# Jeremy-Cleland/hmer-img2latex

Measured on AMD Instinct MI355X. Metric: decoded LaTeX tokens/sec at batch 256, 320x64 imgs, seq 150, higher is better.
Workload: dtype f32

## Files before the change

hmer-img2latex_amd/csrc/api.hip:

```cpp
#include "common.h"
#include <new>

extern "C" int i2l_version(void) { return 107; }

extern "C" const char* i2l_error_string(int code) {
    switch (code) {
        case I2L_OK: return "ok";
        case I2L_ERR_ARG: return "invalid argument (null pointer or non-positive dimension)";
        case I2L_ERR_UNSUPPORTED: return "dimension not supported by the gfx950 kernels";
        case I2L_ERR_WORKSPACE: return "workspace missing or too small";
        case I2L_ERR_LAUNCH: return "HIP launch error";
        default: return "unknown error";
    }
}

struct i2l_lanes {
    int n = 0;
    hipStream_t s[I2L_MAX_LANES] = {};
    hipEvent_t fork[I2L_MAX_LANES] = {}, join[I2L_MAX_LANES] = {};
};

extern "C" int i2l_lanes_create(const i2l_stream_t* streams, int n, i2l_lanes** out) {
    if (!streams || !out || n < 1 || n > I2L_MAX_LANES) return I2L_ERR_ARG;
    for (int i = 0; i < n; ++i)
        if (!streams[i]) return I2L_ERR_ARG;
    i2l_lanes* l = new (std::nothrow) i2l_lanes();
    if (!l) return I2L_ERR_WORKSPACE;
    l->n = n;
    bool ok = true;
    for (int i = 0; i < n; ++i) {
        l->s[i] = i2l_s(streams[i]);
        ok = ok && hipEventCreateWithFlags(&l->fork[i], hipEventDisableTiming) == hipSuccess;
        ok = ok && hipEventCreateWithFlags(&l->join[i], hipEventDisableTiming) == hipSuccess;
    }
    if (!ok) { i2l_lanes_destroy(l); return I2L_ERR_LAUNCH; }
    *out = l;
    return I2L_OK;
}

extern "C" int i2l_lanes_destroy(i2l_lanes* l) {
    if (!l) return I2L_OK;
    for (int i = 0; i < I2L_MAX_LANES; ++i) {
        if (l->fork[i]) (void)hipEventDestroy(l->fork[i]);
        if (l->join[i]) (void)hipEventDestroy(l->join[i]);
    }
    delete l;
    return I2L_OK;
}

hipStream_t i2l_side_fork(i2l_lanes* l, hipStream_t main, int lane) {
    if (!l || lane < 0) return nullptr;
    if (lane >= l->n) lane = l->n - 1;
    if (hipEventRecord(l->fork[lane], main) != hipSuccess) return nullptr;
    if (hipStreamWaitEvent(l->s[lane], l->fork[lane], 0) != hipSuccess) return nullptr;
    return l->s[lane];
}

extern "C" int i2l_lanes_join(i2l_lanes* l, i2l_stream_t stream) {
    if (!l) return I2L_ERR_ARG;
    for (int i = 0; i < l->n; ++i) {
        if (hipEventRecord(l->join[i], l->s[i]) != hipSuccess) return I2L_ERR_LAUNCH;
        if (hipStreamWaitEvent(i2l_s(stream), l->join[i], 0) != hipSuccess) return I2L_ERR_LAUNCH;
    }
    return I2L_OK;
}

namespace {
__global__ void wait_value32_kernel(const unsigned* flag, unsigned value, long long ticks) {
    const long long t0 = (long long)wall_clock64();
    for (;;) {
        const unsigned v = __hip_atomic_load(flag, __ATOMIC_ACQUIRE, __HIP_MEMORY_SCOPE_AGENT);
        if ((int)(v - value) >= 0) return;
        if ((long long)wall_clock64() - t0 > ticks) return;
        __builtin_amdgcn_s_sleep(4);
    }
}
}

extern "C" int i2l_stream_wait_value32(const uint32_t* flag, uint32_t value, float timeout_us, i2l_stream_t stream) {
    if (!flag || !(timeout_us >= 0.f) || timeout_us > 100000.f) return I2L_ERR_ARG;
    hipLaunchKernelGGL(wait_value32_kernel, dim3(1), dim3(1), 0, i2l_s(stream), flag, value, (long long)(timeout_us * 100.f));
    return hipGetLastError() == hipSuccess ? I2L_OK : I2L_ERR_LAUNCH;
}
```

hmer-img2latex_amd/csrc/decode.hip:

```cpp
#include <math.h>
#include <stdlib.h>

#include "common.h"

namespace {

#include "lstm_rows.inc.h"

constexpr int MAXL = I2L_MAX_LSTM_LAYERS;
constexpr int NT = 256;
constexpr int VCHUNK = 2 * NT;

constexpr size_t GROUP_STATUS_BYTES = 2048;
inline bool group_shape_ok(int V, int H, int L) { return L == 1 && H == 256 && V <= 512; }

__global__ __launch_bounds__(256) void transpose_perm_kernel(const float* __restrict__ W, int N, int K,
                                                             float* __restrict__ out, int ld_out, int Npad,
                                                             int perm_h) {
    __shared__ float tile[64][65];
    const int c0 = blockIdx.x * 64, k0 = blockIdx.y * 64;
    const int tx = threadIdx.x & 63, ty = threadIdx.x >> 6;
    for (int i = ty; i < 64; i += 4) {
        const int c = c0 + i, k = k0 + tx;
        const int n = perm_h > 0 ? (c & 3) * perm_h + (c >> 2) : c;
// ... 358 lines not shown
                __syncthreads();
                if (p.top_k > 0) {
                    const int kk = min(p.top_k, V);
                    float kth = -1.f;
                    for (int v = tid; v < V; v += NT) {
                        const float pv = pr[v];
                        int gt = 0, ge = 0;
                        for (int u = 0; u < V; ++u) { const float pu = pr[u]; gt += pu > pv; ge += pu >= pv; }
                        if (gt < kk && kk <= ge) kth = pv;
                    }
                    kth = block_max(kth, redv, tid);
                    float s2 = 0.f;
                    for (int v = tid; v < V; v += NT) { const float q = pr[v] < kth ? 0.f : pr[v]; pr[v] = q; s2 += q; }
                    s2 = block_sum(s2, redv, tid);
                    if (s2 > 0.f) for (int v = tid; v < V; v += NT) pr[v] = pr[v] / s2;
                    __syncthreads();
                }
                if (p.top_p > 0.f) {
                    float* nx = lg + (size_t)(R + r) * w.Vp;
                    float s2 = 0.f;
                    for (int v = tid; v < V; v += NT) {
                        const float pv = pr[v];
                        float before = 0.f;
                        for (int u = 0; u < V; ++u) { const float pu = pr[u]; if (pu > pv || (pu == pv && u < v)) before += pu; }
                        const float q = before > p.top_p ? 0.f : pv;
                        nx[v] = q;
                        s2 += q;
                    }
                    __syncthreads();
                    for (int v = tid; v < V; v += NT) pr[v] = nx[v];
                    s2 = block_sum(s2, redv, tid);
                    if (s2 > 0.f) for (int v = tid; v < V; v += NT) pr[v] = pr[v] / s2;
                    __syncthreads();
                }
                if (p.probs && row0 + r < B) {
                    float* po = p.probs + ((size_t)(row0 + r) * T + t) * V;
                    for (int v = tid; v < V; v += NT) po[v] = pr[v];
                }
                const int CH = (V + NT - 1) / NT;
                float part = 0.f;
                for (int v = tid * CH; v < min(V, (tid + 1) * CH); ++v) part += pr[v];
                float* scan = psum;
                scan[tid] = part;
                __syncthreads();
                if (tid == 0) {
                    float run = 0.f;
                    for (int i = 0; i < NT; ++i) { const float x = scan[i]; scan[i] = run; run += x; }
                    scan[NT] = run;
                }
                __syncthreads();
                const float total = scan[NT];
                const float target = uniform01(p.seed, (unsigned)(row0 + r), (unsigned)t) * total;
                int pick = 0x7fffffff;
                float run = scan[tid];
                for (int v = tid * CH; v < min(V, (tid + 1) * CH); ++v) {
                    const float q = pr[v];
                    if (q > 0.f && run + q > target && pick == 0x7fffffff && run <= target) pick = v;
                    run += q;
                }
                float dummy = pick == 0x7fffffff ? -1.f : 1.f;
                int pk = pick;
                float bv[1] = {dummy};
                int bi[1] = {pk};
                block_argmax<1>(bv, bi, redv, redi, tid);
                besti[r] = bi[0] < V ? bi[0] : besti[r];
            }
        }
        if (tid == 0) {
#pragma unroll
            for (int r = 0; r < R; ++r) {
                const int row = row0 + r;
                const int sel = besti[r] < V ? besti[r] : 0;
                const int was_fin = fin_s[r];
                if (p.ids && row < B) p.ids[(size_t)row * T + t] = (p.stop == I2L_STOP_STICKY && was_fin) ? -1 : sel;
                tok_s[r] = sel;
                if (sel == p.end_id || row >= B) fin_s[r] = 1;
            }
        }
        __syncthreads();
        par ^= 1;
        if (p.stop == I2L_STOP_STICKY) {
            bool all = true;
#pragma unroll
            for (int r = 0; r < R; ++r) all = all && (fin_s[r] != 0);
            if (all) { ++t; break; }
        }
    }
    if (p.ids && t < T) {
        for (int idx = tid; idx < R * (T - t); idx += NT) {
            const int r = idx / (T - t), tt = t + (idx - r * (T - t));
            if (row0 + r < B) p.ids[(size_t)(row0 + r) * T + tt] = -1;
        }
    }
    if (p.h_out || p.c_out) {
        for (int idx = tid; idx < L * R * H; idx += NT) {
            const int l = idx / (R * H);
            const int rem = idx - l * (R * H);
            const int r = rem / H, j = rem - r * H;
            if (row0 + r < B) {
                const size_t g = ((size_t)l * B + row0 + r) * H + j;
                if (p.h_out) p.h_out[g] = hs[(size_t)par * L * R * H + idx];
                if (p.c_out) p.c_out[g] = cs[idx];
            }
        }
    }
}

struct BeamParams {
    StepWeights w;
    int images, T, start_id, end_id;
    int32_t* tokhist;
    int32_t* parhist;
    int32_t* seq_out;
    int32_t* len_out;
    double* score_out;
};

template <int K>
__global__ __launch_bounds__(NT) void beam_kernel(BeamParams p) {
    extern __shared__ __attribute__((aligned(16))) float smem[];
    const StepWeights& w = p.w;
    const int H = w.H, L = w.L, T = p.T, V = w.V, Vp = w.Vp;
    const int LKH = L * K * H;
    float* hs = smem;
    float* cs = hs + 2 * LKH;
    float* lg = cs + 2 * LKH;
    float* psum = lg + (size_t)K * Vp;
    double* score = reinterpret_cast<double*>(psum + K * 512);
    double* nscore = score + K;
    float* topv = reinterpret_cast<float*>(nscore + K);
    int* topi = reinterpret_cast<int*>(topv + K * K);
    int* last = topi + K * K;
    int* live = last + K;
    int* npar = live + K;
    int* ntok = npar + K;
    int* ctl = ntok + K;

    const int tid = threadIdx.x, lane = tid & 63, wave = tid >> 6;
    const int img = blockIdx.x;
    int32_t* tokhist = p.tokhist + (size_t)img * T * K;
    int32_t* parhist = p.parhist + (size_t)img * T * K;

    for (int idx = tid; idx < 2 * LKH; idx += NT) { hs[idx] = 0.f; cs[idx] = 0.f; }
    if (tid == 0) {
        for (int q = 0; q < K; ++q) { score[q] = 0.0; last[q] = p.start_id; live[q] = 0; }
        ctl[0] = 1; ctl[1] = 0; ctl[2] = 0;
    }
    bool has_c = false;
    double best_c = 0.0;
    int best_t = -1, best_q = 0;
    int t_last = -1;
    __syncthreads();

    int par = 0, cpar = 0;
    for (int t = 0; t < T; ++t) {
        if (tid == 0) {
            const int nb = ctl[0];
            int nl = 0;
            for (int q = 0; q < K; ++q) {
                int lv = 0;
                if (q < nb) {
                    if (last[q] == p.end_id) {
                        if (!has_c || score[q] > best_c) { has_c = true; best_c = score[q]; best_t = t - 1; best_q = q; }
                    } else { lv = 1; ++nl; }
                }
                live[q] = lv;
            }
            ctl[1] = nl;
        }
        __syncthreads();
        if (ctl[1] == 0) break;

        int tok[K], grow[K];
#pragma unroll
        for (int r = 0; r < K; ++r) { tok[r] = min(max(last[r], 0), V - 1); grow[r] = img; }
        lstm_layers<K>(w, tok, grow, hs, cs + (size_t)cpar * LKH, cs + (size_t)(cpar ^ 1) * LKH, par, tid);
        const float* h_top = hs + ((size_t)(par ^ 1) * L + (L - 1)) * K * H;
        float* lp[K];
#pragma unroll
        for (int r = 0; r < K; ++r) lp[r] = nullptr;
        float best[K];
        int besti[K];
        project<K>(w, h_top, lp, lg, false, 1.f, best, besti, psum, tid);
        __syncthreads();

        for (int r = wave; r < K; r += NT / 64) {
            if (!live[r]) continue;
            const float* x = lg + (size_t)r * Vp;
            float m = -INFINITY;
            for (int v = lane; v < V; v += 64) m = fmaxf(m, x[v]);
            m = wave_max(m);
            float s = 0.f;
            for (int v = lane; v < V; v += 64) s += expf(x[v] - m);
            s = wave_sum(s);
            const float lse = logf(s);
            unsigned taken = 0;
            for (int j = 0; j < K; ++j) {
                float bv = -INFINITY;
                int bi = 0x7fffffff;
                for (int v = lane, i = 0; v < V; v += 64, ++i)
                    if (!((taken >> i) & 1u) && x[v] > bv) { bv = x[v]; bi = v; }
                wave_argmax(bv, bi);
                if (bi < V && (bi & 63) == lane) taken |= 1u << (bi >> 6);
                if (lane == 0) { topv[r * K + j] = (bv - m) - lse; topi[r * K + j] = bi < V ? bi : 0; }
            }
        }
        __syncthreads();

        if (tid == 0) {
            const int nlive = ctl[1];
            const int ncand = nlive * K;
            const int nnew = ncand < K ? ncand : K;
            unsigned long long used = 0ull;
            for (int q = 0; q < nnew; ++q) {
                double bs = 0.0;
                int bc = -1;
                for (int s0 = 0; s0 < K; ++s0) {
                    if (!live[s0]) continue;
                    for (int j = 0; j < K; ++j) {
                        const int c = s0 * K + j;
                        if ((used >> c) & 1ull) continue;
                        const double sc = score[s0] + (double)topv[c];
                        if (bc < 0 || sc > bs) { bs = sc; bc = c; }
                    }
                }
                used |= 1ull << bc;
                npar[q] = bc / K;
                ntok[q] = topi[bc];
                nscore[q] = bs;
                tokhist[(size_t)t * K + q] = topi[bc];
                parhist[(size_t)t * K + q] = bc / K;
            }
            for (int q = nnew; q < K; ++q) { npar[q] = 0; ntok[q] = 0; nscore[q] = 0.0; }
            ctl[0] = nnew;
            t_last = t;
        }
        __syncthreads();

        {
            const float* hsrc = hs + (size_t)(par ^ 1) * LKH;
            float* hdst = hs + (size_t)par * LKH;
            const float* csrc = cs + (size_t)(cpar ^ 1) * LKH;
            float* cdst = cs + (size_t)cpar * LKH;
            for (int idx = tid; idx < LKH; idx += NT) {
                const int l = idx / (K * H);
                const int rem = idx - l * (K * H);
                const int q = rem / H, j = rem - q * H;
                const size_t src = ((size_t)l * K + npar[q]) * H + j;
                hdst[idx] = hsrc[src];
                cdst[idx] = csrc[src];
            }
        }
        __syncthreads();
        if (tid == 0) {
            const int nb = ctl[0];
            bool all_end = true;
            for (int q = 0; q < K; ++q) {
                score[q] = nscore[q];
                last[q] = ntok[q];
                if (q < nb && ntok[q] != p.end_id) all_end = false;
            }
            if (all_end) {
                for (int q = 0; q < nb; ++q)
                    if (!has_c || score[q] > best_c) { has_c = true; best_c = score[q]; best_t = t; best_q = q; }
                ctl[2] = 1;
            }
        }
        __syncthreads();
        if (ctl[2]) break;
    }

    if (tid == 0) {
        int tt = has_c ? best_t : t_last, q = has_c ? best_q : 0;
        const double sc = has_c ? best_c : score[0];
        int32_t* out = p.seq_out + (size_t)img * (T + 1);
        int n = tt + 1;
        for (int pos = tt; pos >= 0; --pos) {
            out[pos] = tokhist[(size_t)pos * K + q];
            q = parhist[(size_t)pos * K + q];
        }
        int len = n;
        for (int i = 0; i < n; ++i)
            if (out[i] == p.end_id) { len = i; break; }
        for (int i = len; i < T + 1; ++i) out[i] = -1;
        p.len_out[img] = len;
        if (p.score_out) p.score_out[img] = sc;
    }
}

struct GroupVariant {
    void (*kernel)(GroupParams);
    int flag;
    int rows, threads;
    size_t lds, xchg_per_group;
};
constexpr int GROUP_VARIANTS = 3;
template <int M>
constexpr GroupVariant grouped_variant(int flag) {
    using S = GroupShape<M>;
    return {decode_group_kernel<M>, flag, M, S::NT, S::LDS, S::XCHG_PER_GROUP};
}
constexpr GroupVariant group_variant(int i) {
    constexpr GroupVariant table[GROUP_VARIANTS] = {
        {decode_group16_kernel, I2L_FLAG_DECODE_GROUP16, G16Q, G16NT, GRP16_LDS, GROUP16_XCHG_PER_GROUP},
        grouped_variant<8>(I2L_FLAG_DECODE_GROUP8),
        grouped_variant<4>(0),
    };
    return table[i];
}

struct Layout {
    size_t P, Genc, WhhT[MAXL], WihT[MAXL], biasP[MAXL], WoutT, boutP, wpack16, gemm_ws, xchg, xchg_bytes, total;
    int Vp;
};

Layout make_layout(int rows, int V, int E, int H, int L) {
    Layout o{};
    size_t off = 0;
    auto take = [&](size_t floats) { size_t r = off; off += i2l_align(floats * sizeof(float)); return r; };
    const size_t G = 4 * (size_t)H;
    o.Vp = i2l_cdiv(V, VCHUNK) * VCHUNK;
    o.P = take((size_t)V * G);
    o.Genc = take((size_t)rows * G);
    for (int l = 0; l < L; ++l) o.WhhT[l] = take((size_t)H * G);
    for (int l = 1; l < L; ++l) o.WihT[l] = take((size_t)H * G);
    for (int l = 1; l < L; ++l) o.biasP[l] = take(G);
    o.WoutT = take((size_t)H * o.Vp);
    o.boutP = take(o.Vp);
    if (group_shape_ok(V, H, L)) o.wpack16 = take((size_t)16 * 4 * 36 * 64 * 4);
    size_t g1 = i2l_gemm_workspace_bytes(V, 4 * H, E), g2 = i2l_gemm_workspace_bytes(rows, 4 * H, E);
    o.gemm_ws = off;
    off += i2l_align(g1 > g2 ? g1 : g2);
    if (group_shape_ok(V, H, L)) {
        o.xchg = off;
        size_t most = 0;
        for (int i = 0; i < GROUP_VARIANTS; ++i) {
            const GroupVariant g = group_variant(i);
            const size_t x = group_xchg_bytes(i2l_cdiv(rows, g.rows), g.xchg_per_group);
            most = x > most ? x : most;
        }
        o.xchg_bytes = GROUP_STATUS_BYTES + most;
        off += i2l_align(o.xchg_bytes);
    }
    o.total = off;
    return o;
}

int check_weights(const i2l_decoder_weights* w) {
    if (!w || !w->embedding || !w->w_ih || !w->w_hh || !w->b_ih || !w->b_hh || !w->w_out || !w->b_out)
        return I2L_ERR_ARG;
    if (w->vocab <= 0 || w->embed <= 0 || w->hidden <= 0 || w->layers <= 0) return I2L_ERR_ARG;
    if (w->layers > MAXL || w->hidden % 64 != 0 || w->hidden > 2048 || w->embed % 4 != 0) return I2L_ERR_UNSUPPORTED;
    for (int l = 0; l < w->layers; ++l)
        if (!w->w_ih[l] || !w->w_hh[l] || !w->b_ih[l] || !w->b_hh[l]) return I2L_ERR_ARG;
    return I2L_OK;
}

StepWeights step_weights(const Layout& lo, const char* base, int V, int H, int L) {
    auto F = [&](size_t off) { return reinterpret_cast<const float*>(base + off); };
    StepWeights w{};
    w.H = H; w.L = L; w.V = V; w.Vp = lo.Vp;
    w.P = F(lo.P); w.Genc = F(lo.Genc);
    for (int l = 0; l < L; ++l) {
        w.WhhT[l] = F(lo.WhhT[l]);
        w.WihT[l] = l > 0 ? F(lo.WihT[l]) : nullptr;
        w.biasP[l] = l > 0 ? F(lo.biasP[l]) : nullptr;
    }
    w.WoutT = F(lo.WoutT); w.boutP = F(lo.boutP);
    w.wpack16 = lo.wpack16 ? base + lo.wpack16 : nullptr;
    return w;
}

constexpr int RES_KR = 76, RES_KL = 36;
constexpr int RES2_KR = 64, RES2_KL = 32;

size_t decode_lds_bytes(int R, int L, int H, int Vp, int select, int KL = 0) {
    size_t floats = (size_t)3 * L * R * H + 4 * R + 4 * R + R + R + 4 + (size_t)R * 512 + (size_t)KL * 4 * H;
    if (select != I2L_SELECT_LOGITS) floats += (size_t)R * Vp;
    if (select == I2L_SELECT_SAMPLE) floats += (size_t)R * Vp;
    return floats * sizeof(float);
}

}

extern "C" size_t i2l_decoder_workspace_bytes(int rows, int vocab, int embed, int hidden, int layers) {
    if (rows <= 0 || vocab <= 0 || embed <= 0 || hidden <= 0 || layers <= 0 || layers > MAXL) return 0;
    return make_layout(rows, vocab, embed, hidden, layers).total;
}

extern "C" int i2l_decoder_prepare(const i2l_decoder_weights* w, const float* enc, int rows, int what,
                                   void* workspace, size_t workspace_bytes, i2l_stream_t stream) {
    int rc = check_weights(w);
    if (rc != I2L_OK) return rc;
    if (rows <= 0 || (what & ~I2L_PREP_ALL) || what == 0) return I2L_ERR_ARG;
    if ((what & I2L_PREP_ROWS) && !enc) return I2L_ERR_ARG;
    const int V = w->vocab, E = w->embed, H = w->hidden, L = w->layers;
    const Layout lo = make_layout(rows, V, E, H, L);
    if (!workspace || workspace_bytes < lo.total) return I2L_ERR_WORKSPACE;
    char* base = static_cast<char*>(workspace);
    hipStream_t s = i2l_s(stream);
    auto F = [&](size_t off) { return reinterpret_cast<float*>(base + off); };
    const int G = 4 * H;

    for (int l = 0; l < L && (what & I2L_PREP_WEIGHTS); ++l) {
        dim3 grid(i2l_cdiv(G, 64), i2l_cdiv(H, 64));
        hipLaunchKernelGGL(transpose_perm_kernel, grid, dim3(256), 0, s, w->w_hh[l], G, H, F(lo.WhhT[l]), G, G, H);
        I2L_CHECK_LAUNCH();
        if (l > 0) {
            hipLaunchKernelGGL(transpose_perm_kernel, grid, dim3(256), 0, s, w->w_ih[l], G, H, F(lo.WihT[l]), G, G, H);
            I2L_CHECK_LAUNCH();
            hipLaunchKernelGGL(bias_perm_kernel, dim3(i2l_cdiv(G, 256)), dim3(256), 0, s, w->b_ih[l], w->b_hh[l],
                               F(lo.biasP[l]), H);
            I2L_CHECK_LAUNCH();
        }
    }
    if (what & I2L_PREP_WEIGHTS) {
        dim3 grid(i2l_cdiv(lo.Vp, 64), i2l_cdiv(H, 64));
        hipLaunchKernelGGL(transpose_perm_kernel, grid, dim3(256), 0, s, w->w_out, V, H, F(lo.WoutT), lo.Vp, lo.Vp, 0);
        I2L_CHECK_LAUNCH();
        hipLaunchKernelGGL(bout_pad_kernel, dim3(i2l_cdiv(lo.Vp, 256)), dim3(256), 0, s, w->b_out, F(lo.boutP), V, lo.Vp);
        I2L_CHECK_LAUNCH();
        if (lo.wpack16) {
            hipLaunchKernelGGL(pack16_kernel, dim3(16 * 4), dim3(64), 0, s, F(lo.WhhT[0]), F(lo.WoutT),
                               reinterpret_cast<u32x4_t*>(base + lo.wpack16));
            I2L_CHECK_LAUNCH();
        }
    }
    const size_t gws = lo.total - lo.gemm_ws;
    if (what & I2L_PREP_WEIGHTS) {
        GemmArgs g = gemm_args();
        g.A = w->embedding; g.lda = E;
        g.W = w->w_ih[0]; g.ldw = 2 * E;
        g.C = F(lo.P); g.ldc = G;
        g.M = V; g.N = G; g.K = E; g.perm_h = H;
        rc = i2l_gemm(g, base + lo.gemm_ws, gws, s);
        if (rc != I2L_OK) return rc;
    }
    if (what & I2L_PREP_ROWS) {
        GemmArgs g = gemm_args();
        g.A = enc; g.lda = E;
        g.W = w->w_ih[0] + E; g.ldw = 2 * E;
        g.bias = w->b_ih[0]; g.bias2 = w->b_hh[0];
        g.C = F(lo.Genc); g.ldc = G;
        g.M = rows; g.N = G; g.K = E; g.perm_h = H;
        rc = i2l_gemm(g, base + lo.gemm_ws, gws, s);
        if (rc != I2L_OK) return rc;
    }
    return I2L_OK;
}

namespace {
int launch_decode(const i2l_decoder_weights* w, const void* workspace, int rows, int steps, const int32_t* tok0,
                  const int32_t* forced, const float* h0, const float* c0, float temperature, int select, int stop,
                  int end_id, int top_k, float top_p, unsigned long long seed, int32_t* ids_out, float* logits_out,
                  float* probs_out, float* h_out, float* c_out, i2l_stream_t stream, int rows_per_wg = 0, int flags = 0,
                  uint32_t* resident_flag = nullptr, uint32_t resident_value = 0);
}

extern "C" int i2l_greedy_decode_ex(const i2l_decoder_weights* w, const void* workspace, int rows, int steps,
                                    const int32_t* tok0, const int32_t* forced, const float* h0, const float* c0,
                                    float temperature, int select, int stop, int end_id, int rows_per_workgroup,
                                    int32_t* ids_out, float* logits_out, float* h_out, float* c_out, int flags,
                                    uint32_t* resident_flag, uint32_t resident_value, i2l_stream_t stream) {
    if (select != I2L_SELECT_LOGITS && select != I2L_SELECT_SOFTMAX) return I2L_ERR_ARG;
    if (rows_per_workgroup != 0 && rows_per_workgroup != 1 && rows_per_workgroup != 2 && rows_per_workgroup != 4)
        return I2L_ERR_ARG;
    return launch_decode(w, workspace, rows, steps, tok0, forced, h0, c0, temperature, select, stop, end_id, 0, 0.f, 0ull,
                         ids_out, logits_out, nullptr, h_out, c_out, stream, rows_per_workgroup, flags, resident_flag,
                         resident_value);
}

extern "C" int i2l_greedy_decode(const i2l_decoder_weights* w, const void* workspace, int rows, int steps,
                                 const int32_t* tok0, const int32_t* forced, const float* h0, const float* c0,
                                 float temperature, int select, int stop, int end_id, int32_t* ids_out,
                                 float* logits_out, float* h_out, float* c_out, i2l_stream_t stream) {
    if (select != I2L_SELECT_LOGITS && select != I2L_SELECT_SOFTMAX) return I2L_ERR_ARG;
    return launch_decode(w, workspace, rows, steps, tok0, forced, h0, c0, temperature, select, stop, end_id, 0, 0.f, 0ull,
                         ids_out, logits_out, nullptr, h_out, c_out, stream);
}

extern "C" int i2l_sample_decode(const i2l_decoder_weights* w, const void* workspace, int rows, int steps,
                                 const int32_t* tok0, const float* h0, const float* c0, float temperature, int top_k,
                                 float top_p, uint64_t seed, int stop, int end_id, int32_t* ids_out, float* probs_out,
                                 float* h_out, float* c_out, i2l_stream_t stream) {
    if (!(temperature > 0.f) || top_k < 0 || top_p < 0.f || (top_k == 0 && top_p == 0.f)) return I2L_ERR_ARG;
    if (w && w->vocab > 8 * 256) return I2L_ERR_UNSUPPORTED;
    return launch_decode(w, workspace, rows, steps, tok0, nullptr, h0, c0, temperature, I2L_SELECT_SAMPLE, stop, end_id,
                         top_k, top_p, (unsigned long long)seed, ids_out, nullptr, probs_out, h_out, c_out, stream);
}

namespace {
__global__ void publish_value32_kernel(unsigned* flag, unsigned value) { publish_max32(flag, value); }

int launch_decode(const i2l_decoder_weights* w, const void* workspace, int rows, int steps, const int32_t* tok0,
                  const int32_t* forced, const float* h0, const float* c0, float temperature, int select, int stop,
                  int end_id, int top_k, float top_p, unsigned long long seed, int32_t* ids_out, float* logits_out,
                  float* probs_out, float* h_out, float* c_out, i2l_stream_t stream, int rows_per_wg, int flags,
                  uint32_t* resident_flag, uint32_t resident_value) {
    int rc = check_weights(w);
    if (rc != I2L_OK) return rc;
    if (!workspace || !tok0 || rows <= 0 || steps <= 0) return I2L_ERR_ARG;
    if ((h0 == nullptr) != (c0 == nullptr)) return I2L_ERR_ARG;
    if (stop != I2L_STOP_NONE && stop != I2L_STOP_STICKY) return I2L_ERR_ARG;
    const int V = w->vocab, E = w->embed, H = w->hidden, L = w->layers;
    const Layout lo = make_layout(rows, V, E, H, L);
    const char* base = static_cast<const char*>(workspace);

    DecodeParams p{};
    p.w = step_weights(lo, base, V, H, L);
    p.B = rows; p.T = steps;
    p.tok0 = tok0; p.forced = forced; p.h0 = h0; p.c0 = c0;
    p.h_out = h_out; p.c_out = c_out; p.ids = ids_out; p.logits = logits_out;
    p.temperature = temperature; p.use_temp = (temperature != 1.0f) ? 1 : 0;
    p.select = select; p.stop = stop; p.end_id = end_id;
    p.top_k = top_k; p.top_p = top_p; p.seed = seed; p.probs = probs_out;

    if (rows_per_wg == 0 && lo.xchg_bytes && (select == I2L_SELECT_LOGITS || select == I2L_SELECT_SOFTMAX) && !h0 &&
        !h_out && !c_out &&
        steps >= 8 && steps <= 65000) {
        GroupParams gp{};
        gp.w = p.w; gp.B = rows; gp.T = steps;
        gp.tok0 = tok0; gp.forced = forced; gp.ids = ids_out; gp.logits = logits_out;
        gp.temperature = temperature; gp.use_temp = p.use_temp; gp.stop = stop; gp.end_id = end_id;
        char* xb = const_cast<char*>(base) + lo.xchg;
        gp.status = reinterpret_cast<unsigned*>(xb);
        gp.xchg = reinterpret_cast<u64_t*>(xb + GROUP_STATUS_BYTES);
        gp.opts = group_opts(steps, flags);
        gp.resident_flag = resident_flag; gp.resident_value = resident_value;
        hipStream_t gs = i2l_s(stream);
        const bool ids_only = ids_out && !logits_out && !forced;
        static std::atomic<unsigned> attr[GROUP_VARIANTS]{};
        for (int i = 0; i < GROUP_VARIANTS; ++i) {
            const GroupVariant g = group_variant(i);
            if (g.flag && !((flags & g.flag) && ids_only)) continue;
            if (!i2l_lds_attr(reinterpret_cast<const void*>(g.kernel), g.lds, attr[i])) continue;
            if (!(flags & I2L_FLAG_DECODE_REGION_CLEARED) && hipMemsetAsync(xb, 0, lo.xchg_bytes, gs) != hipSuccess) return I2L_ERR_LAUNCH;
            gp.n_groups = i2l_cdiv(rows, g.rows);
            hipLaunchKernelGGL(g.kernel, dim3(group_grid(gp.n_groups, g.rows)), dim3(g.threads), g.lds, gs, gp);
            I2L_CHECK_LAUNCH();
            return I2L_OK;
        }
    }
    if (resident_flag) {
        hipLaunchKernelGGL(publish_value32_kernel, dim3(1), dim3(1), 0, i2l_s(stream), resident_flag, resident_value);
        I2L_CHECK_LAUNCH();
    }
    int R = rows <= 256 ? 1 : (rows <= 512 ? 2 : 4);
    if (rows_per_wg > 0) R = rows_per_wg;
    while (R > 1 && decode_lds_bytes(R, L, H, lo.Vp, select) > 64 * 1024) R >>= 1;
    const size_t lds = decode_lds_bytes(R, L, H, lo.Vp, select);
    if (lds > 64 * 1024) return I2L_ERR_UNSUPPORTED;
    const dim3 grid(i2l_cdiv(rows, R));
    hipStream_t s = i2l_s(stream);
    if (select == I2L_SELECT_SAMPLE) {
        if (R == 1) hipLaunchKernelGGL((decode_kernel<1, 0, 0, true>), grid, dim3(NT), lds, s, p);
        else if (R == 2) hipLaunchKernelGGL((decode_kernel<2, 0, 0, true>), grid, dim3(NT), lds, s, p);
        else hipLaunchKernelGGL((decode_kernel<4, 0, 0, true>), grid, dim3(NT), lds, s, p);
        I2L_CHECK_LAUNCH();
        return I2L_OK;
    }
    const bool resident = (R == 1 || R == 2) && L == 1 && H == 256 && steps >= 8;
    if (resident) {
        const size_t lds_r = decode_lds_bytes(R, 1, H, lo.Vp, select, R == 1 ? RES_KL : RES2_KL);
        auto kern = R == 1 ? decode_kernel<1, RES_KR, RES_KL> : decode_kernel<2, RES2_KR, RES2_KL>;
        if (lds_r <= 160 * 1024 &&
            hipFuncSetAttribute(reinterpret_cast<const void*>(kern), hipFuncAttributeMaxDynamicSharedMemorySize,
                                (int)lds_r) == hipSuccess) {
            hipLaunchKernelGGL(kern, grid, dim3(NT), lds_r, s, p);
            I2L_CHECK_LAUNCH();
            return I2L_OK;
        }
    }
    if (R == 1) hipLaunchKernelGGL((decode_kernel<1, 0, 0>), grid, dim3(NT), lds, s, p);
    else if (R == 2) hipLaunchKernelGGL((decode_kernel<2, 0, 0>), grid, dim3(NT), lds, s, p);
    else hipLaunchKernelGGL((decode_kernel<4, 0, 0>), grid, dim3(NT), lds, s, p);
    I2L_CHECK_LAUNCH();
    return I2L_OK;
}
}

extern "C" size_t i2l_decode_batched_scratch_bytes(int rows, int vocab, int hidden, int layers) {
    if (!batched_dims_ok(rows, vocab, hidden, layers)) return 0;
    return batched_layout(rows, i2l_cdiv(vocab, VCHUNK) * VCHUNK, hidden, layers).total;
}

namespace {
template <int TB>
void launch_batched_lstm(const BatchedParams& p, int layer, int t, hipStream_t s) {
    hipLaunchKernelGGL(lstm_step_mfma_kernel<TB>, dim3(p.w.H / 16, i2l_cdiv(p.B, TB)), dim3(DB_NT), 0, s, p, layer, t);
}
template <int TB>
void launch_batched_logits(const BatchedParams& p, int t, hipStream_t s) {
    hipLaunchKernelGGL(logits_mfma_kernel<TB>, dim3(p.w.Vp / DB_COLS, i2l_cdiv(p.B, TB)), dim3(DB_NT), 0, s, p, t);
}
}

extern "C" int i2l_greedy_decode_batched(const i2l_decoder_weights* w, const void* workspace, int rows, int steps,
                                         const int32_t* tok0, const int32_t* forced, const float* h0, const float* c0,
                                         float temperature, int select, int stop, int end_id, int32_t* ids_out,
                                         float* logits_out, float* h_out, float* c_out, void* scratch,
                                         size_t scratch_bytes, int flags, uint32_t* resident_flag,
                                         uint32_t resident_value, i2l_stream_t stream) {
    (void)flags;
    int rc = check_weights(w);
    if (rc != I2L_OK) return rc;
    if (select != I2L_SELECT_LOGITS && select != I2L_SELECT_SOFTMAX) return I2L_ERR_ARG;
    if (!workspace || !tok0 || rows <= 0 || steps <= 0) return I2L_ERR_ARG;
    if ((h0 == nullptr) != (c0 == nullptr)) return I2L_ERR_ARG;
    if (stop != I2L_STOP_NONE && stop != I2L_STOP_STICKY) return I2L_ERR_ARG;
    const int V = w->vocab, E = w->embed, H = w->hidden, L = w->layers;
    const Layout lo = make_layout(rows, V, E, H, L);
    const BatchedLayout bl = batched_layout(rows, lo.Vp, H, L);
    if (!scratch || scratch_bytes < bl.total) return I2L_ERR_WORKSPACE;

    char* sb = static_cast<char*>(scratch);
    BatchedParams p{};
    p.w = step_weights(lo, static_cast<const char*>(workspace), V, H, L);
    p.B = rows; p.T = steps; p.genc_div = 1; p.forced = forced;
    p.h = reinterpret_cast<float*>(sb + bl.h); p.c = reinterpret_cast<float*>(sb + bl.c);
    p.lg = reinterpret_cast<float*>(sb + bl.lg);
    p.tok = reinterpret_cast<int*>(sb + bl.tok); p.fin = reinterpret_cast<int*>(sb + bl.fin);
    p.live = reinterpret_cast<unsigned*>(sb + bl.live);
    p.ids = ids_out; p.logits_out = logits_out;
    p.temperature = temperature; p.use_temp = (temperature != 1.0f) ? 1 : 0;
    p.select = select; p.stop = stop; p.end_id = end_id;

    hipStream_t s = i2l_s(stream);
    if (resident_flag) {
        hipLaunchKernelGGL(publish_value32_kernel, dim3(1), dim3(1), 0, s, resident_flag, resident_value);
        I2L_CHECK_LAUNCH();
    }
    const size_t most = (size_t)L * rows * H > (size_t)rows * steps ? (size_t)L * rows * H : (size_t)rows * steps;
    const size_t copy_blocks = (most + DB_NT - 1) / DB_NT;
    const int copy_grid = (int)(copy_blocks < 1024 ? copy_blocks : 1024);
    hipLaunchKernelGGL(init_batched_kernel, dim3(copy_grid), dim3(DB_NT), 0, s, p, tok0, h0, c0);
    I2L_CHECK_LAUNCH();
    const int tb_lstm = batched_tile_rows(H / 16, rows), tb_logits = batched_tile_rows(lo.Vp / DB_COLS, rows);
    const int sel_grid = i2l_cdiv(rows, DB_NT / 64);
    for (int t = 0; t < steps; ++t) {
        for (int l = 0; l < L; ++l) {
            if (tb_lstm == 16) launch_batched_lstm<16>(p, l, t, s);
            else if (tb_lstm == 32) launch_batched_lstm<32>(p, l, t, s);
            else launch_batched_lstm<64>(p, l, t, s);
        }
        if (tb_logits == 16) launch_batched_logits<16>(p, t, s);
        else if (tb_logits == 32) launch_batched_logits<32>(p, t, s);
        else launch_batched_logits<64>(p, t, s);
        hipLaunchKernelGGL(select_batched_kernel, dim3(sel_grid), dim3(DB_NT), 0, s, p, t);
        I2L_CHECK_LAUNCH();
    }
    if (h_out || c_out) {
        hipLaunchKernelGGL(state_out_batched_kernel, dim3(copy_grid), dim3(DB_NT), 0, s, p, h_out, c_out);
        I2L_CHECK_LAUNCH();
    }
    return I2L_OK;
}

namespace {

size_t beam_lds_bytes(int K, int L, int H, int Vp) {
    size_t b = (size_t)4 * L * K * H * sizeof(float) + (size_t)K * Vp * sizeof(float) + (size_t)K * 512 * sizeof(float);
    b = (b + 7) / 8 * 8;
    b += 2 * (size_t)K * sizeof(double) + (size_t)2 * K * K * 4 + (size_t)4 * K * 4 + 4 * 4;
    return b;
}

template <int K>
int launch_beam(const BeamParams& p, size_t lds, hipStream_t s) {
    if (lds > 64 * 1024) {
        if (hipFuncSetAttribute(reinterpret_cast<const void*>(&beam_kernel<K>),
                                hipFuncAttributeMaxDynamicSharedMemorySize, (int)lds) != hipSuccess)
            return I2L_ERR_UNSUPPORTED;
    }
    hipLaunchKernelGGL(beam_kernel<K>, dim3(p.images), dim3(NT), lds, s, p);
    I2L_CHECK_LAUNCH();
    return I2L_OK;
}

}

namespace {
inline bool beam_group_ok(int beam, int H, int L) { return L == 1 && H == 256 && beam >= 2 && beam <= 6; }
inline int beam_groups(int images, int beam) { return i2l_cdiv(images, BG_S / beam); }
inline size_t beam_hist_bytes(int images, int beam, int steps) {
    return i2l_align((size_t)2 * images * steps * beam * sizeof(int32_t));
}
template <int K>
int launch_beam_group(const BeamGroupParams& p, hipStream_t s) {
    constexpr size_t lds = bg_lds_bytes();
    static_assert(lds <= 160 * 1024, "beam_group_kernel LDS");
    static std::atomic<unsigned> attr{0};
    if (!i2l_lds_attr(reinterpret_cast<const void*>(&beam_group_kernel<K>), lds, attr)) return I2L_ERR_UNSUPPORTED;
    hipLaunchKernelGGL(beam_group_kernel<K>, dim3(group_grid(p.n_groups, GQ)), dim3(GNT), lds, s, p);
    I2L_CHECK_LAUNCH();
    return I2L_OK;
}
}

extern "C" size_t i2l_beam_workspace_bytes(int images, int beam, int hidden, int layers, int steps) {
    if (images <= 0 || beam <= 0 || beam > I2L_MAX_BEAM || steps <= 0) return 0;
    size_t b = beam_hist_bytes(images, beam, steps);
    if (beam_group_ok(beam, hidden, layers))
        b += GROUP_STATUS_BYTES + group_xchg_bytes(beam_groups(images, beam), BEAM_XCHG_PER_GROUP);
    return b;
}

extern "C" int i2l_beam_decode(const i2l_decoder_weights* w, const void* workspace, int images, int beam, int steps,
                               int start_id, int end_id, void* beam_workspace, size_t beam_workspace_bytes,
                               int32_t* seq_out, int32_t* len_out, double* score_out, int flags, i2l_stream_t stream) {
    int rc = check_weights(w);
    if (rc != I2L_OK) return rc;
    if (!workspace || !beam_workspace || !seq_out || !len_out || images <= 0 || steps <= 0 || beam <= 0)
        return I2L_ERR_ARG;
    if (beam > I2L_MAX_BEAM || beam > w->vocab) return I2L_ERR_UNSUPPORTED;
    const size_t need = (size_t)2 * images * steps * beam * sizeof(int32_t);
    if (beam_workspace_bytes < need) return I2L_ERR_WORKSPACE;
    const int V = w->vocab, E = w->embed, H = w->hidden, L = w->layers;
    const Layout lo = make_layout(images, V, E, H, L);
    if (lo.Vp > 64 * 32) return I2L_ERR_UNSUPPORTED;
    hipStream_t s = i2l_s(stream);
    const bool group_on = !(flags & I2L_FLAG_NO_GROUP);
    if (group_on && beam_group_ok(beam, H, L) && V <= 512 && steps <= 65000 &&
        beam_workspace_bytes >= i2l_beam_workspace_bytes(images, beam, H, L, steps)) {
        BeamGroupParams gp{};
        gp.w = step_weights(lo, static_cast<const char*>(workspace), V, H, L);
        gp.images = images; gp.T = steps; gp.n_groups = beam_groups(images, beam);
        gp.start_id = start_id; gp.end_id = end_id;
        gp.tokhist = static_cast<int32_t*>(beam_workspace);
        gp.parhist = gp.tokhist + (size_t)images * steps * beam;
        gp.seq_out = seq_out; gp.len_out = len_out; gp.score_out = score_out;
        char* xb = static_cast<char*>(beam_workspace) + beam_hist_bytes(images, beam, steps);
        const size_t xbytes = GROUP_STATUS_BYTES + group_xchg_bytes(gp.n_groups, BEAM_XCHG_PER_GROUP);
        gp.status = reinterpret_cast<unsigned*>(xb);
        gp.xchg = reinterpret_cast<u64_t*>(xb + GROUP_STATUS_BYTES);
        gp.opts = group_opts(steps, flags);
        if (hipMemsetAsync(xb, 0, xbytes, s) != hipSuccess) return I2L_ERR_LAUNCH;
        switch (beam) {
            case 2: return launch_beam_group<2>(gp, s);
            case 3: return launch_beam_group<3>(gp, s);
            case 4: return launch_beam_group<4>(gp, s);
            case 5: return launch_beam_group<5>(gp, s);
            case 6: return launch_beam_group<6>(gp, s);
            default: break;
        }
    }
    BeamParams p{};
    p.w = step_weights(lo, static_cast<const char*>(workspace), V, H, L);
    p.images = images; p.T = steps; p.start_id = start_id; p.end_id = end_id;
    p.tokhist = static_cast<int32_t*>(beam_workspace);
    p.parhist = p.tokhist + (size_t)images * steps * beam;
    p.seq_out = seq_out; p.len_out = len_out; p.score_out = score_out;
    const size_t lds = beam_lds_bytes(beam, L, H, lo.Vp);
    if (lds > 160 * 1024) return I2L_ERR_UNSUPPORTED;
    switch (beam) {
        case 1: return launch_beam<1>(p, lds, s);
        case 2: return launch_beam<2>(p, lds, s);
        case 3: return launch_beam<3>(p, lds, s);
        case 4: return launch_beam<4>(p, lds, s);
        case 5: return launch_beam<5>(p, lds, s);
        case 6: return launch_beam<6>(p, lds, s);
        case 7: return launch_beam<7>(p, lds, s);
        case 8: return launch_beam<8>(p, lds, s);
        default: return I2L_ERR_UNSUPPORTED;
    }
}

extern "C" size_t i2l_beam_batched_scratch_bytes(int images, int beam, int vocab, int hidden, int layers, int steps) {
    if (!beam_batched_dims_ok(images, beam, vocab, hidden, layers, steps)) return 0;
    return beam_batched_layout(images, beam, i2l_cdiv(vocab, VCHUNK) * VCHUNK, hidden, layers, steps).total;
}

namespace {
template <int K>
void launch_beam_step_batched(const BeamBatchedParams& p, float* c_cur, float* c_next, int t, hipStream_t s) {
    hipLaunchKernelGGL(beam_step_batched_kernel<K>, dim3(p.images), dim3(DB_NT), 0, s, p, c_cur, c_next, t);
}
}

extern "C" int i2l_beam_decode_batched(const i2l_decoder_weights* w, const void* workspace, int images, int beam,
                                       int steps, int start_id, int end_id, void* scratch, size_t scratch_bytes,
                                       int32_t* seq_out, int32_t* len_out, double* score_out, int flags,
                                       i2l_stream_t stream) {
    (void)flags;
    int rc = check_weights(w);
    if (rc != I2L_OK) return rc;
    if (!workspace || !scratch || !seq_out || !len_out || images <= 0 || steps <= 0 || beam <= 0) return I2L_ERR_ARG;
    const int V = w->vocab, E = w->embed, H = w->hidden, L = w->layers;
    if (!beam_batched_dims_ok(images, beam, V, H, L, steps)) return I2L_ERR_UNSUPPORTED;
    const Layout lo = make_layout(images, V, E, H, L);
    const BeamBatchedLayout bl = beam_batched_layout(images, beam, lo.Vp, H, L, steps);
    if (scratch_bytes < bl.total) return I2L_ERR_WORKSPACE;

    char* sb = static_cast<char*>(scratch);
    const int R = images * beam;
    const size_t LRH = (size_t)L * R * H;
    BeamBatchedParams bp{};
    bp.images = images; bp.T = steps; bp.V = V; bp.Vp = lo.Vp; bp.H = H; bp.L = L;
    bp.start_id = start_id; bp.end_id = end_id;
    bp.tokhist = reinterpret_cast<int32_t*>(sb + bl.hist);
    bp.parhist = bp.tokhist + (size_t)images * steps * beam;
    bp.h = reinterpret_cast<float*>(sb + bl.h); bp.c = reinterpret_cast<float*>(sb + bl.c);
    bp.lg = reinterpret_cast<float*>(sb + bl.lg);
    bp.score = reinterpret_cast<double*>(sb + bl.score);
    bp.last = reinterpret_cast<int*>(sb + bl.last); bp.slot_live = reinterpret_cast<int*>(sb + bl.slot_live);
    bp.img = reinterpret_cast<BeamImage*>(sb + bl.img);
    bp.live = reinterpret_cast<unsigned*>(sb + bl.live);
    bp.seq_out = seq_out; bp.len_out = len_out; bp.score_out = score_out;

    BatchedParams p{};
    p.w = step_weights(lo, static_cast<const char*>(workspace), V, H, L);
    p.B = R; p.T = steps; p.genc_div = beam; p.forced = nullptr;
    p.h = bp.h; p.lg = reinterpret_cast<float*>(sb + bl.lg);
    p.tok = bp.last; p.live = bp.live;
    p.temperature = 1.0f; p.select = I2L_SELECT_LOGITS; p.stop = I2L_STOP_NONE; p.end_id = end_id;

    hipStream_t s = i2l_s(stream);
    const size_t init_blocks = (2 * LRH + DB_NT - 1) / DB_NT;
    hipLaunchKernelGGL(beam_init_batched_kernel, dim3((unsigned)(init_blocks < 1024 ? init_blocks : 1024)), dim3(DB_NT), 0,
                       s, bp, beam);
    I2L_CHECK_LAUNCH();
    const int tb_lstm = batched_tile_rows(H / 16, R), tb_logits = batched_tile_rows(lo.Vp / DB_COLS, R);
    for (int t = 0; t < steps; ++t) {
        float* c_cur = bp.c + (size_t)(t & 1) * LRH;
        float* c_next = bp.c + (size_t)((t + 1) & 1) * LRH;
        p.c = c_cur;
        for (int l = 0; l < L; ++l) {
            if (tb_lstm == 16) launch_batched_lstm<16>(p, l, 0, s);
            else if (tb_lstm == 32) launch_batched_lstm<32>(p, l, 0, s);
            else launch_batched_lstm<64>(p, l, 0, s);
        }
        if (tb_logits == 16) launch_batched_logits<16>(p, 0, s);
        else if (tb_logits == 32) launch_batched_logits<32>(p, 0, s);
        else launch_batched_logits<64>(p, 0, s);
        switch (beam) {
            case 1: launch_beam_step_batched<1>(bp, c_cur, c_next, t, s); break;
            case 2: launch_beam_step_batched<2>(bp, c_cur, c_next, t, s); break;
            case 3: launch_beam_step_batched<3>(bp, c_cur, c_next, t, s); break;
            case 4: launch_beam_step_batched<4>(bp, c_cur, c_next, t, s); break;
            case 5: launch_beam_step_batched<5>(bp, c_cur, c_next, t, s); break;
            case 6: launch_beam_step_batched<6>(bp, c_cur, c_next, t, s); break;
            case 7: launch_beam_step_batched<7>(bp, c_cur, c_next, t, s); break;
            default: launch_beam_step_batched<8>(bp, c_cur, c_next, t, s); break;
        }
        I2L_CHECK_LAUNCH();
    }
    hipLaunchKernelGGL(beam_final_batched_kernel, dim3(i2l_cdiv(images, DB_NT)), dim3(DB_NT), 0, s, bp, beam);
    I2L_CHECK_LAUNCH();
    return I2L_OK;
}

extern "C" size_t i2l_decoder_group_status_offset(int rows, int vocab, int embed, int hidden, int layers) {
    const Layout lo = make_layout(rows, vocab, embed, hidden, layers);
    return lo.xchg_bytes ? lo.xchg : 0;
}

extern "C" size_t i2l_decoder_group_region_bytes(int rows, int vocab, int embed, int hidden, int layers) {
    return make_layout(rows, vocab, embed, hidden, layers).xchg_bytes;
}

#ifdef I2L_GROUP_STAMPS
extern "C" size_t i2l_debug_group_status_offset(int rows, int vocab, int embed, int hidden, int layers) {
    return make_layout(rows, vocab, embed, hidden, layers).xchg;
}
#endif
```

hmer-img2latex_amd/csrc/decode_group.inc.h:

```cpp
#include "group_common.inc.h"

constexpr int GQ = 4;
constexpr int GNT = 512;
constexpr int GRAN_H = 256;
constexpr int GRAN_C = GRAN_H;
constexpr int GRAN_X = GRAN_H + 16;
constexpr int GRAN = GRAN_H + 32;

template <int M>
struct GroupShape {
    static_assert(M == 4 || M == 8, "members per group");
    static constexpr int NT = 2048 / M;
    static constexpr int UPM = 256 / M;
    static constexpr int CPM = 512 / M;
    static constexpr size_t LDS = (size_t)(256 * CPM + 2 * 256 * M + (M == 4 ? 4 * NT : 0)) * sizeof(float) +
                                  (size_t)2 * M * 8 + 8 * sizeof(int);
    static constexpr size_t XCHG_PER_GROUP = (size_t)2 * M * GRAN * 8;
};

struct GroupParams {
    StepWeights w;
    int B, T, n_groups;
    const int32_t* tok0;
    const int32_t* forced;
    int32_t* ids;
    float* logits;
    float temperature;
    int use_temp, stop, end_id;
    u64_t* xchg;
    unsigned* status;
    GroupOpts opts;
    unsigned* resident_flag;
    unsigned resident_value;
};

constexpr int DPP_SHL12 = 0x10C;

template <int NT>
__device__ __forceinline__ void load_weight_image(f32x2 (&wreg)[32][2], float4* wout_s4, const StepWeights& w, int unit,
                                                  int ke, int col, int ks, int tid) {
#pragma unroll
    for (int j = 0; j < 32; ++j) {
        const float4 t4 = *reinterpret_cast<const float4*>(w.WhhT[0] + (size_t)(8 * j + ke) * 1024 + 4 * unit);
        wreg[j][0] = f32x2{t4.x, t4.y};
        wreg[j][1] = f32x2{t4.z, t4.w};
    }
#pragma unroll
    for (int j = 0; j < 16; ++j)
        wout_s4[j * NT + tid] = *reinterpret_cast<const float4*>(w.WoutT + (size_t)(16 * j + ks) * 512 + col);
}

template <class Hook>
__device__ __forceinline__ void rec_product4(f32x2 (&acc)[4][2], const f32x2 (&wreg)[32][2], const float4* hq4,
                                             Hook&& hook) {
    float4 hb[2][4];
#pragma unroll
    for (int i = 0; i < 4; ++i) hb[0][i] = hq4[8 * i];
#pragma unroll
    for (int b = 0; b < 8; ++b) {
        if (b + 1 < 8) {
#pragma unroll
            for (int i = 0; i < 4; ++i) hb[(b + 1) & 1][i] = hq4[8 * ((b + 1) * 4 + i)];
        }
        hook(b);
        __builtin_amdgcn_sched_barrier(0);
#pragma unroll
        for (int i = 0; i < 4; ++i) fma_4x4(acc, wreg[b * 4 + i][0], wreg[b * 4 + i][1], hb[b & 1][i]);
    }
}
__device__ __forceinline__ void fold_gates4(const f32x2 (&acc)[4][2], int ke, float (&z)[2]) {
    const bool b0 = ke & 1, b1 = ke & 2, b2 = ke & 4;
#pragma unroll
    for (int e = 0; e < 2; ++e) {
        float wv[2];
#pragma unroll
        for (int rp = 0; rp < 2; ++rp) {
            const float ux = rs_level<DPP_HMIRROR>(acc[e][rp].x, acc[2 + e][rp].x, b2);
            const float uy = rs_level<DPP_HMIRROR>(acc[e][rp].y, acc[2 + e][rp].y, b2);
            wv[rp] = rs_level<DPP_XOR1>(ux, uy, b0);
        }
        z[e] = rs_level<DPP_XOR2>(wv[0], wv[1], b1);
    }
}
template <int NT>
__device__ __forceinline__ void logits_product4(f32x2 (&pa)[4][2], const float4* wout_s4, const float4* hq4, int tid) {
#pragma unroll
    for (int c = 0; c < 4; ++c) { pa[c][0] = splat2(0.f); pa[c][1] = splat2(0.f); }
    float4 wb[2][2], hb[2][2];
    auto fetch = [&](int set, int b) {
#pragma unroll
        for (int i = 0; i < 2; ++i) {
            wb[set][i] = wout_s4[(b * 2 + i) * NT + tid];
            hb[set][i] = hq4[16 * (b * 2 + i)];
        }
    };
    fetch(0, 0);
#pragma unroll
    for (int b = 0; b < 8; ++b) {
        if (b + 1 < 8) fetch((b + 1) & 1, b + 1);
        __builtin_amdgcn_sched_barrier(0);
#pragma unroll
        for (int i = 0; i < 2; ++i) {
            const float4 w4 = wb[b & 1][i];
            fma_4x4(pa, f32x2{w4.x, w4.y}, f32x2{w4.z, w4.w}, hb[b & 1][i]);
        }
    }
}
__device__ __forceinline__ float fold_logits4(const f32x2 (&pa)[4][2], int ks) {
    const bool b0 = ks & 1, b1 = ks & 2, b2 = ks & 4, b3 = ks & 8;
    float z[2];
#pragma unroll
    for (int e = 0; e < 2; ++e) {
        float wv[2];
#pragma unroll
        for (int rp = 0; rp < 2; ++rp) {
            const float ux = rs_level<DPP_HMIRROR>(pa[e][rp].x, pa[2 + e][rp].x, b2);
            const float uy = rs_level<DPP_HMIRROR>(pa[e][rp].y, pa[2 + e][rp].y, b2);
            wv[rp] = rs_level<DPP_XOR1>(ux, uy, b0);
        }
        z[e] = rs_level<DPP_XOR2>(wv[0], wv[1], b1);
    }
    return rs_level<DPP_ROR8>(z[0], z[1], b3);
}

template <class Hook>
__device__ __forceinline__ void rec_product8(f32x2 (&acc)[2][4][2], const f32x2 (&wreg)[32][2], const float4* hq4,
                                             Hook&& hook) {
    float4 hb[2][2][2];
#pragma unroll
    for (int i = 0; i < 2; ++i) { hb[0][i][0] = hq4[16 * i]; hb[0][i][1] = hq4[16 * i + 1]; }
#pragma unroll
    for (int b = 0; b < 16; ++b) {
        if (b + 1 < 16) {
#pragma unroll
            for (int i = 0; i < 2; ++i) {
                hb[(b + 1) & 1][i][0] = hq4[16 * ((b + 1) * 2 + i)];
                hb[(b + 1) & 1][i][1] = hq4[16 * ((b + 1) * 2 + i) + 1];
            }
        }
        hook(b);
        __builtin_amdgcn_sched_barrier(0);
#pragma unroll
        for (int i = 0; i < 2; ++i) {
            fma_4x4(acc[0], wreg[b * 2 + i][0], wreg[b * 2 + i][1], hb[b & 1][i][0]);
            fma_4x4(acc[1], wreg[b * 2 + i][0], wreg[b * 2 + i][1], hb[b & 1][i][1]);
        }
    }
}
__device__ __forceinline__ void fold_gates8(const f32x2 (&acc)[2][4][2], int ke, float (&z)[4]) {
    const bool b0 = ke & 1, b1 = ke & 2, b2 = ke & 4;
#pragma unroll
    for (int g = 0; g < 4; ++g) {
        const float u0x = rs_level<DPP_HMIRROR>(acc[0][g][0].x, acc[1][g][0].x, b2);
        const float u0y = rs_level<DPP_HMIRROR>(acc[0][g][0].y, acc[1][g][0].y, b2);
        const float u1x = rs_level<DPP_HMIRROR>(acc[0][g][1].x, acc[1][g][1].x, b2);
        const float u1y = rs_level<DPP_HMIRROR>(acc[0][g][1].y, acc[1][g][1].y, b2);
        const float vx = rs_level<DPP_XOR2>(u0x, u1x, b1);
        const float vy = rs_level<DPP_XOR2>(u0y, u1y, b1);
        z[g] = rs_level<DPP_XOR1>(vx, vy, b0);
    }
}
template <int NT>
__device__ __forceinline__ void logits_product8(f32x2 (&pa)[2][4][2], const float4* wout_s4, const float4* hq4, int tid) {
#pragma unroll
    for (int hf = 0; hf < 2; ++hf)
#pragma unroll
        for (int c = 0; c < 4; ++c) { pa[hf][c][0] = splat2(0.f); pa[hf][c][1] = splat2(0.f); }
    float4 wb[2], hb[2][2];
    wb[0] = wout_s4[tid];
    hb[0][0] = hq4[0]; hb[0][1] = hq4[1];
#pragma unroll
    for (int j = 0; j < 16; ++j) {
        if (j + 1 < 16) {
            wb[(j + 1) & 1] = wout_s4[(j + 1) * NT + tid];
            hb[(j + 1) & 1][0] = hq4[32 * (j + 1)];
            hb[(j + 1) & 1][1] = hq4[32 * (j + 1) + 1];
        }
        __builtin_amdgcn_sched_barrier(0);
        const float4 w4 = wb[j & 1];
        fma_4x4(pa[0], f32x2{w4.x, w4.y}, f32x2{w4.z, w4.w}, hb[j & 1][0]);
        fma_4x4(pa[1], f32x2{w4.x, w4.y}, f32x2{w4.z, w4.w}, hb[j & 1][1]);
    }
}
__device__ __forceinline__ void fold_logits8(const f32x2 (&pa)[2][4][2], int ks, float (&lv)[2]) {
    const bool b0 = ks & 1, b1 = ks & 2, b2 = ks & 4, b3 = ks & 8;
    float v[4];
#pragma unroll
    for (int c = 0; c < 4; ++c) {
        const float u0x = rs_level<DPP_ROR8>(pa[0][c][0].x, pa[1][c][0].x, b3);
        const float u0y = rs_level<DPP_ROR8>(pa[0][c][0].y, pa[1][c][0].y, b3);
        const float u1x = rs_level<DPP_ROR8>(pa[0][c][1].x, pa[1][c][1].x, b3);
        const float u1y = rs_level<DPP_ROR8>(pa[0][c][1].y, pa[1][c][1].y, b3);
        const float wx = rs_level<DPP_HMIRROR>(u0x, u1x, b2);
        const float wy = rs_level<DPP_HMIRROR>(u0y, u1y, b2);
        v[c] = rs_level<DPP_XOR2>(wx, wy, b1);
    }
    lv[0] = rs_level<DPP_XOR1>(v[0], v[2], b0);
    lv[1] = rs_level<DPP_XOR1>(v[1], v[3], b0);
}

template <int M>
__global__ __launch_bounds__(GroupShape<M>::NT) void decode_group_kernel(GroupParams p) {
    using S = GroupShape<M>;
    constexpr int NT = S::NT, UPM = S::UPM, CPM = S::CPM;
    constexpr bool FULL = M == 4;
    extern __shared__ __attribute__((aligned(16))) float smem[];
    float4* wout_s4 = reinterpret_cast<float4*>(smem);
    float* h_s = smem + 256 * CPM;
    float4* genc_s = reinterpret_cast<float4*>(h_s + 2 * 256 * M);
    u64_t* redk = reinterpret_cast<u64_t*>(genc_s + (M == 4 ? NT : 0));
    int* cnt_s = reinterpret_cast<int*>(redk + 2 * M);

    const StepWeights& w = p.w;
    const int tid = threadIdx.x, lane = tid & 63, wave = tid >> 6;
    const GroupSeat seat = group_seat<M>();
    const int group = seat.group, m = seat.m;
    if (group >= p.n_groups) return;
    const int B = p.B, T = p.T, V = w.V;
    const int row0 = group * M;
    const int ul = tid >> 3, ke = tid & 7;
    const int unit = UPM * m + ul;
    const int cq = tid >> 4, ks = tid & 15;
    const int l_row = M == 4 ? ks & 3 : ks >> 1;
    const int l_v = CPM * m + 4 * cq + (M == 4 ? ((ks >> 2) & 1) * 2 + (ks >> 3) : 2 * (ks & 1));
    const int my_r = ke & (M - 1);
    constexpr int G = 1024;

    f32x2 wreg[32][2];
    load_weight_image<NT>(wreg, wout_s4, w, unit, ke, CPM * m + 4 * cq, ks, tid);
    for (int idx = tid; idx < 2 * 256 * M; idx += NT) h_s[idx] = 0.f;
    if (tid < 2 * M) redk[tid] = 0;
    if (tid < 4) cnt_s[tid] = 0;
    float4 genc;
    {
        const float4 g4 = *reinterpret_cast<const float4*>(w.Genc + (size_t)min(row0 + my_r, B - 1) * G + 4 * unit);
        if constexpr (M == 4) genc_s[tid] = g4; else genc = g4;
    }
    float l_bias[M / 4];
#pragma unroll
    for (int i = 0; i < M / 4; ++i) l_bias[i] = w.boutP[l_v + i];
    float c_own = 0.f, h_own = 0.f;
    unsigned fin = 0;
#pragma unroll
    for (int r = 0; r < M; ++r)
        if (row0 + r >= B) fin |= 1u << r;
    u64_t* xg = p.xchg + (size_t)group * 2 * M * GRAN;
    const bool own_row = row0 + m < B;
    int32_t* ids_row = (p.ids && own_row) ? p.ids + (size_t)(row0 + m) * T : nullptr;
    float* lrow = (FULL && p.logits && row0 + l_row < B && l_v < V) ? p.logits + (size_t)(row0 + l_row) * T * V + l_v
                                                                    : nullptr;
    __syncthreads();
    if (wave == 0) {
        const Placement pl = group_placement<M>(xg, GRAN, GRAN_X, m, p.opts);
        if (lane == 0) {
            cnt_s[3] = (pl.one_xcd && !pl.timed_out) ? 1 : 0;
            if (pl.timed_out) cnt_s[2] = 1;
            if (m == 0 && !pl.timed_out)
                report_group(p.status, p.n_groups, p.resident_flag, p.resident_value, pl.one_xcd && !p.opts.agent_scope);
        }
    }
    __syncthreads();
    const bool local = cnt_s[3] != 0 && !p.opts.agent_scope;

    int mytok = min(max(p.tok0[min(row0 + my_r, B - 1)], 0), V - 1);
    if (FULL && p.forced) mytok = min(max(p.forced[(size_t)min(row0 + my_r, B - 1) * T], 0), V - 1);
    float4 pvec = *reinterpret_cast<const float4*>(w.P + (size_t)mytok * G + 4 * unit);

    int t = 0;
    bool failed = cnt_s[2] != 0;
    I2L_STAMPS_BEGIN;
    for (; !failed; ++t) {
        f32x2 acc[M / 4][4][2];
#pragma unroll
        for (int hf = 0; hf < M / 4; ++hf)
#pragma unroll
            for (int g = 0; g < 4; ++g) { acc[hf][g][0] = splat2(0.f); acc[hf][g][1] = splat2(0.f); }
        const float* hprev = h_s + ((t - 1) & 1) * 256 * M;
        const u64_t* cand_src = xg + (size_t)((t - 1) & 1) * M * GRAN + (size_t)((lane / M) & (M - 1)) * GRAN + GRAN_C +
                                (lane & (M - 1));
        const unsigned c_epoch = (unsigned)t;
        bool have = t == 0;
        int tk[M] = {};
        u64_t gv = 0;
        auto issue = [&]() {
            if (lane < M * M) gv = load_granule(cand_src);
        };
        auto check = [&]() {
            if (!__all(lane >= M * M || (unsigned)(gv >> 48) == c_epoch)) return;
            u64_t best;
            if constexpr (M == 4) {
                const int g_lo = (int)(unsigned)gv, g_hi = (int)(unsigned)(gv >> 32);
                best = am_key(__int_as_float(g_lo), g_hi & 0xFFFF);
                best = umax64(best, am_key(__int_as_float(__builtin_amdgcn_mov_dpp(g_lo, DPP_SHL4, 0xF, 0xF, true)),
                                           __builtin_amdgcn_mov_dpp(g_hi, DPP_SHL4, 0xF, 0xF, true) & 0xFFFF));
                best = umax64(best, am_key(__int_as_float(__builtin_amdgcn_mov_dpp(g_lo, DPP_SHL8, 0xF, 0xF, true)),
                                           __builtin_amdgcn_mov_dpp(g_hi, DPP_SHL8, 0xF, 0xF, true) & 0xFFFF));
                best = umax64(best, am_key(__int_as_float(__builtin_amdgcn_mov_dpp(g_lo, DPP_SHL12, 0xF, 0xF, true)),
                                           __builtin_amdgcn_mov_dpp(g_hi, DPP_SHL12, 0xF, 0xF, true) & 0xFFFF));
            } else {
                best = am_key(__uint_as_float((unsigned)gv), (int)((unsigned)(gv >> 32) & 0xFFFFu));
                best = umax64(best, dpp_u64<DPP_SHL8>(best));
                best = umax64(best, (u64_t)__shfl_xor((unsigned long long)best, 16));
                best = umax64(best, (u64_t)__shfl_xor((unsigned long long)best, 32));
            }
            const int bi = am_idx(best);
#pragma unroll
            for (int r = 0; r < M; ++r) {
                tk[r] = __builtin_amdgcn_readlane(bi, r);
                tk[r] = tk[r] < V ? tk[r] : 0;
            }
            have = true;
            if (t < T) {
                mytok = tk[0];
#pragma unroll
                for (int r = 1; r < M; ++r) mytok = my_r == r ? tk[r] : mytok;
                if (FULL && p.forced) mytok = min(max(p.forced[(size_t)min(row0 + my_r, B - 1) * T + t], 0), V - 1);
                pvec = *reinterpret_cast<const float4*>(w.P + (size_t)mytok * G + 4 * unit);
            }
        };
        if (t > 0 && t < T) {
            constexpr int NB = 2 * M;
            auto poll = [&](int b) {
                if (b == NB / 8) issue();
                if (b == NB / 2) { check(); if (!have) issue(); }
                if (b == NB - NB / 8 && !have) check();
            };
            if constexpr (M == 4) rec_product4(acc[0], wreg, reinterpret_cast<const float4*>(hprev) + ke, poll);
            else rec_product8(acc, wreg, reinterpret_cast<const float4*>(hprev) + 2 * ke, poll);
        }
        I2L_STAMP(0);
        bool bail = false;
        if (!have) {
            PollClock clk;
            for (;;) {
                issue();
                check();
// ... 137 lines not shown
```

hmer-img2latex_amd/csrc/decode_group16.inc.h:

```cpp
#include "mfma_slab.inc.h"

constexpr int G16Q = 16;
constexpr int G16NT = 256;
constexpr int G16GRAN_H = 256;
constexpr int G16GRAN_C = G16GRAN_H;
constexpr int G16GRAN_X = G16GRAN_H + 16;
constexpr int G16GRAN = G16GRAN_H + 32;
constexpr int G16_HP_PIECE = 32 * 16 * 8;
constexpr size_t GRP16_LDS = (size_t)2 * 3 * G16_HP_PIECE * 2 + (size_t)2 * 64 * 16 + (size_t)2 * 16 * 8 + 8 * sizeof(int);
constexpr size_t GROUP16_XCHG_PER_GROUP = (size_t)2 * G16Q * G16GRAN * 8;

__device__ __forceinline__ void load_run64(const u64_t* src, u32x4_t (&g)[4]) {
    asm volatile(
        "global_load_dwordx4 %0, %4, off sc1\n\t"
        "global_load_dwordx4 %1, %4, off offset:16 sc1\n\t"
        "global_load_dwordx4 %2, %4, off offset:32 sc1\n\t"
        "global_load_dwordx4 %3, %4, off offset:48 sc1\n\t"
        "s_waitcnt vmcnt(0)"
        : "=&v"(g[0]), "=&v"(g[1]), "=&v"(g[2]), "=&v"(g[3])
        : "v"(src)
        : "memory");
}

__global__ __launch_bounds__(64) void pack16_kernel(const float* __restrict__ WhhT, const float* __restrict__ WoutT,
                                                    u32x4_t* __restrict__ pack) {
    const int m = blockIdx.x >> 2, wave = blockIdx.x & 3, lane = threadIdx.x;
    const int lhi = lane >> 4, lcol = lane & 15, ltile = wave & 1, lhalf = wave >> 1;
    u32x4_t* dst = pack + (size_t)blockIdx.x * 36 * 64 + lane;
    const float* src = WhhT + 64 * m + 16 * wave + lcol;
    for (int ks = 0; ks < 8; ++ks) {
        Frag16 f0, f1, f2;
#pragma unroll
        for (int j = 0; j < 8; ++j) split3(src[(size_t)(32 * ks + 8 * lhi + j) * 1024], f0.s[j], f1.s[j], f2.s[j]);
        dst[(ks * 3 + 0) * 64] = f0.q; dst[(ks * 3 + 1) * 64] = f1.q; dst[(ks * 3 + 2) * 64] = f2.q;
    }
    const float* srl = WoutT + 32 * m + 16 * ltile + lcol;
    for (int ks = 0; ks < 4; ++ks) {
        Frag16 f0, f1, f2;
#pragma unroll
        for (int j = 0; j < 8; ++j) split3(srl[(size_t)(32 * (4 * lhalf + ks) + 8 * lhi + j) * 512], f0.s[j], f1.s[j], f2.s[j]);
        dst[(24 + ks * 3 + 0) * 64] = f0.q; dst[(24 + ks * 3 + 1) * 64] = f1.q; dst[(24 + ks * 3 + 2) * 64] = f2.q;
    }
}

__device__ __forceinline__ void load_run64x2(const u64_t* s0, const u64_t* s1, u32x4_t (&g)[8]) {
    asm volatile(
        "global_load_dwordx4 %0, %8, off sc1\n\t"
        "global_load_dwordx4 %1, %8, off offset:16 sc1\n\t"
        "global_load_dwordx4 %2, %8, off offset:32 sc1\n\t"
        "global_load_dwordx4 %3, %8, off offset:48 sc1\n\t"
        "global_load_dwordx4 %4, %9, off sc1\n\t"
        "global_load_dwordx4 %5, %9, off offset:16 sc1\n\t"
        "global_load_dwordx4 %6, %9, off offset:32 sc1\n\t"
        "global_load_dwordx4 %7, %9, off offset:48 sc1\n\t"
        "s_waitcnt vmcnt(0)"
        : "=&v"(g[0]), "=&v"(g[1]), "=&v"(g[2]), "=&v"(g[3]), "=&v"(g[4]), "=&v"(g[5]), "=&v"(g[6]), "=&v"(g[7])
        : "v"(s0), "v"(s1)
        : "memory");
}
__device__ __forceinline__ void unpack_run(const u32x4_t* g, u32x4_t* dst) {
    u32x4_t o0, o1, o2;
    o0.x = (g[0].y & 0xFFFFu) | (g[0].w << 16); o0.y = (g[1].y & 0xFFFFu) | (g[1].w << 16);
    o0.z = (g[2].y & 0xFFFFu) | (g[2].w << 16); o0.w = (g[3].y & 0xFFFFu) | (g[3].w << 16);
    o1.x = (g[0].x >> 16) | (g[0].z & 0xFFFF0000u); o1.y = (g[1].x >> 16) | (g[1].z & 0xFFFF0000u);
    o1.z = (g[2].x >> 16) | (g[2].z & 0xFFFF0000u); o1.w = (g[3].x >> 16) | (g[3].z & 0xFFFF0000u);
    o2.x = (g[0].x & 0xFFFFu) | (g[0].z << 16); o2.y = (g[1].x & 0xFFFFu) | (g[1].z << 16);
    o2.z = (g[2].x & 0xFFFFu) | (g[2].z << 16); o2.w = (g[3].x & 0xFFFFu) | (g[3].z << 16);
    dst[0] = o0;
    dst[G16_HP_PIECE / 8] = o1;
    dst[2 * (G16_HP_PIECE / 8)] = o2;
}

__global__ __launch_bounds__(G16NT, 2) void decode_group16_kernel(GroupParams p) {
    extern __shared__ __attribute__((aligned(16))) unsigned char smem16[];
    unsigned short* hp = reinterpret_cast<unsigned short*>(smem16);
    f32x4_t* lpart = reinterpret_cast<f32x4_t*>(smem16 + (size_t)2 * 3 * G16_HP_PIECE * 2);
    u64_t* redk = reinterpret_cast<u64_t*>(lpart + 2 * 64);
    int* cnt_s = reinterpret_cast<int*>(redk + 2 * 16);
    const StepWeights& w = p.w;
    const int tid = threadIdx.x, lane = tid & 63, wave = tid >> 6;
    const int within = blockIdx.x & 127;
    const int group = (blockIdx.x >> 7) * 8 + (within & 7), m = within >> 3;
    if (group >= p.n_groups) return;
    const int B = p.B, T = p.T, V = w.V;
    const int row0 = group * G16Q;
    constexpr int G = 1024;
    const int lq = lane & 3, uq = (lane >> 2) & 3, lhi = lane >> 4, lcol = lane & 15;
    const int cell_row = 4 * lhi + lq;
    const int unit = 16 * m + 4 * wave + uq;
    const int ltile = wave & 1, lhalf = wave >> 1;

    u64_t* xg = p.xchg + (size_t)group * 2 * G16Q * G16GRAN;
    if (tid < 8) cnt_s[tid] = 0;
    if (wave == 0) {
        unsigned xcc;
        asm volatile("s_getreg_b32 %0, hwreg(HW_REG_XCC_ID)" : "=s"(xcc));
        xcc &= 0xFu;
        if (lane == 0 && !(p.opts.drop_member && m == 3))
            store_granule(xg + (size_t)m * G16GRAN + G16GRAN_X, granule(0xC0DEu, __uint_as_float(xcc)), false);
        const int pq = (lane & 15) + ((lane & 15) >= m ? 1 : 0);
        u64_t pv = 0;
        bool bad = false;
        long long t_start = 0;
        unsigned spins = 0;
        for (;;) {
            bool ok = true;
            if (lane < 15) { pv = load_granule(xg + (size_t)pq * G16GRAN + G16GRAN_X); ok = (unsigned)(pv >> 32) == 0xC0DEu; }
            if (__all(ok)) break;
            __builtin_amdgcn_s_sleep(1);
            if ((++spins & 255u) == 0) {
                const long long now = (long long)wall_clock64();
                if (t_start == 0) t_start = now;
                else if (now - t_start > p.opts.limit_first) { bad = true; break; }
            }
        }
        const bool all_same = __all(lane >= 15 || (unsigned)pv == xcc);
        if (lane == 0) {
            cnt_s[3] = (all_same && !bad) ? 1 : 0;
            if (bad) cnt_s[2] = 1;
            if (m == 0 && !bad) {
                count_resident_group(p.status, p.n_groups, p.resident_flag, p.resident_value);
                if (all_same && !p.opts.agent_scope) atomicAdd(p.status + GRP_STAT_LOCAL, 1u);
            }
        }
    }
    bf16x8_t wg[24], wl[12];
    {
        const u32x4_t* pk = static_cast<const u32x4_t*>(w.wpack16) + (size_t)(m * 4 + wave) * 36 * 64 + lane;
#pragma unroll
        for (int i = 0; i < 24; ++i) { Frag16 f; f.q = pk[i * 64]; wg[i] = f.v; }
#pragma unroll
        for (int i = 0; i < 12; ++i) { Frag16 f; f.q = pk[(24 + i) * 64]; wl[i] = f.v; }
    }
    for (int idx = tid; idx < 2 * 3 * G16_HP_PIECE / 2; idx += G16NT) reinterpret_cast<unsigned*>(hp)[idx] = 0u;
    if (tid < 32) redk[tid] = 0;
    const float4 genc = *reinterpret_cast<const float4*>(w.Genc + (size_t)min(row0 + cell_row, B - 1) * G + 4 * unit);
    const float l_bias = w.boutP[32 * m + 16 * ltile + lcol];
    float c_own = 0.f, h_own = 0.f;
    unsigned fin = 0;
#pragma unroll
    for (int r = 0; r < G16Q; ++r)
        if (row0 + r >= B) fin |= 1u << r;
    const bool own_row = row0 + m < B;
    int32_t* ids_row = (p.ids && own_row) ? p.ids + (size_t)(row0 + m) * T : nullptr;

    __syncthreads();
    const bool local = cnt_s[3] != 0 && !p.opts.agent_scope;

    int mytok = min(max(p.tok0[min(row0 + cell_row, B - 1)], 0), V - 1);
    float4 pvec = *reinterpret_cast<const float4*>(w.P + (size_t)mytok * G + 4 * unit);

    int t = 0;
    bool failed = cnt_s[2] != 0;
#ifdef I2L_GROUP_STAMPS
    long long st_acc[8] = {0, 0, 0, 0, 0, 0, 0, 0};
    long long st_last = (long long)wall_clock64();
#define I2L_STAMP16(i) do { const long long n_ = (long long)wall_clock64(); st_acc[i] += n_ - st_last; st_last = n_; } while (0)
#else
#define I2L_STAMP16(i) do { } while (0)
#endif
    for (; !failed; ++t) {
        f32x4_t acc[3];
#pragma unroll
        for (int c = 0; c < 3; ++c) acc[c] = f32x4_t{0.f, 0.f, 0.f, 0.f};
        const u64_t* cand_src = xg + (size_t)((t - 1) & 1) * G16Q * G16GRAN + (size_t)(4 * lhi) * G16GRAN + G16GRAN_C + lcol;
        const unsigned c_epoch = (unsigned)t & 0xFFFFu;
        bool have = t == 0;
        int tk[16];
#pragma unroll
        for (int r = 0; r < 16; ++r) tk[r] = 0;
        u64_t gv[4] = {0, 0, 0, 0};
        auto issue = [&]() {
#pragma unroll
            for (int i = 0; i < 4; ++i) gv[i] = load_granule(cand_src + (size_t)i * G16GRAN);
        };
        auto check = [&]() {
            bool ok = true;
#pragma unroll
            for (int i = 0; i < 4; ++i) ok = ok && (unsigned)(gv[i] >> 48) == c_epoch;
            if (!__all(ok)) return;
            u64_t best = 0;
#pragma unroll
            for (int i = 0; i < 4; ++i)
                best = umax64(best, am_key(__uint_as_float((unsigned)gv[i]), (int)((unsigned)(gv[i] >> 32) & 0xFFFFu)));
            best = umax64(best, (u64_t)__shfl_xor((unsigned long long)best, 16));
            best = umax64(best, (u64_t)__shfl_xor((unsigned long long)best, 32));
            const int bi = am_idx(best);
#pragma unroll
            for (int r = 0; r < 16; ++r) {
                tk[r] = __builtin_amdgcn_readlane(bi, r);
                tk[r] = tk[r] < V ? tk[r] : 0;
            }
            have = true;
            if (t < T) {
                mytok = __shfl(bi, cell_row);
                mytok = mytok < V ? mytok : 0;
                pvec = *reinterpret_cast<const float4*>(w.P + (size_t)mytok * G + 4 * unit);
            }
        };
        if (t > 0 && t < T) {
            const u32x4_t* hq = reinterpret_cast<const u32x4_t*>(hp + (size_t)((t - 1) & 1) * 3 * G16_HP_PIECE) + lhi * 16 + lcol;
            issue();
            Frag16 fa[2][3];
#pragma unroll
            for (int c = 0; c < 3; ++c) fa[0][c].q = hq[(c * 32) * 16];
#pragma unroll
            for (int ks = 0; ks < 8; ++ks) {
                if (ks + 1 < 8) {
#pragma unroll
                    for (int c = 0; c < 3; ++c) fa[(ks + 1) & 1][c].q = hq[(c * 32 + 4 * (ks + 1)) * 16];
                }
                if (ks == 6) { check(); if (!have) issue(); }
                __builtin_amdgcn_sched_barrier(0);
                const bf16x8_t a0 = fa[ks & 1][0].v, a1 = fa[ks & 1][1].v, a2 = fa[ks & 1][2].v;
                acc[0] = __builtin_amdgcn_mfma_f32_16x16x32_bf16(a0, wg[ks * 3 + 0], acc[0], 0, 0, 0);
                acc[1] = __builtin_amdgcn_mfma_f32_16x16x32_bf16(a0, wg[ks * 3 + 1], acc[1], 0, 0, 0);
                acc[1] = __builtin_amdgcn_mfma_f32_16x16x32_bf16(a1, wg[ks * 3 + 0], acc[1], 0, 0, 0);
                acc[2] = __builtin_amdgcn_mfma_f32_16x16x32_bf16(a0, wg[ks * 3 + 2], acc[2], 0, 0, 0);
                acc[2] = __builtin_amdgcn_mfma_f32_16x16x32_bf16(a1, wg[ks * 3 + 1], acc[2], 0, 0, 0);
                acc[2] = __builtin_amdgcn_mfma_f32_16x16x32_bf16(a2, wg[ks * 3 + 0], acc[2], 0, 0, 0);
            }
            if (!have) check();
        }
        I2L_STAMP16(0);
        bool bail = false;
        if (!have) {
            long long t_start = 0;
            unsigned spins = 0;
            for (;;) {
                issue();
                check();
                if (have) break;
                __builtin_amdgcn_s_sleep(1);
                if ((++spins & 255u) == 0) {
                    const long long now = (long long)wall_clock64();
                    if (t_start == 0) t_start = now;
                    else if (now - t_start > p.opts.limit_step) { bail = true; break; }
                }
            }
            if (bail) cnt_s[2] = 1;
        }
        if (t > 0 && !bail) {
            bool all_fin = true;
#pragma unroll
            for (int r = 0; r < G16Q; ++r) {
                const bool was_fin = (fin >> r) & 1u;
                if (r == m && tid == 0 && ids_row) ids_row[t - 1] = (p.stop == I2L_STOP_STICKY && was_fin) ? -1 : tk[r];
                if (tk[r] == p.end_id) fin |= 1u << r;
                all_fin = all_fin && ((fin >> r) & 1u);
            }
            if (t == T || (p.stop == I2L_STOP_STICKY && all_fin)) break;
        }
        I2L_STAMP16(1);
        const unsigned epoch = ((unsigned)t + 1u) & 0xFFFFu;
        const int par = t & 1;
        u64_t* slot = xg + (size_t)par * G16Q * G16GRAN;
        unsigned short* hcur = hp + (size_t)par * 3 * G16_HP_PIECE;
        if (!bail) {
            const bool b0 = lq & 1, b1 = lq & 2;
            float z[4];
#pragma unroll
            for (int i = 0; i < 4; ++i) z[i] = (acc[2][i] + acc[1][i]) + acc[0][i];
            const float r0 = dpp_f<DPP_XOR1>(b0 ? z[0] : z[1]), r1 = dpp_f<DPP_XOR1>(b0 ? z[2] : z[3]);
            const float e0 = b0 ? r0 : z[0], e1 = b0 ? z[1] : r0, e2 = b0 ? r1 : z[2], e3 = b0 ? z[3] : r1;
            const float s0 = dpp_f<DPP_XOR2>(b1 ? e0 : e2), s1 = dpp_f<DPP_XOR2>(b1 ? e1 : e3);
            const float gi = b1 ? s0 : e0, gf = b1 ? s1 : e1, gc = b1 ? e2 : s0, go = b1 ? e3 : s1;
            const float xi = (gi + genc.x) + pvec.x, xf = (gf + genc.y) + pvec.y;
            const float xc = (gc + genc.z) + pvec.z, xo = (go + genc.w) + pvec.w;
            const float ig = sigmoidf_(xi), fg = sigmoidf_(xf), gg = tanhf_(xc), og = sigmoidf_(xo);
            c_own = fg * c_own + ig * gg;
            h_own = og * tanhf_(c_own);
            unsigned short q0, q1, q2;
            split3(h_own, q0, q1, q2);
            const int ul = 4 * wave + uq;
            const u64_t gran = ((u64_t)epoch << 48) | ((u64_t)q0 << 32) | ((u64_t)q1 << 16) | (u64_t)q2;
            store_granule(slot + (size_t)m * G16GRAN + ((ul >> 3) * 16 + cell_row) * 8 + (ul & 7), gran, local);
            const int o = ((2 * m + (ul >> 3)) * 16 + cell_row) * 8 + (ul & 7);
            hcur[o] = q0;
            hcur[G16_HP_PIECE + o] = q1;
            hcur[2 * G16_HP_PIECE + o] = q2;
        }
        I2L_STAMP16(2);
        if (!bail) {
            const int ta = tid, tb = tid + G16NT < 15 * 32 ? tid + G16NT : tid;
            const int qa_ = ta >> 5, qa = qa_ + (qa_ >= m ? 1 : 0), qb_ = tb >> 5, qb = qb_ + (qb_ >= m ? 1 : 0);
            const u64_t* sa = slot + (size_t)qa * G16GRAN + (((ta >> 4) & 1) * 16 + (ta & 15)) * 8;
            const u64_t* sb = slot + (size_t)qb * G16GRAN + (((tb >> 4) & 1) * 16 + (tb & 15)) * 8;
            u32x4_t g[8];
            long long t_start = 0;
            unsigned spins = 0;
            for (;;) {
                load_run64x2(sa, sb, g);
                bool ok = true;
#pragma unroll
                for (int i = 0; i < 8; ++i) ok = ok && (g[i].y >> 16) == epoch && (g[i].w >> 16) == epoch;
                if (ok) break;
                __builtin_amdgcn_s_sleep(1);
                if ((++spins & 255u) == 0) {
                    const long long now = (long long)wall_clock64();
                    if (t_start == 0) t_start = now;
                    else if (now - t_start > p.opts.limit_step) { cnt_s[2] = 1; break; }
                }
            }
            unpack_run(g, reinterpret_cast<u32x4_t*>(hcur) + (2 * qa + ((ta >> 4) & 1)) * 16 + (ta & 15));
            unpack_run(g + 4, reinterpret_cast<u32x4_t*>(hcur) + (2 * qb + ((tb >> 4) & 1)) * 16 + (tb & 15));
        }
        I2L_STAMP16(3);
        __syncthreads();
        if (cnt_s[2] != 0) { failed = true; break; }
        I2L_STAMP16(4);

        {
            f32x4_t la[3] = {f32x4_t{0.f, 0.f, 0.f, 0.f}, f32x4_t{0.f, 0.f, 0.f, 0.f}, f32x4_t{0.f, 0.f, 0.f, 0.f}};
            const u32x4_t* hq = reinterpret_cast<const u32x4_t*>(hcur) + lhi * 16 + lcol;
            Frag16 fa[4][3];
#pragma unroll
            for (int ks = 0; ks < 4; ++ks)
#pragma unroll
                for (int c = 0; c < 3; ++c) fa[ks][c].q = hq[(c * 32 + 4 * (4 * lhalf + ks)) * 16];
#pragma unroll
            for (int ks = 0; ks < 4; ++ks) {
                const bf16x8_t a0 = fa[ks][0].v, a1 = fa[ks][1].v, a2 = fa[ks][2].v;
                la[0] = __builtin_amdgcn_mfma_f32_16x16x32_bf16(a0, wl[ks * 3 + 0], la[0], 0, 0, 0);
                la[1] = __builtin_amdgcn_mfma_f32_16x16x32_bf16(a0, wl[ks * 3 + 1], la[1], 0, 0, 0);
                la[1] = __builtin_amdgcn_mfma_f32_16x16x32_bf16(a1, wl[ks * 3 + 0], la[1], 0, 0, 0);
                la[2] = __builtin_amdgcn_mfma_f32_16x16x32_bf16(a0, wl[ks * 3 + 2], la[2], 0, 0, 0);
                la[2] = __builtin_amdgcn_mfma_f32_16x16x32_bf16(a1, wl[ks * 3 + 1], la[2], 0, 0, 0);
                la[2] = __builtin_amdgcn_mfma_f32_16x16x32_bf16(a2, wl[ks * 3 + 0], la[2], 0, 0, 0);
            }
            f32x4_t part;
#pragma unroll
            for (int i = 0; i < 4; ++i) part[i] = (la[2][i] + la[1][i]) + la[0][i];
            if (lhalf == 1) {
                lpart[ltile * 64 + lane] = part;
                if (lane == 0) __hip_atomic_store(cnt_s + 4 + ltile, (int)epoch, __ATOMIC_RELEASE, __HIP_MEMORY_SCOPE_WORKGROUP);
                I2L_STAMP16(5);
            } else {
                while (__hip_atomic_load(cnt_s + 4 + ltile, __ATOMIC_ACQUIRE, __HIP_MEMORY_SCOPE_WORKGROUP) != (int)epoch)
                    __builtin_amdgcn_s_sleep(0);
                const f32x4_t other = lpart[ltile * 64 + lane];
                I2L_STAMP16(5);
                const int l_v = 32 * m + 16 * ltile + lcol;
#pragma unroll
                for (int i = 0; i < 4; ++i) {
                    float lv = (part[i] + other[i]) + l_bias;
                    if (p.use_temp) lv = lv / p.temperature;
                    unsigned vk = __float_as_uint(lv + 0.0f);
                    vk ^= (vk >> 31) ? 0xFFFFFFFFu : 0x80000000u;
                    unsigned mx = vk;
                    mx = max(mx, (unsigned)__builtin_amdgcn_mov_dpp((int)mx, DPP_ROR8, 0xF, 0xF, true));
                    mx = max(mx, (unsigned)__builtin_amdgcn_mov_dpp((int)mx, DPP_ROR4, 0xF, 0xF, true));
                    mx = max(mx, (unsigned)__builtin_amdgcn_mov_dpp((int)mx, DPP_XOR2, 0xF, 0xF, true));
                    mx = max(mx, (unsigned)__builtin_amdgcn_mov_dpp((int)mx, DPP_XOR1, 0xF, 0xF, true));
                    const unsigned long long hit = __ballot(vk == mx);
                    const int first = __ffs((unsigned)(hit >> (16 * lhi)) & 0xFFFFu) - 1;
                    const u64_t key = ((u64_t)mx << 32) | (u64_t)(0xFFFFFFFFu - (unsigned)(l_v - lcol + first));
                    if (lcol == 0) atomicMax(reinterpret_cast<unsigned long long*>(redk + par * 16 + 4 * lhi + i), (unsigned long long)key);
                }
                int arrived = 0;
                if (lane == 0) arrived = atomicAdd(cnt_s + par, 1);
                arrived = __builtin_amdgcn_readfirstlane(arrived);
                if (arrived == 1) {
                    if (lane < 16) {
                        const u64_t best = redk[par * 16 + lane];
                        store_granule(slot + (size_t)m * G16GRAN + G16GRAN_C + lane,
                                      granule((epoch << 16) | (unsigned)(am_idx(best) & 0xFFFF), am_val(best)), local);
                        redk[(par ^ 1) * 16 + lane] = 0;
                    }
                    if (lane == 0) cnt_s[par ^ 1] = 0;
                }
                I2L_STAMP16(6);
            }
        }
    }
#ifdef I2L_GROUP_STAMPS
    if (lane == 0 && (wave & 1) == 0 && blockIdx.x < 16)
// ... 11 lines not shown
```

hmer-img2latex_amd/img2latex_amd/_lib.py:

```python
from __future__ import annotations

import ctypes
import os
from ctypes import POINTER, c_char_p, c_double, c_float, c_int, c_int32, c_size_t, c_uint64, c_void_p
from typing import Optional, Sequence

import torch

_HERE = os.path.dirname(os.path.abspath(__file__))
LIB_PATH = os.path.join(_HERE, "libimg2latex_hip.so")

OK = 0
ERR_ARG, ERR_UNSUPPORTED, ERR_WORKSPACE, ERR_LAUNCH = -1, -2, -3, -4
STOP_NONE, STOP_STICKY = 0, 1
SELECT_LOGITS, SELECT_SOFTMAX, SELECT_SAMPLE = 0, 1, 2
PREP_WEIGHTS, PREP_ROWS, PREP_ALL = 1, 2, 3
MAX_LSTM_LAYERS, MAX_BEAM = 4, 8
FLAG_EXACT_FP32, FLAG_NO_GROUP, FLAG_RESNET_NO_RING, FLAG_RESNET_IM2COL_STEM = 0x1, 0x2, 0x4, 0x8
FLAG_WEIGHTS_PACKED = 0x10
FLAG_AGENT_SCOPE_EXCHANGE = 0x20
FLAG_CONV_NO_SPARSE_WGRAD = 0x4000
FLAG_CONV_COL_READY = 0x10000
FLAG_DECODE_REGION_CLEARED = 0x2000000
FLAG_RESNET_WIDE_TILES = 0x40000
FLAG_RESNET_NO_PATCH = 0x20000
FLAG_DECODE_GROUP16 = 0x8000
FLAG_DECODE_GROUP8 = 0x1000
FLAG_DECODE_BATCHED = 0x2000
FLAG_BEAM_BATCHED = 0x80000
FLAG_TRAIN_BATCHED = 0x100000
FLAG_TEST_SHORT_TIMEOUT, FLAG_TEST_DROP_MEMBER = 0x40, 0x80


def flag_resnet_ring_depth(n: int) -> int:
    return (int(n) & 0xF) << 8


def flag_resnet_patch_shape(n: int) -> int:
    return (int(n) & 0xF) << 20


class DecoderWeights(ctypes.Structure):
    _fields_ = [("embedding", c_void_p), ("w_ih", POINTER(c_void_p)), ("w_hh", POINTER(c_void_p)),
                ("b_ih", POINTER(c_void_p)), ("b_hh", POINTER(c_void_p)), ("w_out", c_void_p),
                ("b_out", c_void_p), ("vocab", c_int), ("embed", c_int), ("hidden", c_int), ("layers", c_int)]


class DecoderGrads(ctypes.Structure):
    _fields_ = [("embedding", c_void_p), ("w_ih", POINTER(c_void_p)), ("w_hh", POINTER(c_void_p)),
                ("b_ih", POINTER(c_void_p)), ("b_hh", POINTER(c_void_p)), ("w_out", c_void_p), ("b_out", c_void_p)]


_SIGNATURES = {
    "i2l_version": (c_int, []),
    "i2l_error_string": (c_char_p, [c_int]),
    "i2l_lanes_create": (c_int, [POINTER(c_void_p), c_int, POINTER(c_void_p)]),
    "i2l_lanes_destroy": (c_int, [c_void_p]),
    "i2l_lanes_join": (c_int, [c_void_p, c_void_p]),
    "i2l_stream_wait_value32": (c_int, [c_void_p, ctypes.c_uint32, ctypes.c_float, c_void_p]),
    "i2l_conv_workspace_bytes": (c_size_t, [c_int, c_int]),
    "i2l_conv3x3_relu_pool2_fwd": (c_int, [c_void_p, c_void_p, c_void_p, c_void_p, c_void_p, c_int, c_int, c_int,
                                           c_int, c_int, c_void_p, c_size_t, c_int, c_void_p]),
    "i2l_conv_bwd_workspace_bytes": (c_size_t, [c_int, c_int, c_int, c_int, c_int]),
    "i2l_conv3x3_relu_pool2_bwd": (c_int, [c_void_p, c_void_p, c_void_p, c_void_p, c_void_p, c_void_p, c_void_p,
                                           c_void_p, c_int, c_int, c_int, c_int, c_int, c_void_p, c_size_t, c_int,
                                           c_void_p, c_void_p]),
    "i2l_linear_bwd_workspace_bytes": (c_size_t, [c_int, c_int, c_int]),
    "i2l_linear_bias_act_bwd": (c_int, [c_void_p, c_void_p, c_void_p, c_void_p, c_void_p, c_void_p, c_void_p, c_int,
                                        c_int, c_int, c_int, c_void_p, c_size_t, c_int, c_void_p, c_void_p]),
    "i2l_linear_workspace_bytes": (c_size_t, [c_int, c_int, c_int]),
    "i2l_linear_bias_act_fwd": (c_int, [c_void_p, c_void_p, c_void_p, c_void_p, c_int, c_int, c_int, c_int,
                                        c_void_p, c_size_t, c_int, c_void_p]),
    "i2l_conv_bf16_packed_bytes": (c_size_t, [c_int] * 4),
    "i2l_conv_bn_bf16_pack": (c_int, [c_void_p, c_void_p, c_void_p, c_void_p, c_void_p, c_float, c_void_p, c_size_t,
                                      c_int, c_int, c_int, c_int, c_void_p]),
    "i2l_conv_bf16_workspace_bytes": (c_size_t, [c_int] * 10),
    "i2l_conv_bn_act_bf16_fwd": (c_int, [c_void_p, c_int, c_void_p, c_void_p, c_void_p] + [c_int] * 10 +
                                 [c_void_p, c_size_t, c_int, c_void_p]),
    "i2l_bottleneck_join_bf16_fwd": (c_int, [c_void_p, c_void_p, c_void_p, c_void_p, c_void_p, c_void_p, ctypes.c_long,
                                             c_int, c_int, c_int, c_void_p]),
    "i2l_maxpool3x3s2_bf16_fwd": (c_int, [c_void_p, c_void_p, c_int, c_int, c_int, c_int, c_void_p]),
    "i2l_global_avgpool_bf16_fwd": (c_int, [c_void_p, c_void_p, c_int, c_int, c_int, c_int, c_void_p]),
    "i2l_decoder_workspace_bytes": (c_size_t, [c_int, c_int, c_int, c_int, c_int]),
    "i2l_decoder_prepare": (c_int, [POINTER(DecoderWeights), c_void_p, c_int, c_int, c_void_p, c_size_t, c_void_p]),
    "i2l_greedy_decode": (c_int, [POINTER(DecoderWeights), c_void_p, c_int, c_int, c_void_p, c_void_p, c_void_p,
                                  c_void_p, c_float, c_int, c_int, c_int, c_void_p, c_void_p, c_void_p, c_void_p,
                                  c_void_p]),
    "i2l_greedy_decode_ex": (c_int, [POINTER(DecoderWeights), c_void_p, c_int, c_int, c_void_p, c_void_p, c_void_p,
                                     c_void_p, c_float, c_int, c_int, c_int, c_int, c_void_p, c_void_p, c_void_p,
                                     c_void_p, c_int, c_void_p, ctypes.c_uint32, c_void_p]),
    "i2l_decode_batched_scratch_bytes": (c_size_t, [c_int, c_int, c_int, c_int]),
    "i2l_greedy_decode_batched": (c_int, [POINTER(DecoderWeights), c_void_p, c_int, c_int, c_void_p, c_void_p, c_void_p,
                                          c_void_p, c_float, c_int, c_int, c_int, c_void_p, c_void_p, c_void_p, c_void_p,
                                          c_void_p, c_size_t, c_int, c_void_p, ctypes.c_uint32, c_void_p]),
    "i2l_sample_decode": (c_int, [POINTER(DecoderWeights), c_void_p, c_int, c_int, c_void_p, c_void_p, c_void_p, c_float,
                                  c_int, c_float, c_uint64, c_int, c_int, c_void_p, c_void_p, c_void_p, c_void_p,
                                  c_void_p]),
    "i2l_beam_workspace_bytes": (c_size_t, [c_int, c_int, c_int, c_int, c_int]),
    "i2l_beam_decode": (c_int, [POINTER(DecoderWeights), c_void_p, c_int, c_int, c_int, c_int, c_int, c_void_p,
                                c_size_t, c_void_p, c_void_p, c_void_p, c_int, c_void_p]),
    "i2l_beam_batched_scratch_bytes": (c_size_t, [c_int] * 6),
    "i2l_beam_decode_batched": (c_int, [POINTER(DecoderWeights), c_void_p, c_int, c_int, c_int, c_int, c_int, c_void_p,
                                        c_size_t, c_void_p, c_void_p, c_void_p, c_int, c_void_p]),
    "i2l_attention_context_fwd": (c_int, [c_void_p, c_void_p, c_void_p, c_void_p, c_void_p, c_void_p, c_int, c_int,
                                          c_int, c_int, c_void_p]),
    "i2l_decoder_train_workspace_bytes": (c_size_t, [c_int, c_int, c_int, c_int, c_int, c_int]),
    "i2l_decoder_train_batched_ok": (c_int, [c_int, c_int, c_int, c_int]),
    "i2l_decoder_train_fwd": (c_int, [POINTER(DecoderWeights), c_void_p, c_void_p, c_int, c_int, c_float, c_uint64,
                                      c_int, c_void_p, c_size_t, c_void_p, c_int, c_void_p]),
    "i2l_decoder_train_bwd": (c_int, [POINTER(DecoderWeights), c_void_p, c_int, c_int, c_float, c_uint64, c_int,
                                      c_void_p, c_size_t, c_void_p, POINTER(DecoderGrads), c_void_p, c_int, c_void_p,
                                      c_void_p]),
    "i2l_optimizer_workspace_bytes": (c_size_t, []),
    "i2l_grad_clip_adam_step": (c_int, [c_void_p, c_void_p, c_void_p, c_void_p, c_size_t, c_void_p, c_float, c_float,
                                        c_float, c_float, c_float, c_float, c_int, c_void_p, c_size_t, c_void_p,
                                        c_void_p]),
    "i2l_ce_workspace_bytes": (c_size_t, [c_int]),
    "i2l_ce_label_smooth_fwd_bwd": (c_int, [c_void_p, c_void_p, c_int, c_int, c_int, c_float, c_void_p, c_size_t,
                                            c_void_p, c_void_p, c_void_p]),
}

_SIGNATURES.update({
    "i2l_sequence_metrics": (c_int, [c_void_p, c_void_p, c_int, c_void_p, c_void_p, c_int, c_int, c_int, c_int, c_int,
                                     c_void_p, c_void_p, c_void_p, c_void_p]),
    "i2l_compact_ids": (c_int, [c_void_p, c_int, c_int, c_int, c_int, c_void_p, c_int, c_void_p, c_int, c_void_p, c_void_p]),
    "i2l_detokenize_workspace_bytes": (c_size_t, [c_int]),
    "i2l_detokenize": (c_int, [c_void_p, c_int, c_int, c_int, c_int, c_void_p, c_int, c_void_p, c_void_p, c_int, c_int,
                               c_void_p, ctypes.c_int64, c_void_p, c_void_p, c_void_p, c_size_t, c_void_p]),
    "i2l_tokenize_table_bytes": (c_size_t, [c_int, ctypes.c_int64]),
    "i2l_tokenize_table_build": (c_int, [c_void_p, c_void_p, c_void_p, c_int, c_void_p, c_size_t]),
    "i2l_tokenize": (c_int, [c_void_p, ctypes.c_int64, c_void_p, c_int, c_void_p, c_size_t] + [c_int] * 6 +
                     [c_void_p, c_int, c_void_p, c_void_p, c_void_p, c_void_p]),
    "i2l_tokenize_packed_workspace_bytes": (c_size_t, [c_int]),
    "i2l_tokenize_packed": (c_int, [c_void_p, ctypes.c_int64, c_void_p, c_int, c_void_p, c_size_t] + [c_int] * 4 +
                            [c_void_p, ctypes.c_int64, c_void_p, c_void_p, c_void_p, c_size_t, c_void_p]),
    "i2l_collate_ids": (c_int, [c_void_p, ctypes.c_int64, c_void_p, ctypes.c_int64, c_void_p, c_int, c_int, c_int,
                                c_void_p, c_int, c_void_p, c_void_p]),
    "i2l_gather_ragged_u8": (c_int, [c_void_p, ctypes.c_int64, c_void_p, c_void_p, c_int, ctypes.c_int64, c_void_p,
                                     ctypes.c_int64, c_void_p, c_void_p, c_void_p]),
    "i2l_png_decode_workspace_bytes": (c_size_t, [c_int, ctypes.c_int64]),
    "i2l_png_decode": (c_int, [c_void_p, ctypes.c_int64, c_void_p, c_int, c_void_p, ctypes.c_int64, c_void_p, c_void_p,
                               c_size_t, c_void_p]),
    "i2l_vocab_fit_workspace_bytes": (c_size_t, [c_int, ctypes.c_int64]),
    "i2l_vocab_fit": (c_int, [c_void_p, ctypes.c_int64, c_void_p, c_int, c_void_p, c_void_p, c_int, ctypes.c_int64, c_int,
                      c_void_p, ctypes.c_int64, c_void_p, c_void_p, c_void_p, c_int, c_void_p, c_void_p, c_size_t,
                      c_void_p]),
    "i2l_masked_accuracy": (c_int, [c_void_p, c_void_p, ctypes.c_int64, c_int, ctypes.c_int64, c_void_p, c_void_p]),
    "i2l_lanczos_ksize": (c_int, [c_int, c_int]),
    "i2l_lanczos_coeffs": (c_int, [c_int, c_int, c_void_p, c_void_p]),
    "i2l_preprocess_images": (c_int, [c_void_p, c_void_p, c_void_p, c_int, c_int, c_int, c_int, c_int, c_int, c_void_p,
                                      c_void_p, c_void_p]),
    "i2l_bn_train_workspace_bytes": (c_size_t, [ctypes.c_int64, c_int]),
    "i2l_bn_train_fwd_f32": (c_int, [c_void_p, c_void_p, c_void_p, c_void_p, c_void_p, c_void_p, c_float, c_float, c_int,
                                     c_void_p, c_void_p, c_void_p, ctypes.c_int64, c_int, c_void_p, c_size_t, c_void_p]),
    "i2l_bn_train_bwd_f32": (c_int, [c_void_p, c_void_p, c_void_p, c_void_p, c_void_p, c_void_p, c_void_p, c_void_p,
                                     c_void_p, c_void_p, c_int, ctypes.c_int64, c_int, c_void_p, c_size_t, c_void_p]),
    "i2l_conv_f32_workspace_bytes": (c_size_t, [c_int] * 11),
    "i2l_conv_f32_fwd": (c_int, [c_void_p, c_int, c_void_p, c_void_p] + [c_int] * 9 + [c_void_p, c_size_t, c_int, c_void_p]),
    "i2l_conv_f32_bwd": (c_int, [c_void_p, c_int, c_void_p, c_void_p, c_void_p, c_void_p] + [c_int] * 9 +
                         [c_void_p, c_size_t, c_int, c_void_p]),
    "i2l_bn_eval_fold_f32": (c_int, [c_void_p, c_void_p, c_void_p, c_void_p, c_float, c_void_p, c_void_p, c_int, c_void_p]),
    "i2l_conv_bn_act_f32_fwd": (c_int, [c_void_p, c_int, c_void_p, c_void_p, c_void_p, c_void_p, c_void_p] + [c_int] * 10 +
                                [c_void_p, c_size_t, c_int, c_void_p]),
    "i2l_im2col_f32": (c_int, [c_void_p, c_int, c_int, c_int, c_int, c_int, c_int, c_int, c_int, c_int, c_void_p, c_void_p]),
    "i2l_col2im_f32": (c_int, [c_void_p, c_int, c_int, c_int, c_int, c_int, c_int, c_int, c_int, c_void_p, c_int, c_void_p]),
    "i2l_maxpool3x3s2_f32_fwd": (c_int, [c_void_p, c_void_p, c_int, c_int, c_int, c_int, c_void_p]),
    "i2l_maxpool3x3s2_f32_bwd": (c_int, [c_void_p, c_void_p, c_void_p, c_int, c_int, c_int, c_int, c_void_p]),
    "i2l_global_avgpool_f32_fwd": (c_int, [c_void_p, c_void_p, c_int, c_int, c_int, c_int, c_void_p]),
    "i2l_global_avgpool_bwd_f32": (c_int, [c_void_p, c_void_p, c_int, c_int, c_int, c_int, c_void_p]),
    "i2l_decoder_group_status_offset": (c_size_t, [c_int, c_int, c_int, c_int, c_int]),
    "i2l_decoder_group_region_bytes": (c_size_t, [c_int] * 5),
    "i2l_resample_ksize": (c_int, [c_int, c_int, c_int]),
    "i2l_resample_coeffs": (c_int, [c_int, c_int, c_int, c_void_p, c_void_p]),
    "i2l_resample_coeffs_batch": (c_int, [c_int, c_int, c_void_p, c_void_p, c_void_p, c_void_p, c_int]),
    "i2l_scores_from_statistics": (c_int, [c_void_p, c_int, c_int, c_int, POINTER(c_double), POINTER(c_double)]),
    "i2l_resample_coeffs_device": (c_int, [c_int, c_int, c_void_p, c_void_p, c_void_p, c_void_p, c_int, c_void_p]),
    "i2l_pack_host": (c_int, [c_void_p, c_void_p, c_void_p, c_int, c_void_p, c_int]),
    "i2l_resize_bilinear_f32": (c_int, [c_void_p, c_void_p, ctypes.c_int64, c_int, c_int, c_int, c_int, c_void_p]),
    "i2l_teacher_forced_eval_workspace_bytes": (c_size_t, [c_int, c_int]),
    "i2l_teacher_forced_eval": (c_int, [c_void_p, c_void_p, c_int, c_int, c_int, c_int, c_float, c_void_p, c_size_t,
                                        c_void_p, c_void_p, c_void_p, c_void_p, c_void_p, c_void_p]),
    "i2l_affine_nearest_u8": (c_int, [c_void_p, c_void_p, c_void_p, c_void_p, c_int, c_int, ctypes.c_int64, c_void_p]),
    "i2l_affine_nearest_f32": (c_int, [c_void_p, c_void_p, c_void_p, c_void_p, c_int, c_int, c_int, c_int, c_void_p]),
})
FILTER_LANCZOS, FILTER_BICUBIC = 1, 3
EXPORTED_SYMBOLS = tuple(_SIGNATURES)
_LIB: Optional[ctypes.CDLL] = None


def lib() -> ctypes.CDLL:
    global _LIB
    if _LIB is None:
        if not os.path.exists(LIB_PATH):
            raise RuntimeError(
                f"img2latex_amd: HIP extension {LIB_PATH} is missing -- build it with "
                "`make -C hmer-img2latex_amd/csrc` (or __graft_entry__.build()); there is no CPU fallback")
        handle = ctypes.CDLL(LIB_PATH)
        for name, (res, args) in _SIGNATURES.items():
            fn = getattr(handle, name)
            fn.restype = res
            fn.argtypes = args
        _LIB = handle
    return _LIB


def check(rc: int, what: str) -> None:
    if rc != OK:
        raise RuntimeError(f"img2latex_amd: {what} failed: {lib().i2l_error_string(rc).decode()} (code {rc})")


def ids_timed_out(ids_host: torch.Tensor) -> bool:
    first = ids_host[:, 0] if ids_host.dim() == 2 else ids_host
    return bool(first.numel()) and bool((first == -3).any())


def check_ids(ids_host: torch.Tensor) -> torch.Tensor:
    if ids_timed_out(ids_host):
        raise RuntimeError("img2latex_amd: grouped decode timed out waiting for a peer workgroup "
                           "(GPU oversubscribed?); pass rows_per_workgroup=1 to use the row-per-workgroup kernel")
    return ids_host


def stream_ptr() -> int:
    return torch.cuda.current_stream().cuda_stream


def require_gpu(t: torch.Tensor, name: str, dtype=torch.float32) -> torch.Tensor:
    if not isinstance(t, torch.Tensor):
        raise TypeError(f"{name} must be a torch.Tensor")
    if not t.is_cuda:
        raise RuntimeError(f"img2latex_amd: {name} is on {t.device}; the HIP path needs a ROCm device "
                           "tensor and there is no CPU fallback")
    if t.dtype != dtype:
        raise TypeError(f"{name} must be {dtype}, got {t.dtype}")
    return t if t.is_contiguous() else t.contiguous()


def ptr(t: Optional[torch.Tensor]) -> Optional[int]:
    return None if t is None else t.data_ptr()


class Lanes:

    def __init__(self, device, n: int = 2):
        self.streams = [torch.cuda.Stream(device=device) for _ in range(n)]
        arr = (c_void_p * n)(*[s.cuda_stream for s in self.streams])
        out = c_void_p()
        with torch.cuda.device(device):
            check(lib().i2l_lanes_create(arr, n, ctypes.byref(out)), "lanes_create")
        self.handle = out.value

    def join(self) -> None:
        check(lib().i2l_lanes_join(self.handle, stream_ptr()), "lanes_join")

    def close(self) -> None:
        if getattr(self, "handle", None):
            lib().i2l_lanes_destroy(self.handle)
            self.handle = None

    def __del__(self):
        try:
            self.close()
        except Exception:
            pass


def pointer_array(tensors: Sequence[torch.Tensor]):
    arr = (c_void_p * len(tensors))()
    for i, t in enumerate(tensors):
        arr[i] = t.data_ptr()
    return arr


_STAGE_HOOK = None


def set_stage_hook(fn):
    global _STAGE_HOOK
    old, _STAGE_HOOK = _STAGE_HOOK, fn
    return old


def mark(name: str) -> None:
    if _STAGE_HOOK is not None:
        _STAGE_HOOK(name)
```

hmer-img2latex_amd/img2latex_amd/model/lstm_decoder.py:

```python
from __future__ import annotations

import ctypes
from typing import Optional, Tuple

import torch
import torch.nn as nn

from .. import _lib

Hidden = Tuple[torch.Tensor, torch.Tensor]


class Attention(nn.Module):

    def __init__(self, hidden_dim: int, encoder_dim: int):
        super().__init__()
        self.hidden_dim, self.encoder_dim = hidden_dim, encoder_dim
        self.attn = nn.Linear(hidden_dim + encoder_dim, hidden_dim)
        self.v = nn.Linear(hidden_dim, 1, bias=False)

    def forward(self, hidden: torch.Tensor, encoder_outputs: torch.Tensor) -> torch.Tensor:
        hidden = _lib.require_gpu(hidden, "hidden")
        enc = _lib.require_gpu(encoder_outputs, "encoder_outputs")
        B, S, E = enc.shape
        if hidden.shape != (B, 1, self.hidden_dim) or E != self.encoder_dim:
            raise RuntimeError(f"Attention: bad shapes hidden {tuple(hidden.shape)} enc {tuple(enc.shape)}")
        ctx = torch.empty((B, 1, E), dtype=torch.float32, device=enc.device)
        _lib.check(_lib.lib().i2l_attention_context_fwd(
            hidden.data_ptr(), enc.data_ptr(), self.attn.weight.detach().contiguous().data_ptr(),
            self.attn.bias.detach().data_ptr(), self.v.weight.detach().contiguous().data_ptr(), ctx.data_ptr(),
            B, S, self.hidden_dim, E, _lib.stream_ptr()), "attention_context_fwd")
        return ctx


class LSTMDecoder(nn.Module):

    def __init__(self, vocab_size: int, embedding_dim: int = None, hidden_dim: int = None,
                 max_seq_length: int = None, lstm_layers: int = None, dropout: float = None,
                 attention: bool = True):
        super().__init__()
        embedding_dim = 256 if embedding_dim is None else embedding_dim
        hidden_dim = 256 if hidden_dim is None else hidden_dim
        max_seq_length = 141 if max_seq_length is None else max_seq_length
        lstm_layers = 1 if lstm_layers is None else lstm_layers
        dropout = 0.1 if dropout is None else dropout
        self.vocab_size, self.embedding_dim, self.hidden_dim = vocab_size, embedding_dim, hidden_dim
        self.max_seq_length, self.lstm_layers, self.dropout = max_seq_length, lstm_layers, dropout
        self.use_attention = attention
        self.embedding = nn.Embedding(vocab_size, embedding_dim)
        self.lstm = nn.LSTM(input_size=2 * embedding_dim, hidden_size=hidden_dim, num_layers=lstm_layers,
                            batch_first=True, dropout=dropout if lstm_layers > 1 else 0)
        if attention:
            self.attention = Attention(hidden_dim, embedding_dim)
        self.output_layer = nn.Linear(hidden_dim, vocab_size)
        self.dropout_layer = nn.Dropout(dropout)
        self._ws: Optional[torch.Tensor] = None
        self._ws_key = None
        self._ws_by_stream = {}
        self.kernel_flags = 0

    def _weights_struct(self):
        L = self.lstm_layers
        names = ("weight_ih", "weight_hh", "bias_ih", "bias_hh")
        tens = {n: [_lib.require_gpu(getattr(self.lstm, f"{n}_l{l}").detach(), f"lstm.{n}_l{l}") for l in range(L)]
                for n in names}
        emb = _lib.require_gpu(self.embedding.weight.detach(), "embedding.weight")
        wout = _lib.require_gpu(self.output_layer.weight.detach(), "output_layer.weight")
        bout = _lib.require_gpu(self.output_layer.bias.detach(), "output_layer.bias")
        arrs = {n: _lib.pointer_array(tens[n]) for n in names}
        w = _lib.DecoderWeights()
        w.embedding = emb.data_ptr()
        w.w_ih, w.w_hh = arrs["weight_ih"], arrs["weight_hh"]
        w.b_ih, w.b_hh = arrs["bias_ih"], arrs["bias_hh"]
        w.w_out, w.b_out = wout.data_ptr(), bout.data_ptr()
        w.vocab, w.embed, w.hidden, w.layers = self.vocab_size, self.embedding_dim, self.hidden_dim, L
        return w, (tens, emb, wout, bout, arrs)

    def _weights_version(self):
        return tuple((p.data_ptr(), p._version) for p in self.parameters())

    def prepare(self, encoder_output: torch.Tensor, reuse_weight_images: bool = True, slot=None):
        enc = _lib.require_gpu(encoder_output, "encoder_output")
        if enc.dim() != 2 or enc.shape[1] != self.embedding_dim:
            raise RuntimeError(f"encoder_output must be (B,{self.embedding_dim}), got {tuple(enc.shape)}")
        rows = enc.shape[0]
        L = _lib.lib()
        w, keep = self._weights_struct()
        nbytes = L.i2l_decoder_workspace_bytes(rows, self.vocab_size, self.embedding_dim, self.hidden_dim,
                                               self.lstm_layers)
        if nbytes == 0:
            raise RuntimeError("img2latex_amd: decoder dimensions not supported by the HIP kernels")
        key = (rows, enc.device, self._weights_version())
        what = _lib.PREP_ALL
        sid = _lib.stream_ptr() if slot is None else ("slot", slot)
        self._ws, self._ws_key = self._ws_by_stream.get(sid, (None, None))
        if self._ws is None or self._ws.numel() < nbytes or self._ws.device != enc.device:
            self._ws = torch.empty(nbytes, dtype=torch.uint8, device=enc.device)
            self._ws_key = None
        if reuse_weight_images and self._ws_key == key:
            what = _lib.PREP_ROWS
        _lib.check(L.i2l_decoder_prepare(ctypes.byref(w), enc.data_ptr(), rows, what, self._ws.data_ptr(),
                                         self._ws.numel(), _lib.stream_ptr()), "decoder_prepare")
        self._ws_key = key
        self._ws_by_stream[sid] = (self._ws, key)
        _lib.mark("prepare")
        return w, keep, enc

    def release_slots(self, owner) -> None:
        for sid in [k for k in self._ws_by_stream
                    if isinstance(k, tuple) and k[0] == "slot" and isinstance(k[1], tuple) and len(k[1]) > 1 and k[1][1] == owner]:
            ws, _ = self._ws_by_stream.pop(sid)
            if self._ws is ws:
                self._ws, self._ws_key = None, None

    def group_status(self):
        if self._ws is None or self._ws_key is None:
            return None
        off = _lib.lib().i2l_decoder_group_status_offset(self._ws_key[0], self.vocab_size, self.embedding_dim,
                                                         self.hidden_dim, self.lstm_layers)
        if off == 0:
            return None
        st = self._ws[off:off + 16].view(torch.int32).cpu().tolist()
        return {"timed_out": bool(st[0]), "groups": st[1], "groups_on_one_xcd": st[2]}

    def run_steps(self, encoder_output: torch.Tensor, steps: int, tok0: torch.Tensor,
                  forced: Optional[torch.Tensor] = None, hidden: Optional[Hidden] = None,
                  temperature: float = 1.0, select: int = _lib.SELECT_LOGITS, stop: int = _lib.STOP_NONE,
                  end_id: int = -1, want_ids: bool = True, want_logits: bool = False,
                  want_state: bool = False, reuse_weight_images: bool = True, rows_per_workgroup: int = 0,
                  flags: int = 0, prepared=None, resident=None):
        if prepared is None:
            w, keep, enc = self.prepare(encoder_output, reuse_weight_images)
            ws = self._ws
        else:
            w, keep, enc, ws = prepared
        rows, dev = enc.shape[0], enc.device
        tok0 = _lib.require_gpu(tok0, "tok0", torch.int32)
        if forced is not None:
            forced = _lib.require_gpu(forced, "forced", torch.int32)
            if forced.shape != (rows, steps):
                raise RuntimeError(f"forced tokens must be ({rows},{steps}), got {tuple(forced.shape)}")
        h0 = c0 = None
        if hidden is not None:
            h0 = _lib.require_gpu(hidden[0], "h0")
            c0 = _lib.require_gpu(hidden[1], "c0")
            shp = (self.lstm_layers, rows, self.hidden_dim)
            if tuple(h0.shape) != shp or tuple(c0.shape) != shp:
                raise RuntimeError(f"hidden state must be {shp}, got {tuple(h0.shape)} / {tuple(c0.shape)}")
        ids = torch.empty((rows, steps), dtype=torch.int32, device=dev) if want_ids else None
        logits = torch.empty((rows, steps, self.vocab_size), dtype=torch.float32, device=dev) if want_logits else None
        h = c = None
        if want_state:
            h = torch.empty((self.lstm_layers, rows, self.hidden_dim), dtype=torch.float32, device=dev)
            c = torch.empty_like(h)
        all_flags = int(flags) | int(self.kernel_flags)
        res_ptr = None if resident is None else resident[0].data_ptr()
        res_val = 0 if resident is None else int(resident[1]) & 0xFFFFFFFF
        if all_flags & _lib.FLAG_DECODE_BATCHED:
            nbytes = _lib.lib().i2l_decode_batched_scratch_bytes(rows, self.vocab_size, self.hidden_dim, self.lstm_layers)
            if nbytes == 0:
                raise RuntimeError("img2latex_amd: decoder dimensions not supported by the step-batched decode")
            scratch = torch.empty(nbytes, dtype=torch.uint8, device=dev)
            _lib.check(_lib.lib().i2l_greedy_decode_batched(
                ctypes.byref(w), ws.data_ptr(), rows, steps, tok0.data_ptr(), _lib.ptr(forced), _lib.ptr(h0),
                _lib.ptr(c0), float(temperature), select, stop, int(end_id), _lib.ptr(ids), _lib.ptr(logits),
                _lib.ptr(h), _lib.ptr(c), scratch.data_ptr(), nbytes, all_flags, res_ptr, res_val, _lib.stream_ptr()),
                "greedy_decode_batched")
            _lib.mark("decode")
            del keep, scratch
            return ids, logits, ((h, c) if want_state else None)
        _lib.check(_lib.lib().i2l_greedy_decode_ex(
            ctypes.byref(w), ws.data_ptr(), rows, steps, tok0.data_ptr(), _lib.ptr(forced), _lib.ptr(h0),
            _lib.ptr(c0), float(temperature), select, stop, int(end_id), int(rows_per_workgroup), _lib.ptr(ids),
            _lib.ptr(logits), _lib.ptr(h), _lib.ptr(c), int(flags) | int(self.kernel_flags),
            None if resident is None else resident[0].data_ptr(), 0 if resident is None else int(resident[1]) & 0xFFFFFFFF,
            _lib.stream_ptr()), "greedy_decode")
        _lib.mark("decode")
        del keep
        return ids, logits, ((h, c) if want_state else None)

    def sample_steps(self, encoder_output: torch.Tensor, steps: int, tok0: torch.Tensor, temperature: float,
                     top_k: int, top_p: float, seed: int, stop: int = _lib.STOP_STICKY, end_id: int = -1,
                     hidden: Optional[Hidden] = None, want_probs: bool = False):
        w, keep, enc = self.prepare(encoder_output)
        rows, dev = enc.shape[0], enc.device
        tok0 = _lib.require_gpu(tok0, "tok0", torch.int32)
        h0 = c0 = None
        if hidden is not None:
            h0, c0 = _lib.require_gpu(hidden[0], "h0"), _lib.require_gpu(hidden[1], "c0")
        ids = torch.empty((rows, steps), dtype=torch.int32, device=dev)
        probs = torch.empty((rows, steps, self.vocab_size), dtype=torch.float32, device=dev) if want_probs else None
        _lib.check(_lib.lib().i2l_sample_decode(
            ctypes.byref(w), self._ws.data_ptr(), rows, steps, tok0.data_ptr(), _lib.ptr(h0), _lib.ptr(c0),
            float(temperature), int(top_k), float(top_p), int(seed) & 0xFFFFFFFFFFFFFFFF, stop, int(end_id),
            ids.data_ptr(), _lib.ptr(probs), None, None, _lib.stream_ptr()), "sample_decode")
        del keep
        return ids, probs

    def forward(self, encoder_output: torch.Tensor, target_sequence: torch.Tensor, hidden=None) -> torch.Tensor:
        tgt = target_sequence
        if not tgt.is_cuda:
            raise RuntimeError("img2latex_amd: target_sequence must be on the ROCm device (no CPU fallback)")
        B, T = tgt.shape
        forced = tgt.to(torch.int32).contiguous()
        needs_grad = torch.is_grad_enabled() and (encoder_output.requires_grad
                                                  or any(p.requires_grad for p in self.parameters()))
        if needs_grad or (self.training and self.dropout > 0):
            if hidden is not None:
                raise NotImplementedError("img2latex_amd: training forward starts from a zero state (as the Trainer does)")
            from ._train_fn import DecoderTeacherForcedFn
            seed = int(torch.randint(0, 2 ** 62, (1,)).item())
            return DecoderTeacherForcedFn.apply(self, encoder_output, forced, seed, *self.parameters())
        _, logits, _ = self.run_steps(encoder_output, T, forced[:, 0].contiguous(), forced=forced, hidden=hidden,
                                      want_ids=False, want_logits=True)
        return logits

    def decode_step(self, encoder_output: torch.Tensor, input_token: torch.Tensor, hidden=None
                    ) -> Tuple[torch.Tensor, Hidden]:
        if input_token.dim() != 2 or input_token.shape[1] != 1:
            raise RuntimeError(f"Shape mismatch: input_token must be (B,1), got {tuple(input_token.shape)}")
        if not input_token.is_cuda:
            raise RuntimeError("img2latex_amd: input_token must be on the ROCm device (no CPU fallback)")
        tok0 = input_token.reshape(-1).to(torch.int32).contiguous()
        _, logits, state = self.run_steps(encoder_output, 1, tok0, hidden=hidden, want_ids=False,
                                          want_logits=True, want_state=True, reuse_weight_images=True)
        return logits, state
```

hmer-img2latex_amd/img2latex_amd/pipeline.py:

```python
from __future__ import annotations

from collections import deque
from typing import Deque, List, Optional, Tuple

import torch

from . import _lib


class GreedyPipeline:

    def __init__(self, model, start_token_id: int, end_token_id: int, max_length: int = 150,
                 temperature: float = 1.0, depth: int = 3, rows_per_workgroup: int = 2, decode_streams: int = 1,
                 decode_flags: int = 0, encoder_flags: int = 0, decode_priority: int = 0, encoder_streams: int = 1,
                 encoder_priority: int = 0, hold_encoder: Optional[bool] = None, wait_timeout_us: float = 20000.0,
                 clear_early: bool = True,
                 stop: int = _lib.STOP_NONE, select: int = _lib.SELECT_LOGITS, detokenize=None):
        self.model = model
        self.start, self.end, self.max_length, self.temperature = start_token_id, end_token_id, max_length, temperature
        dev = next(model.parameters()).device
        if dev.type != "cuda":
            raise RuntimeError("img2latex_amd: GreedyPipeline needs the model on a ROCm device (no CPU fallback)")
        self.device = dev
        self.enc_streams = [torch.cuda.Stream(device=dev, priority=int(encoder_priority)) for _ in range(max(1, encoder_streams))]
        self._next_enc = 0
        self.dec_streams = [torch.cuda.Stream(device=dev, priority=int(decode_priority)) for _ in range(max(1, decode_streams))]
        self._next_dec = 0
        self.depth = max(depth, len(self.dec_streams) + len(self.enc_streams))
        self.rows_per_workgroup = rows_per_workgroup
        self.decode_flags = int(decode_flags)
        self.stop, self.select = int(stop), int(select)
        self.encoder_flags = int(encoder_flags)
        if len(self.enc_streams) >= 2:
            self.encoder_flags |= getattr(model.encoder, "MULTI_STREAM_FLAGS", 0)
        if hold_encoder is None:
            hold_encoder = bool(self.decode_flags & (_lib.FLAG_DECODE_GROUP8 | _lib.FLAG_DECODE_GROUP16))
        self.hold_encoder = bool(hold_encoder)
        self.clear_early = bool(clear_early)
        self.wait_timeout_us = float(wait_timeout_us)
        self._resident = torch.zeros(1, dtype=torch.int32, device=dev)
        self.trace: Optional[list] = None
        self.trace_every = 1
        self._inflight: Deque[Tuple[torch.cuda.Event, torch.Tensor, torch.Tensor]] = deque()
        self.copy_stream = torch.cuda.Stream(device=dev)
        self._batch_no = 0
        self._slots = self.depth + 1
        self._free: List[torch.Tensor] = []
        self._lent: Optional[torch.Tensor] = None
        self.detok = detokenize
        self._text_dev: dict = {}
        self._text_free: List[Tuple[torch.Tensor, torch.Tensor]] = []

    def submit(self, images: torch.Tensor) -> None:
        if len(self._inflight) >= self.depth:
            raise RuntimeError(f"GreedyPipeline: {self.depth} batches already in flight; collect() first")
        cur = torch.cuda.current_stream(self.device)
        enc_stream = self.enc_streams[self._next_enc]
        self._next_enc = (self._next_enc + 1) % len(self.enc_streams)
        enc_stream.wait_stream(cur)
        with torch.no_grad():
            with torch.cuda.stream(enc_stream):
                if self.hold_encoder and self._batch_no >= len(self.enc_streams):
                    _lib.check(_lib.lib().i2l_stream_wait_value32(
                        self._resident.data_ptr(), self._batch_no - len(self.enc_streams) + 1, self.wait_timeout_us,
                        _lib.stream_ptr()), "stream_wait_value32")
                rec = None
                if self.trace is not None and self._batch_no % self.trace_every < 2:
                    rec = {k: torch.cuda.Event(enable_timing=True) for k in ("enc_start", "enc_end", "dec_start", "dec_end")}
                    rec["batch"] = self._batch_no
                    rec["enc_start"].record(enc_stream)
                    self.trace.append(rec)
                saved = self.model.encoder.kernel_flags
                self.model.encoder.kernel_flags = saved | self.encoder_flags
                try:
                    enc = self.model.encoder(images)
                finally:
                    self.model.encoder.kernel_flags = saved
                slot = self._batch_no % self._slots
                seq = self._batch_no + 1
                self._batch_no += 1
                dec = self.model.decoder
                w, keep, enc_c = dec.prepare(enc, slot=("pipe", id(self), slot))
                prepared = (w, keep, enc_c, dec._ws)
                dflags = self.decode_flags
                if self.clear_early and dflags & (_lib.FLAG_DECODE_GROUP8 | _lib.FLAG_DECODE_GROUP16):
                    dims = (enc.shape[0], dec.vocab_size, dec.embedding_dim, dec.hidden_dim, dec.lstm_layers)
                    off = _lib.lib().i2l_decoder_group_status_offset(*dims)
                    nb = _lib.lib().i2l_decoder_group_region_bytes(*dims)
                    if off and nb:
                        dec._ws[off:off + nb].zero_()
                        dflags |= _lib.FLAG_DECODE_REGION_CLEARED
                enc_done = torch.cuda.Event() if rec is None else rec["enc_end"]
                enc_done.record(enc_stream)
            images.record_stream(enc_stream)
            dec_stream = self.dec_streams[self._next_dec]
            self._next_dec = (self._next_dec + 1) % len(self.dec_streams)
            with torch.cuda.stream(dec_stream):
                dec_stream.wait_event(enc_done)
                enc.record_stream(dec_stream)
                if rec is not None:
                    rec["dec_start"].record(dec_stream)
                ids, _ = self.model.greedy_ids(enc, self.start, self.end, self.max_length, self.temperature,
                                               stop=self.stop, select=self.select,
                                               rows_per_workgroup=self.rows_per_workgroup, flags=dflags,
                                               prepared=prepared,
                                               resident=(self._resident, seq) if self.hold_encoder else None)
                if rec is not None:
                    rec["dec_end"].record(dec_stream)
                host = self._host_buffer(ids.shape)
                text = dev_text = None
                if self.detok is not None:
                    key = (slot, tuple(ids.shape))
                    if key not in self._text_dev:
                        self._text_dev = {k: v for k, v in self._text_dev.items() if k[0] != slot}
                        self._text_dev[key] = self.detok.buffers(*ids.shape)
                    dev_text = self.detok.launch(ids, self.end, self._text_dev[key])
                    text = self._text_buffer(dev_text)
                if self.copy_stream is None:
                    host.copy_(ids, non_blocking=True)
                    if text is not None:
                        text[0].copy_(dev_text[0], non_blocking=True)
                        text[1].copy_(dev_text[1], non_blocking=True)
                    done = torch.cuda.Event()
                    done.record(dec_stream)
                else:
                    decoded = torch.cuda.Event()
                    decoded.record(dec_stream)
                    self.copy_stream.wait_event(decoded)
                    with torch.cuda.stream(self.copy_stream):
                        host.copy_(ids, non_blocking=True)
                        if text is not None:
                            text[0].copy_(dev_text[0], non_blocking=True)
                            text[1].copy_(dev_text[1], non_blocking=True)
                        done = torch.cuda.Event()
                        done.record(self.copy_stream)
                    ids.record_stream(self.copy_stream)
        self._inflight.append((done, host, enc, text))

    def close(self) -> None:
        inflight = getattr(self, "_inflight", None)
        if inflight:
            inflight.clear()
            for s in self.enc_streams + self.dec_streams + [self.copy_stream]:
                if s is not None:
                    s.synchronize()
        self._text_dev = {}
        dec = getattr(getattr(self, "model", None), "decoder", None)
        if dec is not None and hasattr(dec, "release_slots"):
            dec.release_slots(id(self))

    def __del__(self):
        try:
            self.close()
        except Exception:
            pass

    def _host_buffer(self, shape) -> torch.Tensor:
        for i, t in enumerate(self._free):
            if t.shape == shape:
                return self._free.pop(i)
        return torch.empty(shape, dtype=torch.int32).pin_memory()

    def _text_buffer(self, dev_text) -> Tuple[torch.Tensor, torch.Tensor]:
        shapes = (dev_text[0].shape, dev_text[1].shape)
        for i, t in enumerate(self._text_free):
            if (t[0].shape, t[1].shape) == shapes:
                return self._text_free.pop(i)
        return (torch.empty(shapes[0], dtype=torch.uint8).pin_memory(), torch.empty(shapes[1], dtype=torch.int32).pin_memory())

    def pending(self) -> int:
        return len(self._inflight)

    def collect(self) -> Optional[torch.Tensor]:
        entry = self._collect()
        if entry is None:
            return None
        if entry[1] is not None:
            self._text_free.append(entry[1])
        return entry[0]

    def collect_strings(self) -> Optional[List[str]]:
        if self.detok is None:
            raise RuntimeError("GreedyPipeline: collect_strings() needs detokenize=<DetokenizeTable>")
        entry = self._collect()
        if entry is None:
            return None
        text = entry[1]
        try:
            return self.detok.strings(*text)
        finally:
            self._text_free.append(text)

    def _collect(self):
        if not self._inflight:
            return None
        done, host, enc, text = self._inflight.popleft()
        done.synchronize()
        if _lib.ids_timed_out(host):
            import warnings
            warnings.warn("img2latex_amd: grouped decode timed out inside the pipeline; re-running the batch on the "
                          "row-per-workgroup kernel", RuntimeWarning)
            with torch.no_grad():
                ids, _ = self.model.greedy_ids(enc, self.start, self.end, self.max_length, self.temperature,
                                               stop=self.stop, select=self.select, rows_per_workgroup=1)
            host.copy_(ids)
            if text is not None:
                dev_text = self.detok.launch(ids, self.end)
                text[0].copy_(dev_text[0])
                text[1].copy_(dev_text[1])
        if self._lent is not None:
            self._free.append(self._lent)
        self._lent = host
        return _lib.check_ids(host), text

    def drain(self) -> List[torch.Tensor]:
        out = []
        while self._inflight:
            out.append(self.collect().clone())
        return out

    def to_sequences(self, ids_host: torch.Tensor):
        all_end = (ids_host == self.end).all(dim=0)
        steps = int(all_end.nonzero()[0]) + 1 if bool(all_end.any()) else ids_host.shape[1]
        return [[self.start] + r for r in ids_host[:, :steps].tolist()]
```

include/img2latex_hip.h:

```cpp
#ifndef IMG2LATEX_HIP_H
#define IMG2LATEX_HIP_H

#include <stddef.h>
#include <stdint.h>

#ifdef __cplusplus
extern "C" {
#endif

#define I2L_OK 0
#define I2L_ERR_ARG (-1)
#define I2L_ERR_UNSUPPORTED (-2)
#define I2L_ERR_WORKSPACE (-3)
#define I2L_ERR_LAUNCH (-4)

#define I2L_MAX_LSTM_LAYERS 4
#define I2L_MAX_BEAM 8

typedef void* i2l_stream_t;

#define I2L_FLAG_EXACT_FP32 0x1
#define I2L_FLAG_NO_GROUP 0x2
#define I2L_FLAG_RESNET_NO_RING 0x4
#define I2L_FLAG_RESNET_IM2COL_STEM 0x8
#define I2L_FLAG_WEIGHTS_PACKED 0x10
#define I2L_FLAG_AGENT_SCOPE_EXCHANGE 0x20
#define I2L_FLAG_TEST_SHORT_TIMEOUT 0x40
#define I2L_FLAG_TEST_DROP_MEMBER 0x80
#define I2L_FLAG_DECODE_GROUP8 0x1000
#define I2L_FLAG_DECODE_BATCHED 0x2000
#define I2L_FLAG_BEAM_BATCHED 0x80000
#define I2L_FLAG_TRAIN_BATCHED 0x100000
#define I2L_FLAG_DECODE_GROUP16 0x8000
#define I2L_FLAG_CONV_COL_READY 0x10000
#define I2L_FLAG_RESNET_WIDE_TILES 0x40000
#define I2L_FLAG_RESNET_NO_PATCH 0x20000
#define I2L_FLAG_DECODE_REGION_CLEARED 0x2000000
#define I2L_FLAG_CONV_NO_SPARSE_WGRAD 0x4000
#define I2L_FLAG_RESNET_RING_DEPTH(n) (((n) & 0xF) << 8)
#define I2L_FLAG_RESNET_PATCH_SHAPE(n) (((n) & 0xF) << 20)

int i2l_version(void);
const char* i2l_error_string(int code);
#define I2L_MAX_LANES 4
typedef struct i2l_lanes i2l_lanes;
int i2l_lanes_create(const i2l_stream_t* streams, int n, i2l_lanes** out);
int i2l_lanes_destroy(i2l_lanes* lanes);
int i2l_lanes_join(i2l_lanes* lanes, i2l_stream_t stream);
int i2l_stream_wait_value32(const uint32_t* flag, uint32_t value, float timeout_us, i2l_stream_t stream);


size_t i2l_conv_workspace_bytes(int Cin, int Cout);
int i2l_conv3x3_relu_pool2_fwd(const float* x, const float* w, const float* bias, float* y,
                               uint8_t* argmax_out, int B, int Cin, int H, int W, int Cout, void* workspace,
                               size_t workspace_bytes, int flags, i2l_stream_t stream);

size_t i2l_conv_bwd_workspace_bytes(int B, int Cin, int H, int W, int Cout);
int i2l_conv3x3_relu_pool2_bwd(const float* x, const float* w, const float* y, const uint8_t* argmax,
                               const float* dy, float* dx, float* dw, float* db, int B, int Cin, int H,
                               int W, int Cout, void* workspace, size_t workspace_bytes, int flags,
                               i2l_lanes* lanes, i2l_stream_t stream);

size_t i2l_linear_workspace_bytes(int M, int K, int N);
int i2l_linear_bias_act_fwd(const float* x, const float* w, const float* bias, float* y,
                            int M, int K, int N, int relu, void* workspace, size_t workspace_bytes,
                            int flags, i2l_stream_t stream);
size_t i2l_linear_bwd_workspace_bytes(int M, int K, int N);
int i2l_linear_bias_act_bwd(const float* x, const float* w, const float* y, const float* dy, float* dx,
                            float* dw, float* db, int M, int K, int N, int relu, void* workspace,
                            size_t workspace_bytes, int flags, i2l_lanes* lanes, i2l_stream_t stream);

size_t i2l_conv_bf16_packed_bytes(int Cout, int Cin, int kh, int kw);
int i2l_conv_bn_bf16_pack(const float* w, const float* bn_weight, const float* bn_bias, const float* bn_mean,
                          const float* bn_var, float bn_eps, void* packed, size_t packed_bytes, int Cout,
                          int Cin, int kh, int kw, i2l_stream_t stream);
size_t i2l_conv_bf16_workspace_bytes(int B, int H, int W, int Cin, int Cout, int kh, int kw, int stride, int pad,
                                     int flags);
int i2l_conv_bn_act_bf16_fwd(const void* x, int x_is_nchw_f32, const void* packed, const void* residual,
                             void* y, int B, int H, int W, int Cin, int Cout, int kh, int kw, int stride,
                             int pad, int relu, void* workspace, size_t workspace_bytes, int flags,
                             i2l_stream_t stream);
int i2l_bottleneck_join_bf16_fwd(const void* o2, const void* packed3, const void* identity, void* y, const void* packed1_next,
                                 void* z, long positions, int c_mid, int c_out, int n2, i2l_stream_t stream);
int i2l_maxpool3x3s2_bf16_fwd(const void* x, void* y, int B, int H, int W, int C, i2l_stream_t stream);
int i2l_global_avgpool_bf16_fwd(const void* x, float* y, int B, int H, int W, int C, i2l_stream_t stream);

size_t i2l_conv_f32_workspace_bytes(int x_kind, int B, int H, int W, int Cin, int Cout, int kh, int kw, int stride,
                                    int pad, int backward_dx);
int i2l_conv_f32_fwd(const float* x, int x_kind, const float* w, float* z, int B, int H, int W, int Cin, int Cout,
                     int kh, int kw, int stride, int pad, void* workspace, size_t workspace_bytes, int flags,
                     i2l_stream_t stream);
int i2l_conv_f32_bwd(const float* x, int x_kind, const float* w, const float* dz, float* dx, float* dw, int B, int H,
                     int W, int Cin, int Cout, int kh, int kw, int stride, int pad, void* workspace,
                     size_t workspace_bytes, int flags, i2l_stream_t stream);
size_t i2l_bn_train_workspace_bytes(int64_t M, int C);
int i2l_bn_train_fwd_f32(const float* z, const float* residual, const float* gamma, const float* beta,
                         float* running_mean, float* running_var, float momentum, float eps, int relu, float* y,
                         float* save_mean, float* save_invstd, int64_t M, int C, void* workspace,
                         size_t workspace_bytes, i2l_stream_t stream);
int i2l_bn_train_bwd_f32(const float* dy, const float* y_relu, const float* z, const float* gamma, const float* save_mean,
                         const float* save_invstd, float* dz, float* dgamma, float* dbeta, float* dres,
                         int dres_accumulate, int64_t M, int C, void* workspace, size_t workspace_bytes,
                         i2l_stream_t stream);
int i2l_bn_eval_fold_f32(const float* gamma, const float* beta, const float* running_mean, const float* running_var,
                         float eps, float* scale_out, float* shift_out, int C, i2l_stream_t stream);
int i2l_conv_bn_act_f32_fwd(const float* x, int x_kind, const float* w, const float* scale, const float* shift,
                            const float* residual, float* y, int B, int H, int W, int Cin, int Cout, int kh, int kw,
                            int stride, int pad, int relu, void* workspace, size_t workspace_bytes, int flags,
                            i2l_stream_t stream);
int i2l_im2col_f32(const void* x, int x_kind, int B, int H, int W, int C, int kh, int kw, int stride, int pad,
                   float* col, i2l_stream_t stream);
int i2l_col2im_f32(const float* dcol, int B, int H, int W, int C, int kh, int kw, int stride, int pad, float* dx,
                   int accumulate, i2l_stream_t stream);
int i2l_maxpool3x3s2_f32_fwd(const float* x, float* y, int B, int H, int W, int C, i2l_stream_t stream);
int i2l_maxpool3x3s2_f32_bwd(const float* x, const float* dy, float* dx, int B, int H, int W, int C, i2l_stream_t stream);
int i2l_global_avgpool_f32_fwd(const float* x, float* y, int B, int H, int W, int C, i2l_stream_t stream);
int i2l_global_avgpool_bwd_f32(const float* dfeat, float* dx, int B, int H, int W, int C, i2l_stream_t stream);


typedef struct i2l_decoder_weights {
    const float* embedding;
    const float* const* w_ih;
    const float* const* w_hh;
    const float* const* b_ih;
    const float* const* b_hh;
    const float* w_out;
    const float* b_out;
    int vocab, embed, hidden, layers;
} i2l_decoder_weights;

size_t i2l_decoder_workspace_bytes(int rows, int vocab, int embed, int hidden, int layers);

#define I2L_PREP_WEIGHTS 1
#define I2L_PREP_ROWS 2
#define I2L_PREP_ALL 3
int i2l_decoder_prepare(const i2l_decoder_weights* w, const float* enc, int rows, int what,
                        void* workspace, size_t workspace_bytes, i2l_stream_t stream);

#define I2L_STOP_NONE 0
#define I2L_STOP_STICKY 1

#define I2L_SELECT_LOGITS 0
#define I2L_SELECT_SOFTMAX 1
#define I2L_SELECT_SAMPLE 2

int i2l_greedy_decode(const i2l_decoder_weights* w, const void* workspace, int rows, int steps,
                      const int32_t* tok0, const int32_t* forced, const float* h0, const float* c0,
                      float temperature, int select, int stop, int end_id,
                      int32_t* ids_out, float* logits_out, float* h_out, float* c_out,
                      i2l_stream_t stream);

int i2l_greedy_decode_ex(const i2l_decoder_weights* w, const void* workspace, int rows, int steps,
                         const int32_t* tok0, const int32_t* forced, const float* h0, const float* c0,
                         float temperature, int select, int stop, int end_id, int rows_per_workgroup,
                         int32_t* ids_out, float* logits_out, float* h_out, float* c_out, int flags,
                         uint32_t* resident_flag, uint32_t resident_value, i2l_stream_t stream);

size_t i2l_decode_batched_scratch_bytes(int rows, int vocab, int hidden, int layers);
int i2l_greedy_decode_batched(const i2l_decoder_weights* w, const void* workspace, int rows, int steps,
                              const int32_t* tok0, const int32_t* forced, const float* h0, const float* c0,
                              float temperature, int select, int stop, int end_id, int32_t* ids_out,
                              float* logits_out, float* h_out, float* c_out, void* scratch, size_t scratch_bytes,
                              int flags, uint32_t* resident_flag, uint32_t resident_value, i2l_stream_t stream);

int i2l_sample_decode(const i2l_decoder_weights* w, const void* workspace, int rows, int steps,
                      const int32_t* tok0, const float* h0, const float* c0, float temperature, int top_k,
                      float top_p, uint64_t seed, int stop, int end_id, int32_t* ids_out, float* probs_out,
                      float* h_out, float* c_out, i2l_stream_t stream);

size_t i2l_beam_workspace_bytes(int images, int beam, int hidden, int layers, int steps);
int i2l_beam_decode(const i2l_decoder_weights* w, const void* workspace, int images, int beam,
                    int steps, int start_id, int end_id, void* beam_workspace,
                    size_t beam_workspace_bytes, int32_t* seq_out, int32_t* len_out,
                    double* score_out, int flags, i2l_stream_t stream);

size_t i2l_beam_batched_scratch_bytes(int images, int beam, int vocab, int hidden, int layers, int steps);
int i2l_beam_decode_batched(const i2l_decoder_weights* w, const void* workspace, int images, int beam, int steps,
                            int start_id, int end_id, void* scratch, size_t scratch_bytes, int32_t* seq_out,
                            int32_t* len_out, double* score_out, int flags, i2l_stream_t stream);

int i2l_attention_context_fwd(const float* hidden, const float* enc, const float* w_attn,
                              const float* b_attn, const float* v, float* context,
                              int B, int S, int H, int E, i2l_stream_t stream);


typedef struct i2l_decoder_grads {
    float* embedding;
    float* const* w_ih;
    float* const* w_hh;
    float* const* b_ih;
    float* const* b_hh;
    float* w_out;
    float* b_out;
} i2l_decoder_grads;

size_t i2l_decoder_train_workspace_bytes(int B, int T, int vocab, int embed, int hidden, int layers);
int i2l_decoder_train_batched_ok(int vocab, int embed, int hidden, int layers);
int i2l_decoder_train_fwd(const i2l_decoder_weights* w, const float* enc, const int32_t* tokens, int B, int T,
                          float dropout_p, uint64_t seed, int attention_path, void* workspace,
                          size_t workspace_bytes, float* logits_out, int flags, i2l_stream_t stream);
int i2l_decoder_train_bwd(const i2l_decoder_weights* w, const int32_t* tokens, int B, int T, float dropout_p,
                          uint64_t seed, int attention_path, void* workspace, size_t workspace_bytes,
                          const float* dlogits, const i2l_decoder_grads* grads, float* denc_out,
                          int flags, i2l_lanes* lanes, i2l_stream_t stream);

size_t i2l_ce_workspace_bytes(int rows);
int i2l_ce_label_smooth_fwd_bwd(const float* logits, const int32_t* targets, int rows, int vocab, int pad_id,
                                float label_smoothing, void* workspace, size_t workspace_bytes,
                                float* dlogits_out, float* loss_sum_and_count_out, i2l_stream_t stream);

size_t i2l_optimizer_workspace_bytes(void);
int i2l_grad_clip_adam_step(float* params, const float* grads, float* exp_avg, float* exp_avg_sq, size_t n,
                            const float* count_ptr, float max_norm, float lr, float beta1, float beta2,
                            float eps, float weight_decay, int step, void* workspace, size_t workspace_bytes,
                            float* stats_out, i2l_stream_t stream);


int i2l_sequence_metrics(const int32_t* pred, const int32_t* pred_len, int pred_stride, const int32_t* target,
                         const int32_t* target_len, int target_stride, int pairs, int max_len, int max_n,
                         int pad_id, int32_t* lev_out, int32_t* match_out, int32_t* tla_out, i2l_stream_t stream);

int i2l_scores_from_statistics(const int32_t* stats, int pairs, int stride, int n, double* bleu_mean_out,
                               double* lev_mean_out);

int i2l_compact_ids(const int32_t* ids, int rows, int width, int stride, int end_id, const int32_t* drop_ids,
                    int n_drop, int32_t* out_ids, int out_stride, int32_t* out_len, i2l_stream_t stream);

size_t i2l_detokenize_workspace_bytes(int rows);
int i2l_detokenize(const int32_t* ids, int rows, int width, int stride, int end_id, const int32_t* drop_ids, int n_drop,
                   const uint8_t* tok_bytes, const int32_t* tok_off, int vocab, int unk_id, uint8_t* out_bytes,
                   int64_t out_capacity, int32_t* out_off, int32_t* status, void* workspace, size_t workspace_bytes,
                   i2l_stream_t stream);

size_t i2l_tokenize_table_bytes(int n, int64_t key_bytes);
int i2l_tokenize_table_build(const uint8_t* tok_bytes, const int32_t* tok_off, const int32_t* tok_id, int n, void* image,
                             size_t image_bytes);
int i2l_tokenize(const uint8_t* text, int64_t text_bytes, const int32_t* row_off, int rows, const void* table,
                 size_t table_bytes, int unk_id, int pad_id, int start_id, int end_id, int add_special, int width,
                 int32_t* out_ids, int out_stride, int32_t* out_len, int32_t* out_count, int32_t* status,
                 i2l_stream_t stream);

#define I2L_TOKENIZE_PACKED_OVERFLOW 1
size_t i2l_tokenize_packed_workspace_bytes(int rows);
int i2l_tokenize_packed(const uint8_t* text, int64_t text_bytes, const int32_t* row_off, int rows, const void* table,
                        size_t table_bytes, int unk_id, int start_id, int end_id, int add_special, int32_t* out_ids,
                        int64_t out_capacity, int64_t* out_off, int32_t* status, void* workspace, size_t workspace_bytes,
                        i2l_stream_t stream);

#define I2L_COLLATE_ROW_TOO_LONG 1
#define I2L_COLLATE_BAD_INDEX 2
int i2l_collate_ids(const int32_t* ids, int64_t n_ids, const int64_t* off, int64_t rows, const int64_t* index, int B, int width,
                    int pad_id, int32_t* out, int out_stride, int32_t* status, i2l_stream_t stream);

int i2l_gather_ragged_u8(const uint8_t* src, int64_t src_bytes, const int64_t* src_off, const int64_t* size, int n,
                         int64_t max_size, uint8_t* dst, int64_t dst_bytes, const int64_t* dst_off, int32_t* status,
                         i2l_stream_t stream);

typedef struct i2l_png_image {
    int64_t z_off, z_len;
    int64_t pal_off;
    int64_t out_off;
    int32_t width, height, colour_type;
    int32_t pal_n;
    int32_t channels;
    int32_t reserved;
} i2l_png_image;
#define I2L_PNG_E_HEADER 1
#define I2L_PNG_E_TRUNCATED 2
#define I2L_PNG_E_BLOCK_TYPE 3
#define I2L_PNG_E_STORED_LEN 4
#define I2L_PNG_E_CODE_LENGTHS 5
#define I2L_PNG_E_SYMBOL 6
#define I2L_PNG_E_DISTANCE 7
#define I2L_PNG_E_TOO_MANY 8
#define I2L_PNG_E_TOO_FEW 9
#define I2L_PNG_E_TRAILING 10
#define I2L_PNG_E_ADLER 11
#define I2L_PNG_E_FILTER 12
#define I2L_PNG_E_PALETTE 13
size_t i2l_png_decode_workspace_bytes(int n, int64_t filtered_bytes_total);
int i2l_png_decode(const uint8_t* z, int64_t z_bytes, const i2l_png_image* images, int n, uint8_t* pixels,
                   int64_t pixels_bytes, int32_t* status, void* workspace, size_t workspace_bytes, i2l_stream_t stream);

#define I2L_VOCAB_FIT_META_WORDS 16
#define I2L_VOCAB_FIT_FULL 1
#define I2L_VOCAB_FIT_BAD_OFFSETS 2
#define I2L_VOCAB_FIT_OUT_TOO_SMALL 4
#define I2L_VOCAB_FIT_NO_AGGREGATE 1
size_t i2l_vocab_fit_workspace_bytes(int rows, int64_t slots);
int i2l_vocab_fit(const uint8_t* text, int64_t text_bytes, const int32_t* row_off, int rows, const uint8_t* skip_bytes,
                  const int32_t* skip_off, int n_skip, int64_t slots, int flags, uint8_t* out_bytes,
                  int64_t out_byte_capacity, int32_t* out_off, int32_t* out_count, int32_t* out_first, int out_capacity,
                  int32_t* meta, void* workspace, size_t workspace_bytes, i2l_stream_t stream);

int i2l_masked_accuracy(const float* logits, const int64_t* targets, int64_t rows, int vocab, int64_t pad_id,
                        uint64_t* correct_total_out, i2l_stream_t stream);

size_t i2l_teacher_forced_eval_workspace_bytes(int batch, int steps);
int i2l_teacher_forced_eval(const float* logits, const int32_t* targets, int batch, int steps, int vocab, int pad_id,
                            float label_smoothing, void* workspace, size_t workspace_bytes, int32_t* argmax_out,
                            int32_t* pred_len_out, int32_t* target_len_out, float* loss_sum_count_out,
                            int64_t* correct_total_out, i2l_stream_t stream);

size_t i2l_decoder_group_status_offset(int rows, int vocab, int embed, int hidden, int layers);
size_t i2l_decoder_group_region_bytes(int rows, int vocab, int embed, int hidden, int layers);


int i2l_lanczos_ksize(int in_size, int out_size);
int i2l_lanczos_coeffs(int in_size, int out_size, int32_t* bounds_out, int32_t* kk_out);
#define I2L_FILTER_LANCZOS 1
#define I2L_FILTER_BICUBIC 3
int i2l_resample_ksize(int filter, int in_size, int out_size);
int i2l_resample_coeffs(int filter, int in_size, int out_size, int32_t* bounds_out, int32_t* kk_out);
int i2l_resample_coeffs_batch(int filter, int n, const int32_t* in_sizes, const int32_t* out_sizes,
                              const int64_t* offsets, int32_t* out, int threads);

int i2l_resample_coeffs_device(int filter, int n, const int32_t* in_sizes, const int32_t* out_sizes, const int64_t* offsets,
                               int32_t* tables, int max_out_size, i2l_stream_t stream);
int i2l_pack_host(const void* const* srcs, const int64_t* sizes, const int64_t* offsets, int n, void* dst, int threads);

typedef struct i2l_resize_plan {
    int64_t src_offset;
    int64_t tmp_offset;
    int64_t bh_offset, kh_offset;
    int64_t bv_offset, kv_offset;
    int32_t src_h, src_w, src_c;
    int32_t new_w;
    int32_t ybox_first, tmp_rows;
    int32_t need_h, need_v;
    int32_t kh_ksize, kv_ksize;
} i2l_resize_plan;

int i2l_preprocess_images(const uint8_t* pixels, const i2l_resize_plan* plans, const int32_t* tables, int n,
                          int max_tmp_px, int out_c, int out_h, int out_w, int normalize, void* workspace,
                          float* out, i2l_stream_t stream);

int i2l_resize_bilinear_f32(const float* in, float* out, int64_t planes, int in_h, int in_w, int out_h, int out_w,
                            i2l_stream_t stream);


typedef struct i2l_affine_params {
    int32_t a0, a1, a2, a3, a4, a5;
    int32_t tx, ty;
} i2l_affine_params;

int i2l_affine_nearest_u8(const uint8_t* pixels, uint8_t* out, const i2l_resize_plan* plans,
                          const i2l_affine_params* params, int n, int max_side, int64_t max_page_bytes,
                          i2l_stream_t stream);

int i2l_affine_nearest_f32(const float* x, float* out, const i2l_affine_params* params, const float* fill, int n,
                           int c, int h, int w, i2l_stream_t stream);

#ifdef __cplusplus
}
#endif
#endif
```

Measured before the change: 40.16 million.

## Split greedy decode into halves and co-schedule two batches per group16 launch

The group16 decode kernel is templated on a row-tile count so that one persistent launch can advance two batches at once. Each launch runs the second half of the older batch and the first half of the newer one, saving and restoring LSTM c/h state, tokens and finish masks through a new workspace region. The pipeline is changed to split each batch's decode across consecutive launches, with a tail launch for the last batch. The aim is to amortise the per-step cross-workgroup exchange and sync latency over twice the rows. The cost is state save/restore traffic, more registers and LDS, and more complex pipeline bookkeeping.

```diff
diff --git a/hmer-img2latex_amd/csrc/api.hip b/hmer-img2latex_amd/csrc/api.hip
--- a/hmer-img2latex_amd/csrc/api.hip
+++ b/hmer-img2latex_amd/csrc/api.hip
@@ -1,7 +1,7 @@
 #include "common.h"
 #include <new>
 
-extern "C" int i2l_version(void) { return 107; }
+extern "C" int i2l_version(void) { return 108; }
 
 extern "C" const char* i2l_error_string(int code) {
     switch (code) {
diff --git a/hmer-img2latex_amd/csrc/decode.hip b/hmer-img2latex_amd/csrc/decode.hip
--- a/hmer-img2latex_amd/csrc/decode.hip
+++ b/hmer-img2latex_amd/csrc/decode.hip
@@ -684,7 +684,7 @@
 }
 constexpr GroupVariant group_variant(int i) {
     constexpr GroupVariant table[GROUP_VARIANTS] = {
-        {decode_group16_kernel, I2L_FLAG_DECODE_GROUP16, G16Q, G16NT, GRP16_LDS, GROUP16_XCHG_PER_GROUP},
+        {decode_group16_kernel<1>, I2L_FLAG_DECODE_GROUP16, G16Q, G16NT, GRP16_LDS, GROUP16_XCHG_PER_GROUP},
         grouped_variant<8>(I2L_FLAG_DECODE_GROUP8),
         grouped_variant<4>(0),
     };
@@ -692,7 +692,7 @@
 }
 
 struct Layout {
-    size_t P, Genc, WhhT[MAXL], WihT[MAXL], biasP[MAXL], WoutT, boutP, wpack16, gemm_ws, xchg, xchg_bytes, total;
+    size_t P, Genc, WhhT[MAXL], WihT[MAXL], biasP[MAXL], WoutT, boutP, wpack16, gemm_ws, xchg, xchg_bytes, state, state_bytes, total;
     int Vp;
 };
 
@@ -721,8 +721,13 @@
             const size_t x = group_xchg_bytes(i2l_cdiv(rows, g.rows), g.xchg_per_group);
             most = x > most ? x : most;
         }
+        const size_t x2 = group_xchg_bytes(i2l_cdiv(rows, G16Q), G16Shape<2>::XCHG_PER_GROUP);
+        most = x2 > most ? x2 : most;
         o.xchg_bytes = GROUP_STATUS_BYTES + most;
         off += i2l_align(o.xchg_bytes);
+        o.state = off;
+        o.state_bytes = group16_state_bytes(rows);
+        off += i2l_align(o.state_bytes);
     }
     o.total = off;
     return o;
@@ -959,6 +964,75 @@
     I2L_CHECK_LAUNCH();
     return I2L_OK;
 }
+}
+
+namespace {
+int check_half(const i2l_decode_half* h) {
+    if (!h) return I2L_OK;
+    if (!h->workspace || !h->tok0 || !h->ids_out || h->rows <= 0 || h->steps <= 0) return I2L_ERR_ARG;
+    if (h->first_step < 0 || h->n_steps < 0 || h->first_step > h->steps - h->n_steps) return I2L_ERR_ARG;
+    if (h->steps > 65000) return I2L_ERR_UNSUPPORTED;
+    return I2L_OK;
+}
+}
+
+extern "C" int i2l_greedy_decode_halves(const i2l_decoder_weights* w, const i2l_decode_half* older,
+                                        const i2l_decode_half* newer, float temperature, int select, int stop, int end_id,
+                                        int flags, uint32_t* resident_flag, uint32_t resident_value, i2l_stream_t stream) {
+    int rc = check_weights(w);
+    if (rc != I2L_OK) return rc;
+    if (select != I2L_SELECT_LOGITS && select != I2L_SELECT_SOFTMAX) return I2L_ERR_ARG;
+    if (stop != I2L_STOP_NONE && stop != I2L_STOP_STICKY) return I2L_ERR_ARG;
+    if ((rc = check_half(older)) != I2L_OK || (rc = check_half(newer)) != I2L_OK) return rc;
+    const int V = w->vocab, E = w->embed, H = w->hidden, L = w->layers;
+    if (stop != I2L_STOP_NONE || !group_shape_ok(V, H, L)) return I2L_ERR_UNSUPPORTED;
+    const i2l_decode_half* half[2] = {older && older->n_steps > 0 ? older : nullptr, newer && newer->n_steps > 0 ? newer : nullptr};
+    hipStream_t s = i2l_s(stream);
+    if (!half[0] && !half[1]) {
+        if (resident_flag) {
+            hipLaunchKernelGGL(publish_value32_kernel, dim3(1), dim3(1), 0, s, resident_flag, resident_value);
+            I2L_CHECK_LAUNCH();
+        }
+        return I2L_OK;
+    }
+    const i2l_decode_half* home = half[1] ? half[1] : half[0];
+    const Layout lo = make_layout(home->rows, V, E, H, L);
+    int n_groups = 0, most_steps = 0;
+    for (int k = 0; k < 2; ++k)
+        if (half[k]) {
+            n_groups = std::max(n_groups, i2l_cdiv(half[k]->rows, G16Q));
+            most_steps = std::max(most_steps, half[k]->n_steps);
+        }
+    if (!lo.wpack16 || GROUP_STATUS_BYTES + group_xchg_bytes(n_groups, G16Shape<2>::XCHG_PER_GROUP) > lo.xchg_bytes)
+        return I2L_ERR_UNSUPPORTED;
+    char* base = static_cast<char*>(const_cast<void*>(home->workspace));
+
+    GroupParams gp{};
+    gp.w = step_weights(lo, base, V, H, L);
+    gp.n_groups = n_groups;
+    gp.temperature = temperature; gp.use_temp = (temperature != 1.0f) ? 1 : 0; gp.stop = stop; gp.end_id = end_id;
+    char* xb = base + lo.xchg;
+    gp.status = reinterpret_cast<unsigned*>(xb);
+    gp.xchg = reinterpret_cast<u64_t*>(xb + GROUP_STATUS_BYTES);
+    gp.opts = group_opts(most_steps, flags);
+    gp.resident_flag = resident_flag; gp.resident_value = resident_value;
+    for (int k = 0; k < 2; ++k) {
+        HalfTile& t = gp.tile[k];
+        if (!half[k]) continue;
+        const i2l_decode_half& h = *half[k];
+        const Layout hl = make_layout(h.rows, V, E, H, L);
+        char* hb = static_cast<char*>(const_cast<void*>(h.workspace));
+        t.Genc = reinterpret_cast<const float*>(hb + hl.Genc);
+        t.tok0 = h.tok0; t.ids = h.ids_out; t.B = h.rows; t.T = h.steps; t.t0 = h.first_step; t.n = h.n_steps;
+        t.state_in = h.first_step > 0 ? hb + hl.state : nullptr;
+        t.state_out = h.first_step + h.n_steps < h.steps ? hb + hl.state : nullptr;
+    }
+    static std::atomic<unsigned> attr{};
+    if (!i2l_lds_attr(reinterpret_cast<const void*>(decode_group16_kernel<2>), G16Shape<2>::LDS, attr)) return I2L_ERR_UNSUPPORTED;
+    if (!(flags & I2L_FLAG_DECODE_REGION_CLEARED) && hipMemsetAsync(xb, 0, lo.xchg_bytes, s) != hipSuccess) return I2L_ERR_LAUNCH;
+    hipLaunchKernelGGL(decode_group16_kernel<2>, dim3(group_grid(n_groups, G16Q)), dim3(G16NT), G16Shape<2>::LDS, s, gp);
+    I2L_CHECK_LAUNCH();
+    return I2L_OK;
 }
 
 extern "C" size_t i2l_decode_batched_scratch_bytes(int rows, int vocab, int hidden, int layers) {
@@ -1239,6 +1313,12 @@
 extern "C" size_t i2l_decoder_group_region_bytes(int rows, int vocab, int embed, int hidden, int layers) {
     return make_layout(rows, vocab, embed, hidden, layers).xchg_bytes;
 }
+extern "C" size_t i2l_decoder_group_state_offset(int rows, int vocab, int embed, int hidden, int layers) {
+    return make_layout(rows, vocab, embed, hidden, layers).state;
+}
+extern "C" size_t i2l_decoder_group_state_bytes(int rows, int vocab, int embed, int hidden, int layers) {
+    return make_layout(rows, vocab, embed, hidden, layers).state_bytes;
+}
 
 #ifdef I2L_GROUP_STAMPS
 extern "C" size_t i2l_debug_group_status_offset(int rows, int vocab, int embed, int hidden, int layers) {
diff --git a/hmer-img2latex_amd/csrc/decode_group.inc.h b/hmer-img2latex_amd/csrc/decode_group.inc.h
--- a/hmer-img2latex_amd/csrc/decode_group.inc.h
+++ b/hmer-img2latex_amd/csrc/decode_group.inc.h
@@ -16,6 +16,16 @@
     static constexpr size_t LDS = (size_t)(256 * CPM + 2 * 256 * M + (M == 4 ? 4 * NT : 0)) * sizeof(float) +
                                   (size_t)2 * M * 8 + 8 * sizeof(int);
     static constexpr size_t XCHG_PER_GROUP = (size_t)2 * M * GRAN * 8;
+};
+
+struct HalfTile {
+    const float* Genc;
+    const int32_t* tok0;
+    int32_t* ids;
+    int B, T;
+    int t0, n;
+    const void* state_in;
+    void* state_out;
 };
 
 struct GroupParams {
@@ -32,6 +42,7 @@
     GroupOpts opts;
     unsigned* resident_flag;
     unsigned resident_value;
+    HalfTile tile[2];
 };
 
 constexpr int DPP_SHL12 = 0x10C;
diff --git a/hmer-img2latex_amd/csrc/decode_group16.inc.h b/hmer-img2latex_amd/csrc/decode_group16.inc.h
--- a/hmer-img2latex_amd/csrc/decode_group16.inc.h
+++ b/hmer-img2latex_amd/csrc/decode_group16.inc.h
@@ -2,13 +2,37 @@
 
 constexpr int G16Q = 16;
 constexpr int G16NT = 256;
-constexpr int G16GRAN_H = 256;
-constexpr int G16GRAN_C = G16GRAN_H;
-constexpr int G16GRAN_X = G16GRAN_H + 16;
-constexpr int G16GRAN = G16GRAN_H + 32;
 constexpr int G16_HP_PIECE = 32 * 16 * 8;
-constexpr size_t GRP16_LDS = (size_t)2 * 3 * G16_HP_PIECE * 2 + (size_t)2 * 64 * 16 + (size_t)2 * 16 * 8 + 8 * sizeof(int);
-constexpr size_t GROUP16_XCHG_PER_GROUP = (size_t)2 * G16Q * G16GRAN * 8;
+template <int RT>
+struct G16Shape {
+    static_assert(RT == 1 || RT == 2, "row tiles per group");
+    static constexpr int GRAN_H = 256 * RT;
+    static constexpr int GRAN_C = GRAN_H;
+    static constexpr int GRAN_X = GRAN_H + 16 * RT;
+    static constexpr int GRAN = GRAN_H + 32 * RT;
+    static constexpr size_t LDS = (size_t)2 * 3 * G16_HP_PIECE * 2 + (size_t)2 * 64 * 16 + (size_t)2 * RT * 16 * 8 + 8 * sizeof(int);
+    static constexpr size_t XCHG_PER_GROUP = (size_t)2 * G16Q * GRAN * 8;
+};
+constexpr size_t GRP16_LDS = G16Shape<1>::LDS;
+constexpr size_t GROUP16_XCHG_PER_GROUP = G16Shape<1>::XCHG_PER_GROUP;
+
+__host__ __device__ constexpr size_t group16_state_rows(int rows) { return (size_t)((rows + G16Q - 1) / G16Q) * G16Q; }
+__host__ __device__ constexpr size_t group16_state_bytes(int rows) {
+    return group16_state_rows(rows) * (2 * 256 * sizeof(float) + sizeof(int)) + group16_state_rows(rows) / G16Q * 2 * sizeof(unsigned);
+}
+struct G16State {
+    float* c; float* h; int* tok; unsigned* fin; unsigned* failed;
+};
+__device__ __forceinline__ G16State group16_state(const void* base, int rows) {
+    const size_t rp = group16_state_rows(rows);
+    G16State s;
+    s.c = static_cast<float*>(const_cast<void*>(base));
+    s.h = s.c + rp * 256;
+    s.tok = reinterpret_cast<int*>(s.h + rp * 256);
+    s.fin = reinterpret_cast<unsigned*>(s.tok + rp);
+    s.failed = s.fin + rp / G16Q;
+    return s;
+}
 
 __device__ __forceinline__ void load_run64(const u64_t* src, u32x4_t (&g)[4]) {
     asm volatile(
@@ -58,6 +82,21 @@
         : "v"(s0), "v"(s1)
         : "memory");
 }
+__device__ __forceinline__ void load_run64x2_at(const u64_t* base, unsigned oa, unsigned ob, u32x4_t (&g)[8]) {
+    asm volatile(
+        "global_load_dwordx4 %0, %8, %10 sc1\n\t"
+        "global_load_dwordx4 %1, %8, %10 offset:16 sc1\n\t"
+        "global_load_dwordx4 %2, %8, %10 offset:32 sc1\n\t"
+        "global_load_dwordx4 %3, %8, %10 offset:48 sc1\n\t"
+        "global_load_dwordx4 %4, %9, %10 sc1\n\t"
+        "global_load_dwordx4 %5, %9, %10 offset:16 sc1\n\t"
+        "global_load_dwordx4 %6, %9, %10 offset:32 sc1\n\t"
+        "global_load_dwordx4 %7, %9, %10 offset:48 sc1\n\t"
+        "s_waitcnt vmcnt(0)"
+        : "=&v"(g[0]), "=&v"(g[1]), "=&v"(g[2]), "=&v"(g[3]), "=&v"(g[4]), "=&v"(g[5]), "=&v"(g[6]), "=&v"(g[7])
+        : "v"(oa), "v"(ob), "s"(base)
+        : "memory");
+}
 __device__ __forceinline__ void unpack_run(const u32x4_t* g, u32x4_t* dst) {
     u32x4_t o0, o1, o2;
     o0.x = (g[0].y & 0xFFFFu) | (g[0].w << 16); o0.y = (g[1].y & 0xFFFFu) | (g[1].w << 16);
@@ -71,7 +110,506 @@
     dst[2 * (G16_HP_PIECE / 8)] = o2;
 }
 
+template <int RT>
 __global__ __launch_bounds__(G16NT, 2) void decode_group16_kernel(GroupParams p) {
+    using S = G16Shape<RT>;
+    constexpr int GRAN = S::GRAN, GRAN_C = S::GRAN_C, GRAN_X = S::GRAN_X;
+    extern __shared__ __attribute__((aligned(16))) unsigned char smem16[];
+    unsigned short* hp = reinterpret_cast<unsigned short*>(smem16);
+    f32x4_t* lpart = reinterpret_cast<f32x4_t*>(smem16 + (size_t)2 * 3 * G16_HP_PIECE * 2);
+    u64_t* redk = reinterpret_cast<u64_t*>(lpart + 2 * 64);
+    int* cnt_s = reinterpret_cast<int*>(redk + 2 * RT * 16);
+    const StepWeights& w = p.w;
+    const int tid = threadIdx.x, lane = tid & 63, wave = tid >> 6;
+    const int within = blockIdx.x & 127;
+    const int group = (blockIdx.x >> 7) * 8 + (within & 7), m = within >> 3;
+    if (group >= p.n_groups) return;
+    const int V = w.V;
+    const int row0 = group * G16Q;
+    constexpr int G = 1024;
+    const int lq = lane & 3, uq = (lane >> 2) & 3, lhi = lane >> 4, lcol = lane & 15;
+    const int cell_row = 4 * lhi + lq;
+    const int unit = 16 * m + 4 * wave + uq;
+    const int ltile = wave & 1, lhalf = wave >> 1;
+
+    u64_t* xg = p.xchg + (size_t)group * 2 * G16Q * GRAN;
+    if (tid < 8) cnt_s[tid] = 0;
+    if (wave == 0) {
+        unsigned xcc;
+        asm volatile("s_getreg_b32 %0, hwreg(HW_REG_XCC_ID)" : "=s"(xcc));
+        xcc &= 0xFu;
+        if (lane == 0 && !(p.opts.drop_member && m == 3))
+            store_granule(xg + (size_t)m * GRAN + GRAN_X, granule(0xC0DEu, __uint_as_float(xcc)), false);
+        const int pq = (lane & 15) + ((lane & 15) >= m ? 1 : 0);
+        u64_t pv = 0;
+        bool bad = false;
+        long long t_start = 0;
+        unsigned spins = 0;
+        for (;;) {
+            bool ok = true;
+            if (lane < 15) { pv = load_granule(xg + (size_t)pq * GRAN + GRAN_X); ok = (unsigned)(pv >> 32) == 0xC0DEu; }
+            if (__all(ok)) break;
+            __builtin_amdgcn_s_sleep(1);
+            if ((++spins & 255u) == 0) {
+                const long long now = (long long)wall_clock64();
+                if (t_start == 0) t_start = now;
+                else if (now - t_start > p.opts.limit_first) { bad = true; break; }
+            }
+        }
+        const bool all_same = __all(lane >= 15 || (unsigned)pv == xcc);
+        if (lane == 0) {
+            cnt_s[3] = (all_same && !bad) ? 1 : 0;
+            if (bad) cnt_s[2] = 1;
+            if (m == 0 && !bad) {
+                count_resident_group(p.status, p.n_groups, p.resident_flag, p.resident_value);
+                if (all_same && !p.opts.agent_scope) atomicAdd(p.status + GRP_STAT_LOCAL, 1u);
+            }
+        }
+    }
+    bf16x8_t wg[24], wl[12];
+    {
+        const u32x4_t* pk = static_cast<const u32x4_t*>(w.wpack16) + (size_t)(m * 4 + wave) * 36 * 64 + lane;
+#pragma unroll
+        for (int i = 0; i < 24; ++i) { Frag16 f; f.q = pk[i * 64]; wg[i] = f.v; }
+        if constexpr (RT == 1) {
+#pragma unroll
+            for (int i = 0; i < 12; ++i) { Frag16 f; f.q = pk[(24 + i) * 64]; wl[i] = f.v; }
+        }
+    }
+    HalfTile tl[RT];
+    if constexpr (RT == 1) tl[0] = HalfTile{w.Genc, p.tok0, p.ids, p.B, p.T, 0, p.T, nullptr, nullptr};
+    else { tl[0] = p.tile[0]; tl[1] = p.tile[1]; }
+    int nk[RT];
+    bool mark_failed[RT];
+    float4 genc[RT], pvec[RT];
+    float c_own[RT], h_own[RT];
+    unsigned fin[RT];
+    int mytok[RT];
+    int32_t* ids_row[RT];
+    int n_steps = 0;
+    if constexpr (RT == 1) {
+        for (int idx = tid; idx < 2 * 3 * G16_HP_PIECE / 2; idx += G16NT) reinterpret_cast<unsigned*>(hp)[idx] = 0u;
+    }
+    if (tid < 32 * RT) redk[tid] = 0;
+    const float l_bias = w.boutP[32 * m + 16 * ltile + lcol];
+#pragma unroll
+    for (int k = 0; k < RT; ++k) {
+        const int B = tl[k].B;
+        nk[k] = (RT == 1 || (tl[k].n > 0 && row0 < B)) ? tl[k].n : 0;
+        mark_failed[k] = false;
+        c_own[k] = 0.f; h_own[k] = 0.f;
+        fin[k] = 0;
+#pragma unroll
+        for (int r = 0; r < G16Q; ++r)
+            if (row0 + r >= B) fin[k] |= 1u << r;
+        const bool own_row = row0 + m < B;
+        ids_row[k] = (tl[k].ids && own_row && nk[k] > 0) ? tl[k].ids + (size_t)(row0 + m) * tl[k].T : nullptr;
+        genc[k] = float4{0.f, 0.f, 0.f, 0.f};
+        pvec[k] = genc[k];
+        mytok[k] = 0;
+        if constexpr (RT == 2) {
+            unsigned short* hk = hp + (size_t)k * 3 * G16_HP_PIECE;
+            const bool resume = nk[k] > 0 && tl[k].t0 > 0;
+            if (resume) {
+                const G16State st = group16_state(tl[k].state_in, B);
+                if (st.failed[group] != 0) { nk[k] = 0; mark_failed[k] = true; }
+                else {
+                    c_own[k] = st.c[(size_t)(row0 + cell_row) * 256 + unit];
+                    h_own[k] = st.h[(size_t)(row0 + cell_row) * 256 + unit];
+                    mytok[k] = st.tok[row0 + cell_row];
+                    fin[k] = st.fin[group];
+                    for (int idx = tid; idx < G16Q * 256; idx += G16NT) {
+                        const int r = idx >> 8, u = idx & 255;
+                        unsigned short q0, q1, q2;
+                        split3(st.h[(size_t)(row0 + r) * 256 + u], q0, q1, q2);
+                        const int o = ((u >> 3) * 16 + r) * 8 + (u & 7);
+                        hk[o] = q0;
+                        hk[G16_HP_PIECE + o] = q1;
+                        hk[2 * G16_HP_PIECE + o] = q2;
+                    }
+                }
+            }
+            if (!(resume && !mark_failed[k]))
+                for (int idx = tid; idx < 3 * G16_HP_PIECE / 2; idx += G16NT) reinterpret_cast<unsigned*>(hk)[idx] = 0u;
+            if (nk[k] > 0 && tl[k].state_out && m == 0 && tid == 0)
+                group16_state(tl[k].state_out, B).failed[group] = 0u;
+        }
+        if (RT == 1 || nk[k] > 0)
+            genc[k] = *reinterpret_cast<const float4*>(tl[k].Genc + (size_t)min(row0 + cell_row, B - 1) * G + 4 * unit);
+        n_steps = max(n_steps, nk[k]);
+    }
+
+    __syncthreads();
+    const bool local = cnt_s[3] != 0 && !p.opts.agent_scope;
+
+#pragma unroll
+    for (int k = 0; k < RT; ++k) {
+        if (RT == 1 || nk[k] > 0) {
+            if (RT == 1 || tl[k].t0 == 0) mytok[k] = tl[k].tok0[min(row0 + cell_row, tl[k].B - 1)];
+            mytok[k] = min(max(mytok[k], 0), V - 1);
+            pvec[k] = *reinterpret_cast<const float4*>(w.P + (size_t)mytok[k] * G + 4 * unit);
+        }
+    }
+
+    int t = 0;
+    bool failed = cnt_s[2] != 0;
+#ifdef I2L_GROUP_STAMPS
+    long long st_acc[8] = {0, 0, 0, 0, 0, 0, 0, 0};
+    long long st_last = (long long)wall_clock64();
+#define I2L_STAMP16(i) do { const long long n_ = (long long)wall_clock64(); st_acc[i] += n_ - st_last; st_last = n_; } while (0)
+#else
+#define I2L_STAMP16(i) do { } while (0)
+#endif
+    for (; !failed && (RT == 1 || n_steps > 0); ++t) {
+        f32x4_t acc[RT][3];
+        bool live[RT];
+        bool any_live = false;
+#pragma unroll
+        for (int k = 0; k < RT; ++k) {
+#pragma unroll
+            for (int c = 0; c < 3; ++c) acc[k][c] = f32x4_t{0.f, 0.f, 0.f, 0.f};
+            live[k] = t < nk[k];
+            any_live = any_live || live[k];
+        }
+        const u64_t* cand_src = xg + (size_t)((t - 1) & 1) * G16Q * GRAN + (size_t)(4 * lhi) * GRAN + GRAN_C + lcol;
+        const unsigned c_epoch = (unsigned)t & 0xFFFFu;
+        bool have = t == 0;
+        int tk[16];
+#pragma unroll
+        for (int r = 0; r < 16; ++r) tk[r] = 0;
+        int rowtok[RT];
+#pragma unroll
+        for (int k = 0; k < RT; ++k) rowtok[k] = 0;
+        u64_t gv[RT][4];
+#pragma unroll
+        for (int k = 0; k < RT; ++k)
+#pragma unroll
+            for (int i = 0; i < 4; ++i) gv[k][i] = 0;
+        auto issue = [&]() {
+#pragma unroll
+            for (int k = 0; k < RT; ++k)
+#pragma unroll
+                for (int i = 0; i < 4; ++i) gv[k][i] = load_granule(cand_src + (size_t)i * GRAN + 16 * k);
+        };
+        auto check = [&]() {
+            bool ok = true;
+#pragma unroll
+            for (int k = 0; k < RT; ++k)
+#pragma unroll
+                for (int i = 0; i < 4; ++i) ok = ok && (unsigned)(gv[k][i] >> 48) == c_epoch;
+            if (!__all(ok)) return;
+#pragma unroll
+            for (int k = 0; k < RT; ++k) {
+                u64_t best = 0;
+#pragma unroll
+                for (int i = 0; i < 4; ++i)
+                    best = umax64(best, am_key(__uint_as_float((unsigned)gv[k][i]), (int)((unsigned)(gv[k][i] >> 32) & 0xFFFFu)));
+                best = umax64(best, (u64_t)__shfl_xor((unsigned long long)best, 16));
+                best = umax64(best, (u64_t)__shfl_xor((unsigned long long)best, 32));
+                const int bi = am_idx(best);
+                if constexpr (RT == 1) {
+#pragma unroll
+                    for (int r = 0; r < 16; ++r) {
+                        tk[r] = __builtin_amdgcn_readlane(bi, r);
+                        tk[r] = tk[r] < V ? tk[r] : 0;
+                    }
+                }
+                rowtok[k] = bi < V ? bi : 0;
+                if (live[k]) {
+                    mytok[k] = __shfl(bi, cell_row);
+                    mytok[k] = mytok[k] < V ? mytok[k] : 0;
+                    pvec[k] = *reinterpret_cast<const float4*>(w.P + (size_t)mytok[k] * G + 4 * unit);
+                    if constexpr (RT == 2) genc[k] = *reinterpret_cast<const float4*>(tl[k].Genc + (size_t)min(row0 + cell_row, tl[k].B - 1) * G + 4 * unit);
+                }
+            }
+            have = true;
+        };
+        if (t > 0 && any_live) issue();
+#pragma unroll
+        for (int k = 0; k < RT; ++k) {
+            if (live[k] && (t > 0 || (RT == 2 && tl[k].t0 > 0))) {
+                const u32x4_t* hq = reinterpret_cast<const u32x4_t*>(hp + (size_t)(RT == 1 ? ((t - 1) & 1) : k) * 3 * G16_HP_PIECE) + lhi * 16 + lcol;
+                Frag16 fa[2][3];
+#pragma unroll
+                for (int c = 0; c < 3; ++c) fa[0][c].q = hq[(c * 32) * 16];
+#pragma unroll
+                for (int ks = 0; ks < 8; ++ks) {
+                    if (ks + 1 < 8) {
+#pragma unroll
+                        for (int c = 0; c < 3; ++c) fa[(ks + 1) & 1][c].q = hq[(c * 32 + 4 * (ks + 1)) * 16];
+                    }
+                    if (ks == 6 && (RT == 1 || (!have && (k == RT - 1 || !live[RT - 1])))) { check(); if (!have) issue(); }
+                    __builtin_amdgcn_sched_barrier(0);
+                    const bf16x8_t a0 = fa[ks & 1][0].v, a1 = fa[ks & 1][1].v, a2 = fa[ks & 1][2].v;
+                    acc[k][0] = __builtin_amdgcn_mfma_f32_16x16x32_bf16(a0, wg[ks * 3 + 0], acc[k][0], 0, 0, 0);
+                    acc[k][1] = __builtin_amdgcn_mfma_f32_16x16x32_bf16(a0, wg[ks * 3 + 1], acc[k][1], 0, 0, 0);
+                    acc[k][1] = __builtin_amdgcn_mfma_f32_16x16x32_bf16(a1, wg[ks * 3 + 0], acc[k][1], 0, 0, 0);
+                    acc[k][2] = __builtin_amdgcn_mfma_f32_16x16x32_bf16(a0, wg[ks * 3 + 2], acc[k][2], 0, 0, 0);
+                    acc[k][2] = __builtin_amdgcn_mfma_f32_16x16x32_bf16(a1, wg[ks * 3 + 1], acc[k][2], 0, 0, 0);
+                    acc[k][2] = __builtin_amdgcn_mfma_f32_16x16x32_bf16(a2, wg[ks * 3 + 0], acc[k][2], 0, 0, 0);
+                }
+                if constexpr (RT == 2) {
+#pragma unroll
+                    for (int i = 0; i < 4; ++i) acc[k][0][i] = (acc[k][2][i] + acc[k][1][i]) + acc[k][0][i];
+                }
+            }
+        }
+        if (t > 0 && any_live && !have) check();
+        I2L_STAMP16(0);
+        bool bail = false;
+        if (!have) {
+            long long t_start = 0;
+            unsigned spins = 0;
+            for (;;) {
+                issue();
+                check();
+                if (have) break;
+                __builtin_amdgcn_s_sleep(1);
+                if ((++spins & 255u) == 0) {
+                    const long long now = (long long)wall_clock64();
+                    if (t_start == 0) t_start = now;
+                    else if (now - t_start > p.opts.limit_step) { bail = true; break; }
+                }
+            }
+            if (bail) cnt_s[2] = 1;
+        }
+        if (t > 0 && !bail) {
+            bool all_fin = true;
+#pragma unroll
+            for (int k = 0; k < RT; ++k) {
+                if constexpr (RT == 1) {
+#pragma unroll
+                    for (int r = 0; r < G16Q; ++r) {
+                        const bool was_fin = (fin[k] >> r) & 1u;
+                        if (r == m && tid == 0 && ids_row[k]) ids_row[k][t - 1] = (p.stop == I2L_STOP_STICKY && was_fin) ? -1 : tk[r];
+                        if (tk[r] == p.end_id) fin[k] |= 1u << r;
+                        all_fin = all_fin && ((fin[k] >> r) & 1u);
+                    }
+                } else {
+                    if (t > nk[k]) continue;
+                    const int tok_m = __builtin_amdgcn_readlane(rowtok[k], m);
+                    if (tid == 0 && ids_row[k]) ids_row[k][tl[k].t0 + t - 1] = tok_m;
+                    fin[k] |= (unsigned)__ballot(lane < G16Q && rowtok[k] == p.end_id);
+                    if (t == nk[k] && tl[k].state_out) {
+                        const G16State st = group16_state(tl[k].state_out, tl[k].B);
+                        st.c[(size_t)(row0 + cell_row) * 256 + unit] = c_own[k];
+                        st.h[(size_t)(row0 + cell_row) * 256 + unit] = h_own[k];
+                        if (m == 0 && wave == 0 && lane < G16Q) st.tok[row0 + lane] = rowtok[k];
+                        if (m == 0 && tid == 0) st.fin[group] = fin[k];
+                    }
+                }
+            }
+            if (RT == 1 ? (t == tl[0].T || (p.stop == I2L_STOP_STICKY && all_fin)) : t == n_steps) break;
+        }
+        I2L_STAMP16(1);
+        if constexpr (RT == 2) __syncthreads();
+        if constexpr (RT == 2) {
+            unsigned wl_off = (unsigned)(((m * 4 + wave) * 36 * 64 + lane) * sizeof(u32x4_t));
+            asm volatile("" : "+v"(wl_off));
+            const u32x4_t* pk = reinterpret_cast<const u32x4_t*>(static_cast<const char*>(w.wpack16) + wl_off);
+#pragma unroll
+            for (int i = 0; i < 12; ++i) { Frag16 f; f.q = pk[(24 + i) * 64]; wl[i] = f.v; }
+        }
+        const unsigned epoch = ((unsigned)t + 1u) & 0xFFFFu;
+        const int par = t & 1;
+        u64_t* slot = xg + (size_t)par * G16Q * GRAN;
+        unsigned short* hcur = hp + (size_t)(RT == 1 ? par : 0) * 3 * G16_HP_PIECE;
+        if (!bail) {
+#pragma unroll
+            for (int k = 0; k < RT; ++k) {
+                if (RT == 1 || live[k]) {
+                    const bool b0 = lq & 1, b1 = lq & 2;
+                    float z[4];
+#pragma unroll
+                    for (int i = 0; i < 4; ++i) z[i] = RT == 1 ? (acc[k][2][i] + acc[k][1][i]) + acc[k][0][i] : acc[k][0][i];
+                    const float r0 = dpp_f<DPP_XOR1>(b0 ? z[0] : z[1]), r1 = dpp_f<DPP_XOR1>(b0 ? z[2] : z[3]);
+                    const float e0 = b0 ? r0 : z[0], e1 = b0 ? z[1] : r0, e2 = b0 ? r1 : z[2], e3 = b0 ? z[3] : r1;
+                    const float s0 = dpp_f<DPP_XOR2>(b1 ? e0 : e2), s1 = dpp_f<DPP_XOR2>(b1 ? e1 : e3);
+                    const float gi = b1 ? s0 : e0, gf = b1 ? s1 : e1, gc = b1 ? e2 : s0, go = b1 ? e3 : s1;
+                    const float xi = (gi + genc[k].x) + pvec[k].x, xf = (gf + genc[k].y) + pvec[k].y;
+                    const float xc = (gc + genc[k].z) + pvec[k].z, xo = (go + genc[k].w) + pvec[k].w;
+                    const float ig = sigmoidf_(xi), fg = sigmoidf_(xf), gg = tanhf_(xc), og = sigmoidf_(xo);
+                    c_own[k] = fg * c_own[k] + ig * gg;
+                    h_own[k] = og * tanhf_(c_own[k]);
+                }
+                unsigned short q0, q1, q2;
+                split3(h_own[k], q0, q1, q2);
+                const int ul = 4 * wave + uq;
+                const u64_t gran = ((u64_t)epoch << 48) | ((u64_t)q0 << 32) | ((u64_t)q1 << 16) | (u64_t)q2;
+                store_granule(slot + (size_t)m * GRAN + 256 * k + ((ul >> 3) * 16 + cell_row) * 8 + (ul & 7), gran, local);
+                const int o = ((2 * m + (ul >> 3)) * 16 + cell_row) * 8 + (ul & 7);
+                unsigned short* hk = hcur + (size_t)k * 3 * G16_HP_PIECE;
+                hk[o] = q0;
+                hk[G16_HP_PIECE + o] = q1;
+                hk[2 * G16_HP_PIECE + o] = q2;
+            }
+        }
+        I2L_STAMP16(2);
+        if (!bail) {
+            constexpr int NTASK = 15 * 32 * RT;
+#pragma unroll
+            for (int pi = 0; pi < RT; ++pi) {
+                const int ja = tid + 2 * G16NT * pi, jb = ja + G16NT < NTASK ? ja + G16NT : ja;
+                const int ka = RT == 2 && ja >= 480 ? 1 : 0, kb = RT == 2 && jb >= 480 ? 1 : 0;
+                const int ta = ja - 480 * ka, tb = jb - 480 * kb;
+                const int qa_ = ta >> 5, qa = qa_ + (qa_ >= m ? 1 : 0), qb_ = tb >> 5, qb = qb_ + (qb_ >= m ? 1 : 0);
+                const u64_t* sa = slot + (size_t)qa * GRAN + 256 * ka + (((ta >> 4) & 1) * 16 + (ta & 15)) * 8;
+                const u64_t* sb = slot + (size_t)qb * GRAN + 256 * kb + (((tb >> 4) & 1) * 16 + (tb & 15)) * 8;
+                u32x4_t g[8];
+                long long t_start = 0;
+                unsigned spins = 0;
+                for (;;) {
+                    if constexpr (RT == 1) load_run64x2(sa, sb, g);
+                    else load_run64x2_at(slot, (unsigned)((sa - slot) * sizeof(u64_t)), (unsigned)((sb - slot) * sizeof(u64_t)), g);
+                    bool ok = true;
+#pragma unroll
+                    for (int i = 0; i < 8; ++i) ok = ok && (g[i].y >> 16) == epoch && (g[i].w >> 16) == epoch;
+                    if (ok) break;
+                    __builtin_amdgcn_s_sleep(1);
+                    if ((++spins & 255u) == 0) {
+                        const long long now = (long long)wall_clock64();
+                        if (t_start == 0) t_start = now;
+                        else if (now - t_start > p.opts.limit_step) { cnt_s[2] = 1; break; }
+                    }
+                }
+                u32x4_t* ha = reinterpret_cast<u32x4_t*>(hcur + (size_t)ka * 3 * G16_HP_PIECE);
+                u32x4_t* hb = reinterpret_cast<u32x4_t*>(hcur + (size_t)kb * 3 * G16_HP_PIECE);
+                unpack_run(g, ha + (2 * qa + ((ta >> 4) & 1)) * 16 + (ta & 15));
+                unpack_run(g + 4, hb + (2 * qb + ((tb >> 4) & 1)) * 16 + (tb & 15));
+                if (RT == 2 && cnt_s[2] != 0) break;
+            }
+        }
+        I2L_STAMP16(3);
+        __syncthreads();
+        if (cnt_s[2] != 0) { failed = true; break; }
+        I2L_STAMP16(4);
+
+        {
+            auto logits_part = [&](int k) {
+                f32x4_t la[3] = {f32x4_t{0.f, 0.f, 0.f, 0.f}, f32x4_t{0.f, 0.f, 0.f, 0.f}, f32x4_t{0.f, 0.f, 0.f, 0.f}};
+                if (RT == 1 || live[k]) {
+                    const u32x4_t* hq = reinterpret_cast<const u32x4_t*>(hcur + (size_t)k * 3 * G16_HP_PIECE) + lhi * 16 + lcol;
+                    constexpr int PF = RT == 1 ? 4 : 2;
+                    Frag16 fa[4][3];
+#pragma unroll
+                    for (int ks = 0; ks < PF; ++ks)
+#pragma unroll
+                        for (int c = 0; c < 3; ++c) fa[ks][c].q = hq[(c * 32 + 4 * (4 * lhalf + ks)) * 16];
+#pragma unroll
+                    for (int ks = 0; ks < 4; ++ks) {
+                        const bf16x8_t a0 = fa[ks][0].v, a1 = fa[ks][1].v, a2 = fa[ks][2].v;
+                        if (ks + PF < 4) {
+#pragma unroll
+                            for (int c = 0; c < 3; ++c) fa[ks + PF][c].q = hq[(c * 32 + 4 * (4 * lhalf + ks + PF)) * 16];
+                        }
+                        if constexpr (RT == 2) __builtin_amdgcn_sched_barrier(0);
+                        la[0] = __builtin_amdgcn_mfma_f32_16x16x32_bf16(a0, wl[ks * 3 + 0], la[0], 0, 0, 0);
+                        la[1] = __builtin_amdgcn_mfma_f32_16x16x32_bf16(a0, wl[ks * 3 + 1], la[1], 0, 0, 0);
+                        la[1] = __builtin_amdgcn_mfma_f32_16x16x32_bf16(a1, wl[ks * 3 + 0], la[1], 0, 0, 0);
+                        la[2] = __builtin_amdgcn_mfma_f32_16x16x32_bf16(a0, wl[ks * 3 + 2], la[2], 0, 0, 0);
+                        la[2] = __builtin_amdgcn_mfma_f32_16x16x32_bf16(a1, wl[ks * 3 + 1], la[2], 0, 0, 0);
+                        la[2] = __builtin_amdgcn_mfma_f32_16x16x32_bf16(a2, wl[ks * 3 + 0], la[2], 0, 0, 0);
+                    }
+                }
+                f32x4_t part;
+#pragma unroll
+                for (int i = 0; i < 4; ++i) part[i] = (la[2][i] + la[1][i]) + la[0][i];
+                return part;
+            };
+            auto flag_of = [&](int k) { return RT == 1 ? (int)epoch : (int)((epoch << 1) | (unsigned)k); };
+            f32x4_t part[RT];
+            part[0] = logits_part(0);
+            if (lhalf == 1) {
+#pragma unroll
+                for (int k = 0; k < RT; ++k) {
+                    if (k > 0) {
+                        part[k] = logits_part(k);
+                        while (__hip_atomic_load(cnt_s + 6 + ltile, __ATOMIC_ACQUIRE, __HIP_MEMORY_SCOPE_WORKGROUP) != flag_of(k - 1))
+                            __builtin_amdgcn_s_sleep(0);
+                    }
+                    lpart[ltile * 64 + lane] = part[k];
+                    if (lane == 0) __hip_atomic_store(cnt_s + 4 + ltile, flag_of(k), __ATOMIC_RELEASE, __HIP_MEMORY_SCOPE_WORKGROUP);
+                }
+                I2L_STAMP16(5);
+            } else {
+#pragma unroll
+                for (int k = 1; k < RT; ++k) part[k] = logits_part(k);
+#pragma unroll
+                for (int k = 0; k < RT; ++k) {
+                    while (__hip_atomic_load(cnt_s + 4 + ltile, __ATOMIC_ACQUIRE, __HIP_MEMORY_SCOPE_WORKGROUP) != flag_of(k))
+                        __builtin_amdgcn_s_sleep(0);
+                    const f32x4_t other = lpart[ltile * 64 + lane];
+                    if (k + 1 < RT) {
+                        if (lane == 0) __hip_atomic_store(cnt_s + 6 + ltile, flag_of(k), __ATOMIC_RELEASE, __HIP_MEMORY_SCOPE_WORKGROUP);
+                    }
+                    if (k == RT - 1) I2L_STAMP16(5);
+                    const int l_v = 32 * m + 16 * ltile + lcol;
+#pragma unroll
+                    for (int i = 0; i < 4; ++i) {
+                        float lv = (part[k][i] + other[i]) + l_bias;
+                        if (p.use_temp) lv = lv / p.temperature;
+                        unsigned vk = __float_as_uint(lv + 0.0f);
+                        vk ^= (vk >> 31) ? 0xFFFFFFFFu : 0x80000000u;
+                        unsigned mx = vk;
+                        mx = max(mx, (unsigned)__builtin_amdgcn_mov_dpp((int)mx, DPP_ROR8, 0xF, 0xF, true));
+                        mx = max(mx, (unsigned)__builtin_amdgcn_mov_dpp((int)mx, DPP_ROR4, 0xF, 0xF, true));
+                        mx = max(mx, (unsigned)__builtin_amdgcn_mov_dpp((int)mx, DPP_XOR2, 0xF, 0xF, true));
+                        mx = max(mx, (unsigned)__builtin_amdgcn_mov_dpp((int)mx, DPP_XOR1, 0xF, 0xF, true));
+                        const unsigned long long hit = __ballot(vk == mx);
+                        const int first = __ffs((unsigned)(hit >> (16 * lhi)) & 0xFFFFu) - 1;
+                        const u64_t key = ((u64_t)mx << 32) | (u64_t)(0xFFFFFFFFu - (unsigned)(l_v - lcol + first));
+                        if (lcol == 0)
+                            atomicMax(reinterpret_cast<unsigned long long*>(redk + (par * RT + k) * 16 + 4 * lhi + i), (unsigned long long)key);
+                    }
+                }
+                int arrived = 0;
+                if (lane == 0) arrived = atomicAdd(cnt_s + par, 1);
+                arrived = __builtin_amdgcn_readfirstlane(arrived);
+                if (arrived == 1) {
+                    if (lane < 16 * RT) {
+                        const u64_t best = redk[par * RT * 16 + lane];
+                        store_granule(slot + (size_t)m * GRAN + GRAN_C + lane,
+                                      granule((epoch << 16) | (unsigned)(am_idx(best) & 0xFFFF), am_val(best)), local);
+                        redk[(par ^ 1) * RT * 16 + lane] = 0;
+                    }
+                    if (lane == 0) cnt_s[par ^ 1] = 0;
+                }
+                I2L_STAMP16(6);
+            }
+        }
+    }
+#ifdef I2L_GROUP_STAMPS
+    if (lane == 0 && (wave & 1) == 0 && blockIdx.x < 16)
+        for (int i = 0; i < 8; ++i) p.status[8 + blockIdx.x * 16 + (wave >> 1) * 8 + i] = (unsigned)st_acc[i];
+#endif
+#undef I2L_STAMP16
+    if (failed) {
+        if (lane == 0) atomicOr(p.status, 1u);
+#pragma unroll
+        for (int k = 0; k < RT; ++k) {
+            if (ids_row[k]) for (int tt = tid; tt < tl[k].T; tt += G16NT) ids_row[k][tt] = -3;
+            if constexpr (RT == 2) {
+                if (nk[k] > 0 && tl[k].state_out && tid == 0) atomicOr(group16_state(tl[k].state_out, tl[k].B).failed + group, 1u);
+            }
+        }
+        return;
+    }
+    if constexpr (RT == 1) {
+        if (ids_row[0]) for (int tt = t + tid; tt < tl[0].T; tt += G16NT) ids_row[0][tt] = -1;
+    } else {
+#pragma unroll
+        for (int k = 0; k < RT; ++k) {
+            if (!mark_failed[k] || row0 + m >= tl[k].B || !tl[k].ids) continue;
+            int32_t* row = tl[k].ids + (size_t)(row0 + m) * tl[k].T;
+            for (int tt = tid; tt < tl[k].T; tt += G16NT) row[tt] = -3;
+        }
+    }
+}
+
+constexpr int G16GRAN_H = G16Shape<1>::GRAN_H, G16GRAN_C = G16Shape<1>::GRAN_C, G16GRAN_X = G16Shape<1>::GRAN_X,
+              G16GRAN = G16Shape<1>::GRAN;
+template <>
+__global__ __launch_bounds__(G16NT, 2) void decode_group16_kernel<1>(GroupParams p) {
     extern __shared__ __attribute__((aligned(16))) unsigned char smem16[];
     unsigned short* hp = reinterpret_cast<unsigned short*>(smem16);
     f32x4_t* lpart = reinterpret_cast<f32x4_t*>(smem16 + (size_t)2 * 3 * G16_HP_PIECE * 2);
diff --git a/hmer-img2latex_amd/img2latex_amd/_lib.py b/hmer-img2latex_amd/img2latex_amd/_lib.py
--- a/hmer-img2latex_amd/img2latex_amd/_lib.py
+++ b/hmer-img2latex_amd/img2latex_amd/_lib.py
@@ -44,6 +44,11 @@
     _fields_ = [("embedding", c_void_p), ("w_ih", POINTER(c_void_p)), ("w_hh", POINTER(c_void_p)),
                 ("b_ih", POINTER(c_void_p)), ("b_hh", POINTER(c_void_p)), ("w_out", c_void_p),
                 ("b_out", c_void_p), ("vocab", c_int), ("embed", c_int), ("hidden", c_int), ("layers", c_int)]
+
+
+class DecodeHalf(ctypes.Structure):
+    _fields_ = [("workspace", c_void_p), ("rows", c_int), ("steps", c_int), ("first_step", c_int), ("n_steps", c_int),
+                ("tok0", c_void_p), ("ids_out", c_void_p)]
 
 
 class DecoderGrads(ctypes.Structure):
@@ -89,6 +94,8 @@
     "i2l_greedy_decode_ex": (c_int, [POINTER(DecoderWeights), c_void_p, c_int, c_int, c_void_p, c_void_p, c_void_p,
                                      c_void_p, c_float, c_int, c_int, c_int, c_int, c_void_p, c_void_p, c_void_p,
                                      c_void_p, c_int, c_void_p, ctypes.c_uint32, c_void_p]),
+    "i2l_greedy_decode_halves": (c_int, [POINTER(DecoderWeights), POINTER(DecodeHalf), POINTER(DecodeHalf), c_float, c_int,
+                                         c_int, c_int, c_int, c_void_p, ctypes.c_uint32, c_void_p]),
     "i2l_decode_batched_scratch_bytes": (c_size_t, [c_int, c_int, c_int, c_int]),
     "i2l_greedy_decode_batched": (c_int, [POINTER(DecoderWeights), c_void_p, c_int, c_int, c_void_p, c_void_p, c_void_p,
                                           c_void_p, c_float, c_int, c_int, c_int, c_void_p, c_void_p, c_void_p, c_void_p,
@@ -170,6 +177,8 @@
     "i2l_global_avgpool_bwd_f32": (c_int, [c_void_p, c_void_p, c_int, c_int, c_int, c_int, c_void_p]),
     "i2l_decoder_group_status_offset": (c_size_t, [c_int, c_int, c_int, c_int, c_int]),
     "i2l_decoder_group_region_bytes": (c_size_t, [c_int] * 5),
+    "i2l_decoder_group_state_offset": (c_size_t, [c_int] * 5),
+    "i2l_decoder_group_state_bytes": (c_size_t, [c_int] * 5),
     "i2l_resample_ksize": (c_int, [c_int, c_int, c_int]),
     "i2l_resample_coeffs": (c_int, [c_int, c_int, c_int, c_void_p, c_void_p]),
     "i2l_resample_coeffs_batch": (c_int, [c_int, c_int, c_void_p, c_void_p, c_void_p, c_void_p, c_int]),
diff --git a/hmer-img2latex_amd/img2latex_amd/model/lstm_decoder.py b/hmer-img2latex_amd/img2latex_amd/model/lstm_decoder.py
--- a/hmer-img2latex_amd/img2latex_amd/model/lstm_decoder.py
+++ b/hmer-img2latex_amd/img2latex_amd/model/lstm_decoder.py
@@ -1,7 +1,7 @@
 from __future__ import annotations
 
 import ctypes
-from typing import Optional, Tuple
+from typing import NamedTuple, Optional, Tuple
 
 import torch
 import torch.nn as nn
@@ -31,6 +31,17 @@
             self.attn.bias.detach().data_ptr(), self.v.weight.detach().contiguous().data_ptr(), ctx.data_ptr(),
             B, S, self.hidden_dim, E, _lib.stream_ptr()), "attention_context_fwd")
         return ctx
+
+
+class DecodeHalf(NamedTuple):
+    ws: torch.Tensor
+    version: tuple
+    rows: int
+    steps: int
+    first_step: int
+    n_steps: int
+    tok0: torch.Tensor
+    ids: torch.Tensor
 
 
 class LSTMDecoder(nn.Module):
@@ -179,6 +190,36 @@
         del keep
         return ids, logits, ((h, c) if want_state else None)
 
+    def halves_supported(self, stop: int = _lib.STOP_NONE) -> bool:
+        return stop == _lib.STOP_NONE and _lib.lib().i2l_decoder_group_state_bytes(
+            16, self.vocab_size, self.embedding_dim, self.hidden_dim, self.lstm_layers) != 0
+
+    def decode_halves(self, older: Optional["DecodeHalf"], newer: Optional["DecodeHalf"], temperature: float = 1.0,
+                      select: int = _lib.SELECT_LOGITS, stop: int = _lib.STOP_NONE, end_id: int = -1, flags: int = 0,
+                      resident=None) -> None:
+        halves = [h for h in (older, newer) if h is not None]
+        if not halves:
+            raise RuntimeError("img2latex_amd: decode_halves needs at least one batch")
+        if len({h.version for h in halves}) != 1 or halves[0].version != self._weights_version():
+            raise RuntimeError("img2latex_amd: decode_halves: the two workspaces were prepared for different weights")
+        w, keep = self._weights_struct()
+        structs = []
+        for h in (older, newer):
+            if h is None:
+                structs.append(None)
+                continue
+            if tuple(h.ids.shape) != (h.rows, h.steps) or h.ids.dtype != torch.int32 or not h.ids.is_contiguous():
+                raise RuntimeError(f"decode_halves: ids must be contiguous int32 ({h.rows},{h.steps})")
+            structs.append(_lib.DecodeHalf(h.ws.data_ptr(), h.rows, h.steps, h.first_step, h.n_steps,
+                                           _lib.require_gpu(h.tok0, "tok0", torch.int32).data_ptr(), h.ids.data_ptr()))
+        _lib.check(_lib.lib().i2l_greedy_decode_halves(
+            ctypes.byref(w), None if structs[0] is None else ctypes.byref(structs[0]),
+            None if structs[1] is None else ctypes.byref(structs[1]), float(temperature), select, stop, int(end_id),
+            int(flags) | int(self.kernel_flags), None if resident is None else resident[0].data_ptr(),
+            0 if resident is None else int(resident[1]) & 0xFFFFFFFF, _lib.stream_ptr()), "greedy_decode_halves")
+        _lib.mark("decode")
+        del keep
+
     def sample_steps(self, encoder_output: torch.Tensor, steps: int, tok0: torch.Tensor, temperature: float,
                      top_k: int, top_p: float, seed: int, stop: int = _lib.STOP_STICKY, end_id: int = -1,
                      hidden: Optional[Hidden] = None, want_probs: bool = False):
diff --git a/hmer-img2latex_amd/img2latex_amd/pipeline.py b/hmer-img2latex_amd/img2latex_amd/pipeline.py
--- a/hmer-img2latex_amd/img2latex_amd/pipeline.py
+++ b/hmer-img2latex_amd/img2latex_amd/pipeline.py
@@ -6,6 +6,15 @@
 import torch
 
 from . import _lib
+from .model.lstm_decoder import DecodeHalf
+
+
+class _Batch:
+    __slots__ = ("no", "done", "host", "enc", "text", "half", "slot", "ids")
+
+    def __init__(self, no, host, enc, slot):
+        self.no, self.host, self.enc, self.slot = no, host, enc, slot
+        self.done = self.text = self.half = self.ids = None
 
 
 class GreedyPipeline:
@@ -15,7 +24,8 @@
                  decode_flags: int = 0, encoder_flags: int = 0, decode_priority: int = 0, encoder_streams: int = 1,
                  encoder_priority: int = 0, hold_encoder: Optional[bool] = None, wait_timeout_us: float = 20000.0,
                  clear_early: bool = True,
-                 stop: int = _lib.STOP_NONE, select: int = _lib.SELECT_LOGITS, detokenize=None):
+                 stop: int = _lib.STOP_NONE, select: int = _lib.SELECT_LOGITS, detokenize=None,
+                 split_decode: Optional[bool] = None):
         self.model = model
         self.start, self.end, self.max_length, self.temperature = start_token_id, end_token_id, max_length, temperature
         dev = next(model.parameters()).device
@@ -41,7 +51,19 @@
         self._resident = torch.zeros(1, dtype=torch.int32, device=dev)
         self.trace: Optional[list] = None
         self.trace_every = 1
-        self._inflight: Deque[Tuple[torch.cuda.Event, torch.Tensor, torch.Tensor]] = deque()
+        self._inflight: Deque[_Batch] = deque()
+        dec = model.decoder
+        can_split = (bool(self.decode_flags & _lib.FLAG_DECODE_GROUP16) and self.stop == _lib.STOP_NONE
+                     and len(self.dec_streams) == 1 and self.rows_per_workgroup == 0 and max_length >= 8
+                     and not (int(getattr(dec, "kernel_flags", 0)) & _lib.FLAG_DECODE_BATCHED)
+                     and hasattr(dec, "halves_supported") and dec.halves_supported(self.stop))
+        if split_decode and not can_split:
+            raise RuntimeError("img2latex_amd: GreedyPipeline(split_decode=True) needs decode_flags with FLAG_DECODE_GROUP16, "
+                               "rows_per_workgroup=0, stop=STOP_NONE, one decode stream, max_length >= 8 and a decoder the "
+                               "16-member grouped kernel takes")
+        self.split_decode = can_split if split_decode is None else bool(split_decode)
+        self._open: Optional[_Batch] = None
+        self._tok0: dict = {}
         self.copy_stream = torch.cuda.Stream(device=dev)
         self._batch_no = 0
         self._slots = self.depth + 1
@@ -100,6 +122,9 @@
                 enc.record_stream(dec_stream)
                 if rec is not None:
                     rec["dec_start"].record(dec_stream)
+                if self.split_decode:
+                    self._submit_split(enc, prepared, slot, seq, dflags, rec, dec_stream)
+                    return
                 ids, _ = self.model.greedy_ids(enc, self.start, self.end, self.max_length, self.temperature,
                                                stop=self.stop, select=self.select,
                                                rows_per_workgroup=self.rows_per_workgroup, flags=dflags,
@@ -107,40 +132,90 @@
                                                resident=(self._resident, seq) if self.hold_encoder else None)
                 if rec is not None:
                     rec["dec_end"].record(dec_stream)
-                host = self._host_buffer(ids.shape)
-                text = dev_text = None
-                if self.detok is not None:
-                    key = (slot, tuple(ids.shape))
-                    if key not in self._text_dev:
-                        self._text_dev = {k: v for k, v in self._text_dev.items() if k[0] != slot}
-                        self._text_dev[key] = self.detok.buffers(*ids.shape)
-                    dev_text = self.detok.launch(ids, self.end, self._text_dev[key])
-                    text = self._text_buffer(dev_text)
-                if self.copy_stream is None:
-                    host.copy_(ids, non_blocking=True)
-                    if text is not None:
-                        text[0].copy_(dev_text[0], non_blocking=True)
-                        text[1].copy_(dev_text[1], non_blocking=True)
-                    done = torch.cuda.Event()
-                    done.record(dec_stream)
-                else:
-                    decoded = torch.cuda.Event()
-                    decoded.record(dec_stream)
-                    self.copy_stream.wait_event(decoded)
-                    with torch.cuda.stream(self.copy_stream):
-                        host.copy_(ids, non_blocking=True)
-                        if text is not None:
-                            text[0].copy_(dev_text[0], non_blocking=True)
-                            text[1].copy_(dev_text[1], non_blocking=True)
-                        done = torch.cuda.Event()
-                        done.record(self.copy_stream)
-                    ids.record_stream(self.copy_stream)
-        self._inflight.append((done, host, enc, text))
+                b = _Batch(seq - 1, self._host_buffer(ids.shape), enc, slot)
+                b.ids = ids
+                self._finish(b, dec_stream)
+        self._inflight.append(b)
+
+    def _finish(self, b: _Batch, dec_stream) -> None:
+        ids, host, slot = b.ids, b.host, b.slot
+        text = dev_text = None
+        if self.detok is not None:
+            key = (slot, tuple(ids.shape))
+            if key not in self._text_dev:
+                self._text_dev = {k: v for k, v in self._text_dev.items() if k[0] != slot}
+                self._text_dev[key] = self.detok.buffers(*ids.shape)
+            dev_text = self.detok.launch(ids, self.end, self._text_dev[key])
+            text = self._text_buffer(dev_text)
+        if self.copy_stream is None:
+            host.copy_(ids, non_blocking=True)
+            if text is not None:
+                text[0].copy_(dev_text[0], non_blocking=True)
+                text[1].copy_(dev_text[1], non_blocking=True)
+            done = torch.cuda.Event()
+            done.record(dec_stream)
+        else:
+            decoded = torch.cuda.Event()
+            decoded.record(dec_stream)
+            self.copy_stream.wait_event(decoded)
+            with torch.cuda.stream(self.copy_stream):
+                host.copy_(ids, non_blocking=True)
+                if text is not None:
+                    text[0].copy_(dev_text[0], non_blocking=True)
+                    text[1].copy_(dev_text[1], non_blocking=True)
+                done = torch.cuda.Event()
+                done.record(self.copy_stream)
+            ids.record_stream(self.copy_stream)
+        b.text, b.done, b.half, b.ids = text, done, None, None
+
+    def _submit_split(self, enc, prepared, slot, seq, dflags, rec, dec_stream) -> None:
+        dec = self.model.decoder
+        no, T = seq - 1, self.max_length
+        assert not self._inflight or self._inflight[0].no > no - self._slots, "a slot workspace is still in use"
+        w, keep, enc_c, ws = prepared
+        rows = enc_c.shape[0]
+        if rows not in self._tok0:
+            self._tok0[rows] = torch.full((rows,), int(self.start), dtype=torch.int32, device=self.device)
+        ids = torch.empty((rows, T), dtype=torch.int32, device=self.device)
+        first = (T + 1) // 2
+        b = _Batch(no, self._host_buffer(ids.shape), enc, slot)
+        b.ids = ids
+        newer = DecodeHalf(ws, dec._ws_key[2], rows, T, 0, first, self._tok0[rows], ids)
+        older, prev = None, self._open
+        if prev is not None:
+            dims = (dec.vocab_size, dec.embedding_dim, dec.hidden_dim, dec.lstm_layers)
+            nb = _lib.lib().i2l_decoder_group_region_bytes
+            if prev.half.version == newer.version and nb(prev.half.rows, *dims) <= nb(rows, *dims):
+                older = prev.half
+            else:
+                self._launch_tail(prev, dec_stream)
+        kw = dict(temperature=self.temperature, select=self.select, stop=self.stop, end_id=self.end)
+        dec.decode_halves(older, newer, flags=dflags, resident=(self._resident, seq) if self.hold_encoder else None, **kw)
+        if rec is not None:
+            rec["dec_end"].record(dec_stream)
+        if older is not None:
+            self._finish(prev, dec_stream)
+        self._open = None
+        if first < T:
+            b.half = newer._replace(first_step=first, n_steps=T - first)
+            self._open = b
+        else:
+            self._finish(b, dec_stream)
+        self._inflight.append(b)
+
+    def _launch_tail(self, b: _Batch, dec_stream) -> None:
+        flags = self.decode_flags & ~_lib.FLAG_DECODE_REGION_CLEARED
+        self.model.decoder.decode_halves(b.half, None, temperature=self.temperature, select=self.select, stop=self.stop,
+                                         end_id=self.end, flags=flags)
+        self._finish(b, dec_stream)
+        if self._open is b:
+            self._open = None
 
     def close(self) -> None:
         inflight = getattr(self, "_inflight", None)
         if inflight:
             inflight.clear()
+            self._open = None
             for s in self.enc_streams + self.dec_streams + [self.copy_stream]:
                 if s is not None:
                     s.synchronize()
@@ -194,7 +269,11 @@
     def _collect(self):
         if not self._inflight:
             return None
-        done, host, enc, text = self._inflight.popleft()
+        b = self._inflight.popleft()
+        if b.done is None:
+            with torch.no_grad(), torch.cuda.stream(self.dec_streams[0]):
+                self._launch_tail(b, self.dec_streams[0])
+        done, host, enc, text = b.done, b.host, b.enc, b.text
         done.synchronize()
         if _lib.ids_timed_out(host):
             import warnings
diff --git a/include/img2latex_hip.h b/include/img2latex_hip.h
--- a/include/img2latex_hip.h
+++ b/include/img2latex_hip.h
@@ -305,6 +305,19 @@
 size_t i2l_decoder_group_status_offset(int rows, int vocab, int embed, int hidden, int layers);
 size_t i2l_decoder_group_region_bytes(int rows, int vocab, int embed, int hidden, int layers);
 
+typedef struct {
+    const void* workspace;
+    int rows, steps;
+    int first_step, n_steps;
+    const int32_t* tok0;
+    int32_t* ids_out;
+} i2l_decode_half;
+int i2l_greedy_decode_halves(const i2l_decoder_weights* w, const i2l_decode_half* older, const i2l_decode_half* newer,
+                             float temperature, int select, int stop, int end_id, int flags,
+                             uint32_t* resident_flag, uint32_t resident_value, i2l_stream_t stream);
+size_t i2l_decoder_group_state_offset(int rows, int vocab, int embed, int hidden, int layers);
+size_t i2l_decoder_group_state_bytes(int rows, int vocab, int embed, int hidden, int layers);
+
 
 int i2l_lanczos_ksize(int in_size, int out_size);
 int i2l_lanczos_coeffs(int in_size, int out_size, int32_t* bounds_out, int32_t* kk_out);
diff --git a/profiles/decode_halves_cost.py b/profiles/decode_halves_cost.py
--- /dev/null
+++ b/profiles/decode_halves_cost.py
@@ -0,0 +1,122 @@
+import argparse
+import os
+import statistics
+import sys
+import time
+
+import torch
+
+ROOT = os.path.join(os.path.dirname(os.path.abspath(__file__)), "..")
+sys.path.insert(0, os.path.join(ROOT, "hmer-img2latex_amd"))
+from img2latex_amd import _lib, synth
+from img2latex_amd.model import Seq2SeqModel
+from img2latex_amd.model.lstm_decoder import DecodeHalf
+from img2latex_amd.pipeline import GreedyPipeline
+
+STEPS, B = 150, 256
+G16 = _lib.FLAG_DECODE_GROUP16
+
+
+def build(dev):
+    cfg = synth.model_config()
+    sd = synth.make_state_dict(cfg, seed=42, out_scale=12.0, enc_scale=16.0, end_clock=(0.05, 12.0, 6.0))
+    m = Seq2SeqModel("cnn_lstm", cfg["vocab_size"], synth.encoder_params(cfg), synth.decoder_params(cfg))
+    m.load_state_dict({k: torch.from_numpy(v.copy()) for k, v in sd.items()})
+    return m.to(dev).eval(), cfg
+
+
+def timed(fn, reps, warmup):
+    ms = []
+    for i in range(warmup + reps):
+        a, b = torch.cuda.Event(enable_timing=True), torch.cuda.Event(enable_timing=True)
+        a.record()
+        fn()
+        b.record()
+        b.synchronize()
+        if i >= warmup:
+            ms.append(a.elapsed_time(b))
+    return statistics.median(ms), min(ms), max(ms)
+
+
+def launch_alone(m, cfg, reps, warmup, dev, out):
+    dec = m.decoder
+    xs = [torch.from_numpy(synth.make_images(B, cfg, seed=s)).to(dev) for s in (1234, 77)]
+    encs = [m.encoder(x).clone() for x in xs]
+    tok0 = torch.full((B,), synth.START, dtype=torch.int32, device=dev)
+    batches = []
+    for i, enc in enumerate(encs):
+        w, keep, enc_c = dec.prepare(enc, slot=("cost", "decode-halves-cost", i))
+        batches.append(dict(prepared=(w, keep, enc_c, dec._ws), ws=dec._ws, version=dec._ws_key[2], enc=enc,
+                            ids=torch.empty((B, STEPS), dtype=torch.int32, device=dev)))
+    first = (STEPS + 1) // 2
+    half = lambda b, t0, n: DecodeHalf(b["ws"], b["version"], B, STEPS, t0, n, tok0, b["ids"])
+    one = lambda b, steps: dec.run_steps(b["enc"], steps, tok0, flags=G16, end_id=synth.END, prepared=b["prepared"])[0]
+    want = [one(b, STEPS).cpu() for b in batches]
+    dec.decode_halves(None, half(batches[0], 0, first), end_id=synth.END)
+    dec.decode_halves(half(batches[0], first, STEPS - first), half(batches[1], 0, first), end_id=synth.END)
+    dec.decode_halves(half(batches[1], first, STEPS - first), None, end_id=synth.END)
+    for b, w_ in zip(batches, want):
+        assert torch.equal(b["ids"].cpu(), w_), "split ids differ from the one-launch ids"
+    dec.decode_halves(None, half(batches[0], 0, first), end_id=synth.END)
+    pair = lambda: dec.decode_halves(half(batches[0], first, STEPS - first), half(batches[1], 0, first), end_id=synth.END)
+    rows = [("RT = 1, one launch of 150 steps", lambda: one(batches[0], STEPS), 150),
+            ("RT = 1, two launches of 75 steps", lambda: (one(batches[0], first), one(batches[1], first)), 150),
+            ("RT = 2, one launch: 75 + 75 steps of two batches", pair, 75)]
+    out.append(f"1. the launch alone, B = {B} (median / min / max ms over {reps} launches; us per launch step)")
+    for name, fn, steps in rows:
+        med, lo, hi = timed(fn, reps, warmup)
+        out.append(f"   {name:52s} {med:7.4f} / {lo:7.4f} / {hi:7.4f} ms   {med * 1e3 / steps:6.3f} us per step")
+    dec.release_slots("decode-halves-cost")
+
+
+def pipeline(m, cfg, batches, rounds, dev, out):
+    x = torch.from_numpy(synth.make_images(B, cfg, seed=1234)).to(dev)
+    res = {True: [], False: []}
+    for _ in range(rounds):
+        for split in (True, False):
+            pipe = GreedyPipeline(m, synth.START, synth.END, STEPS, depth=3, rows_per_workgroup=0, decode_streams=1,
+                                  decode_flags=G16, decode_priority=-1, split_decode=None if split else False)
+            assert pipe.split_decode == split
+            for phase in range(2):
+                torch.cuda.synchronize()
+                t0 = time.perf_counter()
+                for _ in range(batches):
+                    if pipe.pending() >= pipe.depth:
+                        pipe.collect()
+                    pipe.submit(x)
+                while pipe.pending():
+                    pipe.collect()
+                torch.cuda.synchronize()
+                dt = time.perf_counter() - t0
+            res[split].append(dt * 1e3 / batches)
+            pipe.close()
+    out.append(f"2. GreedyPipeline, depth 3, B = {B}, {STEPS} steps: ms per batch over {batches} batches, {rounds} alternating rounds")
+    for split in (True, False):
+        v = res[split]
+        out.append(f"   split_decode {'on ' if split else 'off'}  median {statistics.median(v):.4f}  min {min(v):.4f}  max {max(v):.4f}"
+                   f"   ({B * STEPS / statistics.median(v) / 1e3:.2f} M tokens/s)")
+
+
+def main():
+    ap = argparse.ArgumentParser()
+    ap.add_argument("--reps", type=int, default=40)
+    ap.add_argument("--warmup", type=int, default=10)
+    ap.add_argument("--batches", type=int, default=120)
+    ap.add_argument("--rounds", type=int, default=3)
+    ap.add_argument("--out", default=None)
+    a = ap.parse_args()
+    dev = torch.device("cuda:0")
+    out = []
+    with torch.no_grad():
+        m, cfg = build(dev)
+        launch_alone(m, cfg, a.reps, a.warmup, dev, out)
+        pipeline(m, cfg, a.batches, a.rounds, dev, out)
+    text = "\n".join(out)
+    print(text)
+    if a.out:
+        with open(a.out, "w") as f:
+            f.write(text + "\n")
+
+
+if __name__ == "__main__":
+    main()
```

Result: faster. 41.39 million (median of 6 runs) (+3.1%).
